# flysoaryun/LF-VIO

Measured on AMD Instinct MI355X. Metric: sliding-window solves/sec (10 KF x N landmarks), higher is better.
Workload: dtype f64; 1 GPU; window300; landmarks=300, observations=1419, windows_per_gpu=1, marginalization=MARGIN_OLD, parallelism=1 independent window stream(s), one per GPU, no data-path collective

## Files before the change

lf-vio_amd/csrc/kernels_lin.h:

```cpp
#pragma once
#include "dev_factors.h"
#include "kernels_spec.h"
#include "tr_decide.h"
#include <type_traits>

#define SLOT(base, stride) ((Slot *)((char *)(base) + (size_t)blockIdx.y * (stride)))

constexpr int MODE_SOLVE = 0;
constexpr int MODE_MARG = 1;
constexpr int MODE_GATED = 16;
constexpr int MODE_DECIDE = 64;
constexpr int MODE_NOCOUNT = 32;
DEV bool tail_gate(const Slot *S, int done) { return done && S->tail_state == 0; }
DEV bool is_marg(int mode) { return mode >= MODE_MARG; }
DEV const MargPlan *marg_plan(const Slot *S, int mode) { return &S->marg[mode - MODE_MARG]; }

DEV int gidx20(int p, int q) { return p * 20 - (p * (p - 1)) / 2 + (q - p); }

constexpr int SETUP_PRIOR_WGS = 16;
constexpr int SETUP_WGS = 2 + SETUP_PRIOR_WGS;
constexpr int SETUP_TILED_MAXN = 88;
__global__ __launch_bounds__(256, 4) void k_setup(char *base, size_t stride, int mode, int zero_wt) {
  Slot *S = SLOT(base, stride);
  const int tid = threadIdx.x;
  constexpr int SETUP_PRIOR_SLAB = 2048, SETUP_LDS = LFVIO_WINDOW_SIZE * 15 * 16;
  static_assert(SETUP_LDS >= SETUP_PRIOR_SLAB + LFVIO_MAX_PRIOR_DIM && SETUP_LDS >= 84 + TAB_SCRATCH, "k_setup's workspace");
  __shared__ double sh_setup[SETUP_LDS];
  const int setup_wgs = (zero_wt & 4) ? 3 : SETUP_WGS;
  if (blockIdx.x == 0) {
    const double *src = (const double *)&S->x0;
    double *dst = (double *)&S->x[0];
    for (int k = tid; k < (int)(sizeof(FrameState) / 8); k += 256) dst[k] = src[k];
    if (tid == 0) {
      TRState *t = &S->tr;
      tr_init(t, S->init_radius, S->fn_tol);
      S->tail_state = 0;
      S->passes_used = 0;
      S->dec_pending = 0;
      if (mode >= MODE_MARG) t->mu = 0.0;
    }
    double *bt = sh_setup;
    if (tid < 77) bt[tid] = (&S->x0.pose[0][0])[tid];
    else if (tid < 84) bt[tid] = S->x0.ex[tid - 77];
    __syncthreads();
    const unsigned offm = build_tab(bt, &S->tab[0], tid, bt + 84);
    if (tid == 0) S->ex_fixed_off = ((offm >> TAB_EX_BIT) & 1u) && !S->est_ex;
    if (tid == 0 && S->spec_on) spec_arm(S);
  } else if (blockIdx.x == 1) {
    if (tid >= 16 * ((LFVIO_WINDOW_SIZE + 3) & ~3)) return;
    const int grp = tid >> 4, l = tid & 15;
    const int f = grp < LFVIO_WINDOW_SIZE ? grp : 0;
    const bool mine = grp < LFVIO_WINDOW_SIZE && S->imu_active[f];
    const double *cov = S->imu[f].covariance;
    double m0[15], m1[15];
#pragma unroll
    for (int r = 0; r < 15; r++) {
      m0[r] = l < 15 ? cov[r * 15 + l] : (r == 0 ? 1.0 : 0.0);
      m1[r] = r == l + 1 ? 1.0 : 0.0;
    }
#pragma unroll
    for (int k = 0; k < 15; k++) {
      int p = k;
      double best = -1.0, piv = 0.0;
#pragma unroll
      for (int r = 0; r < 15; r++) {
        const double v = fabs(m0[r]);
        if (r >= k && v > best) best = v, p = r, piv = m0[r];
      }
      p = row_bcast_ik(p, k), piv = row_bcast_k(piv, k);
      double csr[15];
#pragma unroll
      for (int r = 0; r < 15; r++) csr[r] = row_bcast_k(m0[r], k);
      const double ck = csr[k];
#pragma unroll
      for (int r = 0; r < 15; r++) csr[r] = r == p ? ck : csr[r];
      auto step = [&](double(&m)[15]) {
        double Mp = m[0];
#pragma unroll
        for (int r = 1; r < 15; r++) Mp = p == r ? m[r] : Mp;
        const double Mk = m[k], mk = Mp / piv;
#pragma unroll
        for (int r = 0; r < 15; r++) {
          const double Msr = r == p ? Mk : m[r];
          m[r] = r == k ? mk : Msr - csr[r] * mk;
        }
      };
      step(m0), step(m1);
    }
    double *T = sh_setup + f * (15 * 16);
#pragma unroll
    for (int r = 0; r < 15; r++) {
      if (l == 15) T[r * 16] = m0[r];
      else if (l < 14) T[r * 16 + l + 1] = m1[r];
    }
    __syncthreads();
    const int li = l < 15 ? l : 0;
    double lrow[15], mrow[15];
#pragma unroll
    for (int j = 0; j < 15; j++) mrow[j] = T[li * 16 + j], lrow[j] = 0.0;
    bool ok = true;
#pragma unroll
    for (int j = 0; j < 15; j++) {
      double t = mrow[j];
#pragma unroll
      for (int k = 0; k < j; k++) t -= lrow[k] * row_bcast_k(lrow[k], j);
      const double sj = row_bcast_k(t, j);
      if (!(sj > 0.0)) ok = false;
      const double d = sqrt(sj);
      lrow[j] = l == j ? d : t / d;
    }
    if (mine && l < 15) {
#pragma unroll
      for (int i = 0; i < 15; i++) S->imu_sqrt[f][i * 15 + l] = (l >= i && ok) ? lrow[i] : 0.0;
    }
    if (mine && !ok && l == 0) S->imu_active[f] = 0;
  } else if (blockIdx.x >= setup_wgs) {
    const int l = (blockIdx.x - setup_wgs) * 256 + tid;
    if (l < S->N) S->lam[0][l] = S->lam0[l];
    if ((zero_wt & 1) && !S->wt_clean) {
      double2 *wt = (double2 *)(double *)S->Wt;
      const int nw = gridDim.x - setup_wgs, w = blockIdx.x - setup_wgs;
      for (int e = w * 256 + tid; e < WT_PAIRS * SPEC_MAX_LM; e += nw * 256) wt[e] = make_double2(0.0, 0.0);
    }
  } else {
    if (!S->prior_valid) return;
    const int n = S->prior_n;
    const int part = blockIdx.x - 2;
    constexpr int PRIOR_EPT = 8;
    const int nb4 = (n + 3) >> 2, tiles = nb4 * (nb4 + 1) / 2;
    static_assert(((SETUP_TILED_MAXN + 3) / 4) * ((SETUP_TILED_MAXN + 3) / 4 + 1) / 2 <= 256, "a thread per 4 x 4 block of the upper triangle");
    if (zero_wt & 4) {
      if (part != 0) return;
      constexpr int PRIOR_SLAB = SETUP_PRIOR_SLAB;
      double *Js = sh_setup;
      const double *J = S->prior_J;
      const int rows_per = PRIOR_SLAB / n;
      int br = 0, rem = tid < tiles ? tid : 0;
      while (rem >= nb4 - br) rem -= nb4 - br, br++;
      const int r0 = 4 * br, c0 = 4 * (br + rem);
      double acc[4][4], accb = 0;
#pragma unroll
      for (int i = 0; i < 4; i++)
#pragma unroll
        for (int j = 0; j < 4; j++) acc[i][j] = 0.0;
      for (int k0 = 0; k0 < n; k0 += rows_per) {
        const int nk = min(rows_per, n - k0);
        __syncthreads();
        {
          double v[8];
          const double *Jk = J + k0 * n;
#pragma unroll
          for (int q = 0; q < 8; q++) v[q] = Jk[tid + 256 * q < nk * n ? tid + 256 * q : 0];
          const double rv = S->prior_r[k0 + (tid < nk ? tid : 0)];
#pragma unroll
          for (int q = 0; q < 8; q++)
            if (tid + 256 * q < nk * n) Js[tid + 256 * q] = v[q];
          if (tid < nk) Js[PRIOR_SLAB + tid] = rv;
        }
        __syncthreads();
        if (tid < tiles) {
#pragma unroll 2
          for (int k = 0; k < nk; k++) {
            double a[4], b[4];
#pragma unroll
            for (int i = 0; i < 4; i++) a[i] = Js[k * n + r0 + i], b[i] = Js[k * n + c0 + i];
#pragma unroll
            for (int i = 0; i < 4; i++)
#pragma unroll
              for (int j = 0; j < 4; j++) acc[i][j] = fma(a[i], b[j], acc[i][j]);
          }
        }
        if (tid < n)
          for (int k = 0; k < nk; k++) accb = fma(Js[k * n + tid], Js[PRIOR_SLAB + k], accb);
      }
      if (tid < tiles) {
#pragma unroll
        for (int i = 0; i < 4; i++)
#pragma unroll
          for (int j = 0; j < 4; j++) {
            const int r = r0 + i, c = c0 + j;
            if (r < n && c < n) {
              S->prior_A[r * n + c] = acc[i][j];
              if (c0 != r0) S->prior_A[c * n + r] = acc[i][j];
            }
          }
      }
      if (tid < n) S->prior_b0[tid] = accb;
      return;
    }
    const int np = gridDim.y >= 8 ? min(SETUP_PRIOR_WGS, (n * n + 256 * PRIOR_EPT - 1) / (256 * PRIOR_EPT)) : SETUP_PRIOR_WGS;
    if (part >= np) return;
    constexpr int PRIOR_SLAB = SETUP_PRIOR_SLAB;
    double *Js = sh_setup;
    const double *J = S->prior_J;
    const int rows_per = PRIOR_SLAB / n;
    double acc[PRIOR_EPT], accb = 0;
#pragma unroll
    for (int q = 0; q < PRIOR_EPT; q++) acc[q] = 0;
    for (int k0 = 0; k0 < n; k0 += rows_per) {
      const int nk = min(rows_per, n - k0);
      __syncthreads();
      {
        static_assert(PRIOR_SLAB <= 8 * 256, "eight elements of a slab per thread");
        double v[8];
        const double *Jk = J + k0 * n;
#pragma unroll
        for (int q = 0; q < 8; q++) v[q] = Jk[tid + 256 * q < nk * n ? tid + 256 * q : 0];
        const double rv = S->prior_r[k0 + (tid < nk ? tid : 0)];
#pragma unroll
        for (int q = 0; q < 8; q++)
          if (tid + 256 * q < nk * n) Js[tid + 256 * q] = v[q];
        if (tid < nk) Js[PRIOR_SLAB + tid] = rv;
      }
      __syncthreads();
#pragma unroll
      for (int q = 0; q < PRIOR_EPT; q++) {
        const int e = part * 256 + tid + q * 256 * np;
        if (e < n * n) {
          const int r = e / n, c = e % n;
          double s = acc[q];
          for (int k = 0; k < nk; k++) s = fma(Js[k * n + r], Js[k * n + c], s);
          acc[q] = s;
        }
      }
      if (part == 0 && tid < n)
        for (int k = 0; k < nk; k++) accb = fma(Js[k * n + tid], Js[PRIOR_SLAB + k], accb);
    }
#pragma unroll
    for (int q = 0; q < PRIOR_EPT; q++) {
      const int e = part * 256 + tid + q * 256 * np;
      if (e < n * n) S->prior_A[e] = acc[q];
    }
    if (part == 0 && tid < n) S->prior_b0[tid] = accb;
  }
}

DEV void load_pair_uniform(const Tab *T, int pair, PairU &u) {
  u.M2 = ldm(T->M2[pair]);
  u.T = ldm(T->T[pair]);
  u.ric = ldm(T->ric);
  u.ricT = ldm(T->ricT);
  u.c = ld3(T->c[pair]);
  u.tic = ld3(T->tic);
  u.offc = u.offr = nullptr;
}
DEV void load_pair_uniform(const Tab *T, int pair, unsigned offm, PairU &u) {
  load_pair_uniform(T, pair, u);
  if (offm && pair_is_off(offm, pair % 11)) u.offc = T->c[tab_cj(pair)], u.offr = T->T[0];
}

typedef double double4_t __attribute__((ext_vector_type(4)));

constexpr int LIN_THREADS = 256;
constexpr int LIN_LDS_LM = LM_BLOCK * (WLD + 1) + 64 + 2 * LM_BLOCK;
constexpr int LIN_PRIOR_N = 76;
constexpr int LIN_LDS_PRIOR = LIN_PRIOR_N * LIN_PRIOR_N + 4 * KP;
constexpr int LIN_LDS = LIN_LDS_LM > LIN_LDS_PRIOR ? LIN_LDS_LM : LIN_LDS_PRIOR;

DEV double quad_sum(double v) {
  v += dpp_f64<0xB1>(v);
  v += dpp_f64<0x4E>(v);
  return v;
}
DEV d3 quad_sum3(d3 v) { return mk3(quad_sum(v.x), quad_sum(v.y), quad_sum(v.z)); }
template <int LPT>
DEV double track_sum(double v) { return LPT == 8 ? sum8(v) : quad_sum(v); }
template <int LPT>
DEV d3 track_sum3(d3 v) { return mk3(track_sum<LPT>(v.x), track_sum<LPT>(v.y), track_sum<LPT>(v.z)); }

template <bool TIGHT>
DEV void schur_block(int lm0, int lmb, int mode, int Nlim, double (*tile)[WLD + 1], const double *lcoef, const double *le, double *part) {
  const int tid = threadIdx.x;
  const int wv = tid >> 6, lane = tid & 63, kk = lane >> 4, cc = lane & 15;
  double4_t acc[4];
  int ct[4], cu[4];
  bool scale_k[4];
#pragma unroll
  for (int j = 0; j < 4; j++) {
    acc[j] = double4_t{0, 0, 0, 0};
    const int ti = wv + 4 * j;
    const int t = ti < 5 ? 0 : ti < 9 ? 1 : ti < 12 ? 2 : ti < 14 ? 3 : 4;
    const int u = ti - (t * 5 - (t * (t - 1)) / 2) + t;
    ct[j] = ti < NT ? 16 * t + cc : 0, cu[j] = ti < NT ? 16 * u + cc : 0;
    scale_k[j] = mode == MODE_SOLVE && cu[j] == COL_K;
  }
  int rows = Nlim - lm0;
  rows = rows > lmb ? lmb : rows;
  auto sweep = [&](auto ntl) {
    constexpr int NTL = decltype(ntl)::value;
    for (int s4 = 0; 4 * s4 < rows; s4++) {
      const int row = 4 * s4 + kk;
      const double coef = lcoef[row], eb = le[row];
#pragma unroll
      for (int j = 0; j < NTL; j++)
        acc[j] = __builtin_amdgcn_mfma_f64_16x16x4f64(coef * tile[row][ct[j]], tile[row][cu[j]] * (scale_k[j] ? eb : 1.0), acc[j], 0, 0, 0);
    }
  };
  if (TIGHT) {
    if (__builtin_amdgcn_readfirstlane(wv) + 12 < NT) sweep(std::integral_constant<int, 4>{});
    else sweep(std::integral_constant<int, 3>{});
  } else {
    for (int s4 = 0; 4 * s4 < rows; s4++) {
      const int row = 4 * s4 + kk;
      const double coef = lcoef[row], eb = le[row];
#pragma unroll
      for (int j = 0; j < 4; j++) {
        if (wv + 4 * j >= NT) continue;
        const double xa = tile[row][ct[j]];
        double xb = tile[row][cu[j]];
        if (mode == MODE_SOLVE && cu[j] == COL_K) xb *= eb;
        acc[j] = __builtin_amdgcn_mfma_f64_16x16x4f64(coef * xa, xb, acc[j], 0, 0, 0);
      }
    }
  }
#pragma unroll
  for (int j = 0; j < 4; j++) {
    if (wv + 4 * j >= NT) continue;
#pragma unroll
    for (int r = 0; r < 4; r++) part[(wv + 4 * j) * 256 + r * 64 + lane] = acc[j][r];
  }
}
DEV int w_col(int ci, int start, int cnt) { return ci < 6 * cnt ? 6 * start + ci : 66 + (ci - 6 * cnt); }

struct LinView {
  const FrameState *x;
  const Tab *tab;
  const double *lam;
  double mu;
};

template <int LPT>
DEV void lin_schur_only_role(Slot *S, const LinView &lv, int wg, double *lds, double *part) {
  constexpr int LMB = LIN_THREADS / LPT;
  double(*tile)[WLD + 1] = (double(*)[WLD + 1]) lds;
  double *lcoef = lds + LM_BLOCK * (WLD + 1) + 64, *le = lcoef + LM_BLOCK;
  const int tid = threadIdx.x;
  for (int e = tid; e < LM_BLOCK * (WLD + 1); e += LIN_THREADS) lds[e] = 0.0;
  __syncthreads();
  {
    const int lml = tid / LPT, q = tid % LPT, l = wg * LMB + lml;
    if (l < S->N) {
      const int st = S->lm_start[l], cnt = S->lm_cnt[l];
      const double *w = S->W + S->lm_woff[l];
      for (int ci = q; ci < w_row_len(cnt); ci += LPT) tile[lml][w_col(ci, st, cnt)] = w[ci];
    }
  }
  if (tid < LM_BLOCK) {
    const int l = wg * LMB + tid;
    double cf = 0.0, eb = 0.0;
    if (tid < LMB && l < S->N) {
      const double sc = S->scale_l[l], s2a = sc * sc * S->a[l];
      const double D2 = fmin(fmax(s2a, 1e-6), 1e32);
      eb = s2a + lv.mu * D2;
      const double einv = 1.0 / eb;
      cf = sc * sc * einv;
      S->einv_l[l] = einv;
    }
    lcoef[tid] = cf, le[tid] = eb;
  }
  __syncthreads();
  schur_block<false>(wg * LMB, LMB, MODE_SOLVE, S->N, tile, lcoef, le, part);
}

#ifdef LFVIO_LIN_PROFILE
#define LSTAMP(k) do { if (blockIdx.x == 0 && mode == MODE_SOLVE && threadIdx.x == 0) S->dbg[k] = (long long)__builtin_readcyclecounter(); } while (0)
#else
#define LSTAMP(k) do { } while (0)
#endif
template <bool TIGHT, int LPT, bool OFFS>
DEV void lin_landmark_role(Slot *S, const LinView &lv, int wg, int mode, double *lds, double *part) {
  constexpr int LMB = LIN_THREADS / LPT;
  double(*tile)[WLD + 1] = (double(*)[WLD + 1]) lds;
  double *red = lds + LM_BLOCK * (WLD + 1);
  double *lcoef = red + 64, *le = lcoef + LM_BLOCK;
  const int tid = threadIdx.x, lml = tid / LPT, q = tid % LPT;
  const TRState *tr = &S->tr;
  const Tab *T = lv.tab;
  const int Nlim = is_marg(mode) ? marg_plan(S, mode)->N0 : S->N;
  const int l = wg * LMB + lml;
  const bool valid = l < Nlim;
  const int est_td = S->est_td;
  const int est_ex = is_marg(mode) ? 1 : S->est_ex;
  const double td = lv.x->td;
  LSTAMP(22);
  for (int e = tid; e < LM_BLOCK * (WLD + 1); e += LIN_THREADS) lds[e] = 0.0;
  if (tid < 2 * LM_BLOCK) lcoef[tid] = 0.0;
// ... 82 lines not shown
    }
    S->a[l] = a;
    S->b[l] = b;
    tile[lml][COL_B] = b;
    lam2 = lam * lam;
    bmax = fabs(b);
  } else {
    cost = 0.0;
  }
  LSTAMP(18);
  cost = wave_sum(cost);
  g2 = wave_sum(g2);
  asv2 = wave_sum(asv2);
  lam2 = wave_sum(lam2);
  bmax = wave_max(bmax);
  if ((tid & 63) == 0) {
    double *r = red + 8 * (tid >> 6);
    r[0] = cost, r[1] = g2, r[2] = asv2, r[3] = lam2, r[4] = bmax;
  }
  lds_barrier();
  if (tid < 5) {
    double *p = S->lm_part + (size_t)(LPT == 8 ? wg >> 1 : wg) * LMS + (LPT == 8 && (wg & 1) ? 10 : 0);
    p[tid] = tid < 4 ? ((red[tid] + red[8 + tid]) + (red[16 + tid] + red[24 + tid]))
                     : fmax(fmax(red[4], red[12]), fmax(red[20], red[28]));
  }
  LSTAMP(19);
  if (valid) {
    double *w = S->W + woff_l;
    for (int ci = q; ci < w_row_len(cnt_l); ci += LPT) w[ci] = tile[lml][w_col(ci, i, cnt_l)];
  }
  if (TIGHT && mode == MODE_SOLVE && S->N <= SPEC_MAX_LM) {
    constexpr int WGRP = LIN_THREADS / LMB;
    const int lr = tid % LMB, wg4 = tid / LMB;
    double2 *wt = (double2 *)(double *)S->Wt + wg * LMB + lr;
    constexpr int WPT = (WT_PAIRS + WGRP - 1) / WGRP;
    double2 v[WPT];
#pragma unroll
    for (int k = 0; k < WPT; k++) {
      const int cp = wg4 + WGRP * k, c = cp < WT_PAIRS ? 2 * cp : 0;
      v[k] = make_double2(tile[lr][c], c + 1 < KC ? tile[lr][c + 1] : 0.0);
    }
#pragma unroll
    for (int k = 0; k < WPT; k++) {
      const int cp = wg4 + WGRP * k;
      if (cp < WT_PAIRS) wt[(size_t)cp * SPEC_MAX_LM] = v[k];
    }
  }
  LSTAMP(23);
  schur_block<TIGHT>(wg * LMB, LMB, mode, Nlim, tile, lcoef, le, part);
  LSTAMP(20);
}

template <bool OFFS>
DEV void lin_gram_role(Slot *S, const LinView &lv, int wg, int mode, double *lds) {
  const int wv = threadIdx.x >> 6, lane = threadIdx.x & 63;
  const int chunk = 4 * wg + wv;
  if (chunk >= S->nChunks) return;
  if (is_marg(mode) && chunk >= marg_plan(S, mode)->nChunks0) return;
  double *my = lds + wv * (32 * 17 + 256 + 14 * 20);
  double(*stage)[17] = (double(*)[17]) my;
  double(*Qf)[16] = (double(*)[16])(my + 32 * 17);
  double(*E)[20] = (double(*)[20])(my + 32 * 17 + 256);
  double(*T1)[20] = (double(*)[20]) my;
  const Tab *T = lv.tab;
  const int pair = S->chunk_pair[chunk];
  const int j = pair % 11;
  const int begin = S->chunk_begin[chunk], end = S->chunk_end[chunk];
  const int est_td = S->est_td;
  const double td = lv.x->td;
  PairU u;
  if (OFFS) load_pair_uniform(T, pair, tab_offmask(T), u);
  else load_pair_uniform(T, pair, u);
  for (int e = lane; e < 14 * 20; e += 64) E[0][e] = 0.0;
  for (int e = lane; e < 32 * 17; e += 64) stage[0][e] = 0.0;
  const int idx = begin + lane;
  double c0[14], c1[14];
#pragma unroll
  for (int e = 0; e < 14; e++) c0[e] = c1[e] = 0.0;
  if (idx < end) {
    const int oj = S->pm_obs[idx], l = S->pm_lm[idx];
    const int oi = S->lm_obs0[l];
    const double lam = lv.lam[l];
    ObsPair ob;
    load_obs(S, oi, ob.pi, ob.vi, ob.tdi, ob.rowi);
    load_obs(S, oj, ob.pj, ob.vj, ob.tdj, ob.rowj);
    Basis B;
    visual_basis<OFFS>(ob, lam, td, est_td, S->tr_over_row, S->half_row, S->sqrt_info, u, B);
    c0[0] = B.red[0].x, c0[1] = B.red[0].y, c0[2] = B.red[0].z;
    c1[0] = B.red[1].x, c1[1] = B.red[1].y, c1[2] = B.red[1].z;
    c0[3] = B.jti[0].x, c0[4] = B.jti[0].y, c0[5] = B.jti[0].z;
    c1[3] = B.jti[1].x, c1[4] = B.jti[1].y, c1[5] = B.jti[1].z;
    c0[6] = B.jtj[0].x, c0[7] = B.jtj[0].y, c0[8] = B.jtj[0].z;
    c1[6] = B.jtj[1].x, c1[7] = B.jtj[1].y, c1[8] = B.jtj[1].z;
    c0[9] = B.jtx[0].x, c0[10] = B.jtx[0].y, c0[11] = B.jtx[0].z;
    c1[9] = B.jtx[1].x, c1[10] = B.jtx[1].y, c1[11] = B.jtx[1].z;
    c0[12] = B.jtd[0], c1[12] = B.jtd[1];
    c0[13] = B.r[0], c1[13] = B.r[1];
  }
  double4_t acc = double4_t{0, 0, 0, 0};
  const int nrounds = (end - begin + 15) >> 4;
  for (int r = 0; r < nrounds; r++) {
    __builtin_amdgcn_fence(__ATOMIC_RELEASE, "wavefront");
    if ((lane >> 4) == r) {
      const int row = 2 * (lane & 15);
#pragma unroll
      for (int e = 0; e < 14; e++) stage[row][e] = c0[e], stage[row + 1][e] = c1[e];
    }
    __builtin_amdgcn_fence(__ATOMIC_ACQ_REL, "wavefront");
#pragma unroll
    for (int g = 0; g < 8; g++) {
      const double v = stage[4 * g + (lane >> 4)][lane & 15];
      acc = __builtin_amdgcn_mfma_f64_16x16x4f64(v, v, acc, 0, 0, 0);
    }
  }
  __builtin_amdgcn_fence(__ATOMIC_RELEASE, "wavefront");
#pragma unroll
  for (int r = 0; r < 4; r++) Qf[(lane >> 4) + 4 * r][lane & 15] = acc[r];
  if (lane < 9) {
    const int r = lane / 3, c = lane % 3;
    const double m1 = T->M1[j][lane];
    E[r][c] = m1;
    E[r][6 + c] = -m1;
    E[r][12 + c] = T->M2[pair][lane] - T->ricT[lane];
  } else if (lane < 12) {
    const int k = lane - 9;
    E[3 + k][3 + k] = 1.0;
    E[6 + k][9 + k] = 1.0;
    E[9 + k][15 + k] = 1.0;
  } else if (lane == 12) {
    E[12][18] = 1.0;
    E[13][19] = 1.0;
  }
  __builtin_amdgcn_fence(__ATOMIC_ACQ_REL, "wavefront");
  for (int e = lane; e < 14 * 20; e += 64) {
    const int r = e / 20, c = e % 20;
    double s = 0;
#pragma unroll
    for (int k = 0; k < 14; k++) s = fma(Qf[r][k], E[k][c], s);
    T1[r][c] = s;
  }
  __builtin_amdgcn_fence(__ATOMIC_ACQ_REL, "wavefront");
  double *out = S->gram_part + (size_t)chunk * NGP;
  for (int e = lane; e < 400; e += 64) {
    const int p = e / 20, c = e % 20;
    if (p > c) continue;
    double s = 0;
#pragma unroll
    for (int k = 0; k < 14; k++) s = fma(E[k][p], T1[k][c], s);
    out[gidx20(p, c)] = s;
  }
}

template <bool raw_ready>
DEV void lin_imu_role(Slot *S, const LinView &lv, int f, int mode, double *lds) {
  double(*Jr)[30] = (double(*)[30]) lds;
  double(*Jw)[31] = (double(*)[31])(lds + 450);
  double *rr = lds + 450 + 465, *rw = rr + 16;
  const int tid = threadIdx.x;
  double *out = S->imu_out + (size_t)f * IMU_OUT;
  const bool active = S->imu_active[f] && (mode == MODE_SOLVE || (f == 0 && marg_plan(S, mode)->use_imu0)) &&
                      (!S->sharded || S->pose_side);
  if (!active) {
    for (int e = tid; e < IMU_OUT; e += LIN_THREADS) out[e] = 0.0;
    return;
  }
  const FrameState *x = lv.x;
  if (raw_ready) {
    const double *raw = S->imu_raw + (size_t)f * IMU_RAW;
    for (int e = tid; e < 450; e += LIN_THREADS) Jr[e / 30][e % 30] = raw[e];
    if (tid < 15) rr[tid] = raw[450 + tid];
  } else {
    for (int e = tid; e < 450; e += LIN_THREADS) Jr[e / 30][e % 30] = 0.0;
    __syncthreads();
    if (tid == 0) imu_raw_residual(&S->imu[f], S->g, x->pose[f], x->sb[f], x->pose[f + 1], x->sb[f + 1], rr);
    if (tid == 64) imu_raw_jacobian(&S->imu[f], S->g, x->pose[f], x->sb[f], x->pose[f + 1], x->sb[f + 1], &Jr[0][0]);
  }
  __syncthreads();
  const double *Sq = S->imu_sqrt[f];
  if (tid < 15) {
    double s = 0;
    for (int k = 0; k < 15; k++) s = fma(Sq[tid * 15 + k], rr[k], s);
    rw[tid] = s;
  }
  for (int e = tid; e < 450; e += LIN_THREADS) {
    const int r = e / 30, c = e % 30;
    double s = 0;
    for (int k = r; k < 15; k++) s = fma(Sq[r * 15 + k], Jr[k][c], s);
    Jw[r][c] = s;
  }
  __syncthreads();
  for (int e = tid; e < 900; e += LIN_THREADS) {
    const int p = e / 30, c = e % 30;
    double s = 0;
#pragma unroll
    for (int k = 0; k < 15; k++) s = fma(Jw[k][p], Jw[k][c], s);
    out[e] = s;
  }
  if (tid < 30) {
    double s = 0;
#pragma unroll
    for (int k = 0; k < 15; k++) s = fma(Jw[k][tid], rw[k], s);
    out[900 + tid] = s;
  }
  if (tid == 32) {
    double s = 0;
    for (int k = 0; k < 15; k++) s = fma(rw[k], rw[k], s);
    out[930] = 0.5 * s;
  }
}

template <bool STAGED>
DEV void lin_prior_role(Slot *S, const LinView &lv, int mode, double *lds) {
  const int n = S->prior_n;
  const bool staged = STAGED && n <= LIN_PRIOR_N;
  double *Js = lds, *dx = lds + (STAGED ? LIN_PRIOR_N * LIN_PRIOR_N : 0), *r = dx + KP, *part = r + KP;
  const int tid = threadIdx.x;
  double *g = S->prior_g;
  for (int c = tid; c < KP + 4; c += LIN_THREADS) g[c] = 0.0;
  if (!S->prior_valid || (S->sharded && !S->pose_side)) return;
  const FrameState *x = lv.x;
  const double *Jg = S->prior_J;
  if (staged) {
    constexpr int PER = (LIN_PRIOR_N * LIN_PRIOR_N + LIN_THREADS - 1) / LIN_THREADS;
    double v[PER];
#pragma unroll
    for (int k = 0; k < PER; k++) v[k] = tid + LIN_THREADS * k < n * n ? Jg[tid + LIN_THREADS * k] : 0.0;
    if (tid < S->prior_nb) prior_block_dx(S, x, tid, dx);
#pragma unroll
    for (int k = 0; k < PER; k++)
      if (tid + LIN_THREADS * k < n * n) Js[tid + LIN_THREADS * k] = v[k];
  } else if (tid < S->prior_nb) {
    prior_block_dx(S, x, tid, dx);
  }
  __syncthreads();
  const double *J = staged ? Js : Jg;
  for (int row = tid >> 2; row < n; row += LIN_THREADS / 4) {
    double s = 0;
    for (int c = tid & 3; c < n; c += 4) s = fma(J[row * n + c], dx[c], s);
    s = quad_sum(s);
    if ((tid & 3) == 0) r[row] = S->prior_r[row] + s;
  }
  __syncthreads();
  {
    const int c = tid & 127, h = tid >> 7, k0 = h ? n / 2 : 0, k1 = h ? n : n / 2;
    for (int cc = c; cc < n; cc += 128) {
      double s = 0;
      for (int k = k0; k < k1; k++) s = fma(J[k * n + cc], r[k], s);
      part[h * KP + cc] = s;
    }
  }
  __syncthreads();
  for (int c = tid; c < n; c += LIN_THREADS) g[S->prior_cmap[c]] = part[c] + part[KP + c];
  if (tid < 64) {
    double cs = 0;
    for (int row = tid; row < n; row += 64) cs += r[row] * r[row];
    cs = wave_sum(cs);
    if (tid == 0) g[KP] = 0.5 * cs;
  }
}

__global__ __launch_bounds__(64) void k_imu_raw(char *base, size_t stride, int count) {
  const int g = blockIdx.x * 64 + threadIdx.x;
  if (g >= count * LFVIO_WINDOW_SIZE) return;
  const int slot = g / LFVIO_WINDOW_SIZE, f = g - slot * LFVIO_WINDOW_SIZE;
  Slot *S = reinterpret_cast<Slot *>(base + stride * (size_t)slot);
  const TRFlags fl = tr_flags(&S->tr);
  if (fl.done | !fl.do_lin) return;
  if (!S->imu_active[f] || (S->sharded && !S->pose_side)) return;
  const FrameState *x = &S->x[fl.cur];
  double *raw = S->imu_raw + (size_t)f * IMU_RAW;
  for (int e = 0; e < 450; e++) raw[e] = 0.0;
  imu_raw_residual(&S->imu[f], S->g, x->pose[f], x->sb[f], x->pose[f + 1], x->sb[f + 1], raw + 450);
  imu_raw_jacobian(&S->imu[f], S->g, x->pose[f], x->sb[f], x->pose[f + 1], x->sb[f + 1], raw);
}

constexpr int LIN_ROLE_LM = 1, LIN_ROLE_GRAM = 2, LIN_ROLE_POSE = 4, LIN_ROLE_ALL = 7;
constexpr int LIN_ROLE_POSE_RAW = 8;
constexpr int LIN_LDS_POSE = 1024;
template <int ROLES, bool OFFS = true>
__global__ __launch_bounds__(LIN_THREADS, ROLES == LIN_ROLE_GRAM ? 3 : (ROLES == LIN_ROLE_POSE_RAW ? 6 : 2)) void k_lin(char *base, size_t stride, int mode_bits, int gLw, int gCh) {
  Slot *S = SLOT(base, stride);
  TRState *tr = &S->tr;
  const int mode = mode_bits & (MODE_GATED - 1);
  LSTAMP(21);
  const TRFlags fl = tr_flags(tr);
  int do_lin = fl.do_lin, do_schur = fl.do_schur, cur = fl.cur, acc_z = 0;
  double mu = tr->mu;
  int num_succ = tr->num_succ;
  if (mode_bits & MODE_GATED) {
    if (!tail_gate(S, fl.done)) return;
  } else {
    int done = fl.done;
    const bool owner = blockIdx.x == 0 && !(mode_bits & MODE_NOCOUNT);
    if ((mode_bits & MODE_DECIDE) && !done) {
      __shared__ TRDecision dsh;
      if (threadIdx.x < 64) {
        TRHead t = *reinterpret_cast<const TRHead *>(tr);
        const int K = decide_candidates(t);
        DecideSums sm;
        decide_sums(S, t, K, 0, S->nLmBlocks, threadIdx.x, sm);
        if (threadIdx.x == 0) {
          const int az = decide_walk(t, sm, K, 0, S->max_iter, owner ? tr : nullptr);
          decision_from(dsh, t, az);
          if (owner) S->dec = dsh, S->dec_pending = 1;
        }
      }
      __syncthreads();
      do_lin = __builtin_amdgcn_readfirstlane(dsh.do_lin), do_schur = __builtin_amdgcn_readfirstlane(dsh.do_schur);
      cur = __builtin_amdgcn_readfirstlane(dsh.cur), acc_z = __builtin_amdgcn_readfirstlane(dsh.acc_z), done = __builtin_amdgcn_readfirstlane(dsh.done);
      num_succ = __builtin_amdgcn_readfirstlane(dsh.num_succ);
      mu = __hiloint2double(__builtin_amdgcn_readfirstlane(__double2hiint(dsh.mu)), __builtin_amdgcn_readfirstlane(__double2loint(dsh.mu)));
      if (acc_z > 0 && blockIdx.x == gridDim.x - 1 && !(mode_bits & MODE_NOCOUNT)) {
        copy_accepted(S, acc_z, cur, S->N, threadIdx.x, LIN_THREADS);
        if (S->spec_on) {
          __threadfence();
          __syncthreads();
          if (threadIdx.x == 0) spec_publish(S, num_succ, cur);
        }
      } else if (acc_z == 0 && owner && threadIdx.x == 0 && S->spec_on) spec_publish(S, num_succ, cur);
    } else if (owner && threadIdx.x == 0 && mode == MODE_SOLVE && S->spec_on) spec_publish(S, num_succ, cur);
    if (mode == MODE_SOLVE && owner && !done && threadIdx.x == 0) S->passes_used++;
    if (done | (!do_lin & !do_schur)) return;
  }
  LinView lv;
  lv.x = acc_z > 0 ? &S->xE[acc_z > 0 ? acc_z - 1 : 0] : &S->x[cur];
  lv.tab = acc_z > 0 ? &S->tabE[acc_z > 0 ? acc_z - 1 : 0] : &S->tab[cur];
  lv.lam = acc_z > 0 ? (const double *)S->lamE[acc_z > 0 ? acc_z - 1 : 0] : (const double *)S->lam[cur];
  lv.mu = mu;
  __shared__ __attribute__((aligned(16))) double lds[(ROLES & (LIN_ROLE_LM | LIN_ROLE_GRAM)) ? LIN_LDS : LIN_LDS_POSE];
  int b = blockIdx.x;
  if (b < gLw) {
    if (ROLES & LIN_ROLE_LM) {
      const int half = S->lm_half, lmb = half ? LM_BLOCK / 2 : LM_BLOCK;
      const int nblk = ((is_marg(mode) ? marg_plan(S, mode)->N0 : S->N) + lmb - 1) / lmb;
      if (b >= nblk) return;
      double *part = S->schur_part + (size_t)b * SCHUR_LEN;
      if (half) {
        if (do_lin) lin_landmark_role<ROLES == LIN_ROLE_ALL, 8, OFFS>(S, lv, b, mode, lds, part);
        else lin_schur_only_role<8>(S, lv, b, lds, part);
      } else {
        if (do_lin) lin_landmark_role<ROLES == LIN_ROLE_ALL, 4, OFFS>(S, lv, b, mode, lds, part);
        else lin_schur_only_role<4>(S, lv, b, lds, part);
      }
    }
    return;
  }
  if (!do_lin) return;
  b -= gLw;
  if (b < gCh) {
    if (ROLES & LIN_ROLE_GRAM) lin_gram_role<OFFS>(S, lv, b, mode, lds);
    return;
  }
  b -= gCh;
  if (ROLES & (LIN_ROLE_POSE | LIN_ROLE_POSE_RAW)) {
    if (b < LFVIO_WINDOW_SIZE) {
      if (ROLES & LIN_ROLE_POSE_RAW) lin_imu_role<true>(S, lv, b, mode, lds);
      else lin_imu_role<false>(S, lv, b, mode, lds);
      return;
    }
    lin_prior_role<ROLES == LIN_ROLE_ALL>(S, lv, mode, lds);
  }
}

DEV int schur_index(int R, int Cc) {
  const int t = R >> 4, u = Cc >> 4;
  const int tile = t * 5 - (t * (t - 1)) / 2 + (u - t);
  const int row = R & 15, col = Cc & 15;
  return tile * 256 + (row >> 2) * 64 + ((row & 3) << 4) + col;
}

constexpr int HPP_ITEMS = PACKED + KP;
constexpr int HPP_BLOCKS = (HPP_ITEMS + 255) / 256;

DEV int imu_local(int c, int f) {
  if (c < 66) {
    const int fr = c / 6, l = c - 6 * fr;
    if (fr == f) return l;
    if (fr == f + 1) return 15 + l;
    return -1;
  }
  if (c < KC) return -1;
  const int fr = (c - KC) / 9, l = (c - KC) - 9 * fr;
  if (fr == f) return 6 + l;
  if (fr == f + 1) return 21 + l;
  return -1;
}
DEV int col_frame(int c) { return c < 66 ? c / 6 : (c < KC ? -10 : (c - KC) / 9); }
DEV bool pose_terms_here(const Slot *S, int r) { return !S->sharded || S->pose_side == 1 || (S->pose_side == 2 && r >= KC); }

DEV bool col_active(const Slot *S, int c, int mode) {
  if (mode >= MODE_MARG) return true;
  if (!S->est_ex && c >= off_ex() && c < off_ex() + 6) return false;
  if (!S->est_td && c == off_td()) return false;
  return true;
}

constexpr int PRE_GROUP = 32;
__global__ __launch_bounds__(256) void k_presum(char *base, size_t stride, int mode_bits, int groups) {
  const int PRE_SCHUR_BLOCKS = (SCHUR_LEN / 256) * groups;
  Slot *S = SLOT(base, stride);
  const TRState *tr = &S->tr;
  const int mode = mode_bits & (MODE_GATED - 1);
  const TRFlags fl = tr_flags_decided(S);
  if (mode_bits & MODE_GATED) {
    if (!tail_gate(S, fl.done)) return;
  } else if (fl.done | (!fl.do_lin & !fl.do_schur)) return;
  const int tid = threadIdx.x;
  int b = blockIdx.x;
  if (b < NPAIR) {
    if (!fl.do_lin) return;
    const int chunk_limit = is_marg(mode) ? marg_plan(S, mode)->nChunks0 : S->nChunks;
    const int c0 = S->pair_chunk0[b];
    int c1 = S->pair_chunk0[b + 1];
    if (c1 > chunk_limit) c1 = chunk_limit;
    if (tid < NGP) {
      const double *gp = S->gram_part + tid;
      double s0 = 0, s1 = 0, s2 = 0, s3 = 0;
      int c = c0;
      for (; c + 4 <= c1; c += 4) {
        s0 += gp[(size_t)c * NGP], s1 += gp[(size_t)(c + 1) * NGP];
        s2 += gp[(size_t)(c + 2) * NGP], s3 += gp[(size_t)(c + 3) * NGP];
      }
      for (; c < c1; c++) s0 += gp[(size_t)c * NGP];
      S->pairG[(size_t)b * NGP + tid] = (s0 + s1) + (s2 + s3);
    }
    return;
  }
  b -= NPAIR;
  if (b < PRE_SCHUR_BLOCKS) {
    if (!fl.do_schur) return;
    const int grp = b / (SCHUR_LEN / 256), e = (b % (SCHUR_LEN / 256)) * 256 + tid;
    int parts = S->nSchurParts;
    if (is_marg(mode)) parts = (marg_plan(S, mode)->N0 + S->schur_lm - 1) / S->schur_lm;
    const int p0 = grp * PRE_GROUP;
    if (p0 >= parts) return;
    const int p1 = min(parts, p0 + PRE_GROUP);
    double *sp = S->schur_part + e;
    double a0 = 0, a1 = 0, a2 = 0, a3 = 0;
    int p = p0;
    for (; p + 4 <= p1; p += 4) {
      a0 += sp[(size_t)p * SCHUR_LEN], a1 += sp[(size_t)(p + 1) * SCHUR_LEN];
      a2 += sp[(size_t)(p + 2) * SCHUR_LEN], a3 += sp[(size_t)(p + 3) * SCHUR_LEN];
    }
    for (; p < p1; p++) a0 += sp[(size_t)p * SCHUR_LEN];
    sp[(size_t)p0 * SCHUR_LEN] = (a0 + a1) + (a2 + a3);
    return;
  }
  if (!fl.do_lin) return;
  __shared__ double red[5][256];
  const int blocks = S->nLmBlocks;
  double v[5] = {0, 0, 0, 0, 0};
  for (int k = tid; k < blocks; k += 256) {
    const double *q = S->lm_part + (size_t)k * LMS;
    v[0] += q[0], v[1] += q[1], v[2] += q[2], v[3] += q[3], v[4] = fmax(v[4], q[4]);
  }
#pragma unroll
  for (int k = 0; k < 5; k++) red[k][tid] = v[k];
  __syncthreads();
  for (int w = 128; w > 0; w >>= 1) {
    if (tid < w) {
#pragma unroll
      for (int k = 0; k < 4; k++) red[k][tid] += red[k][tid + w];
      red[4][tid] = fmax(red[4][tid], red[4][tid + w]);
    }
    __syncthreads();
  }
  if (tid < 5) S->lm_sum[tid] = red[tid][0];
}

struct SumArgs {
  long long sum_off, sum_end_marg, sum_items, gram_part, pairG, imu_out, prior_A;
};
template <class T>
DEV T *blob_at(const Slot *S, long long off) { return (T *)((char *)S + off); }
#define SUM_KEEP(v) asm volatile("" ::"v"(v))

DEV void sum_hpp_entry(Slot *S, const SumArgs &o, int mode_bits, int e) {
  const int mode = mode_bits & (MODE_GATED - 1);
  const bool in = e < HPP_ITEMS;
  const int ec = in ? e : 0;
  const bool packed = ec < PACKED;
  int r, c;
  if (packed) {
    r = (int)((sqrt(8.0 * ec + 1.0) - 1.0) * 0.5);
    while ((r + 1) * (r + 2) / 2 <= ec) r++;
    while (r * (r + 1) / 2 > ec) r--;
    c = ec - r * (r + 1) / 2;
  } else {
    r = c = ec - PACKED;
  }
  const TRFlags fl = tr_flags_decided(S);
  const int tail_state = S->tail_state, est_ex = S->est_ex, est_td = S->est_td, prior_valid = S->prior_valid, sharded = S->sharded;
  const int pose_side = S->pose_side, pre_gram = S->pre_gram, prior_n = S->prior_n;
  const int marg_chunks = is_marg(mode) ? marg_plan(S, mode)->nChunks0 : 1;
  const int vis = r < KC ? (packed ? ec : SUM_VIS_PACKED + r) : 0;
  const int beg = blob_at<int>(S, o.sum_off)[vis];
  int end = blob_at<int>(S, o.sum_off)[vis + 1];
  const int endm = blob_at<int>(S, o.sum_end_marg)[vis];
  const int pr = S->prior_inv[r], pc = S->prior_inv[c];
  const double pg = S->prior_g[r];
  double imu_v[2] = {0.0, 0.0};
  const int f0 = col_frame(r);
  const double *imu_out = blob_at<double>(S, o.imu_out);
#pragma unroll
  for (int u = 0; u < 2; u++) {
    const int f = f0 - 1 + u;
    if (f0 >= 0 && f >= 0 && f < LFVIO_WINDOW_SIZE) {
      const int pl = imu_local(r, f), ql = imu_local(c, f);
      if (packed) {
        if (pl >= 0 && ql >= 0) imu_v[u] = imu_out[(size_t)f * IMU_OUT + pl * 30 + ql];
      } else if (pl >= 0) {
        imu_v[u] = imu_out[(size_t)f * IMU_OUT + 900 + pl];
      }
    }
  }
  SUM_KEEP(beg);
  SUM_KEEP(end);
  SUM_KEEP(endm);
  SUM_KEEP(pr);
  SUM_KEEP(pc);
  SUM_KEEP(pg);
  SUM_KEEP(imu_v[0]);
  SUM_KEEP(imu_v[1]);
  if (mode_bits & MODE_GATED) {
    if (!(fl.done && tail_state == 0)) return;
  } else if (fl.done | !fl.do_lin) return;
  if (!in) return;
  const bool act_r = is_marg(mode) || !((!est_ex && r >= off_ex() && r < off_ex() + 6) || (!est_td && r == off_td()));
  const bool act_c = is_marg(mode) || !((!est_ex && c >= off_ex() && c < off_ex() + 6) || (!est_td && c == off_td()));
  double val = 0.0;
  if (act_r && act_c) {
    if (is_marg(mode)) end = marg_chunks > 0 ? endm : beg;
    const bool pterms = !sharded || pose_side == 1 || (pose_side == 2 && r >= KC);
    const bool use_prior = packed && prior_valid && pterms && pr >= 0 && pc >= 0;
    double pa = 0.0;
    if (use_prior) pa = blob_at<double>(S, o.prior_A)[pr * prior_n + pc];
    if (r < KC) {
      const int *it = blob_at<int>(S, o.sum_items);
      const double *gp = blob_at<double>(S, pre_gram ? o.pairG : o.gram_part);
      double s0 = 0, s1 = 0, s2 = 0, s3 = 0;
      int k = beg;
      for (; k + 4 <= end; k += 4) {
        const int o0 = it[k], o1 = it[k + 1], o2 = it[k + 2], o3 = it[k + 3];
        s0 += gp[o0], s1 += gp[o1], s2 += gp[o2], s3 += gp[o3];
      }
      for (; k < end; k++) s0 += gp[it[k]];
      val += (s0 + s1) + (s2 + s3);
    }
    if (packed) {
      if (f0 >= 0 && pterms) {
#pragma unroll
        for (int u = 0; u < 2; u++) {
          const int f = f0 - 1 + u;
          if (f >= 0 && f < LFVIO_WINDOW_SIZE && imu_local(r, f) >= 0 && imu_local(c, f) >= 0) val += imu_v[u];
        }
      }
      if (use_prior) val += pa;
    } else {
      if (f0 >= 0 && pterms) {
#pragma unroll
        for (int u = 0; u < 2; u++) {
          const int f = f0 - 1 + u;
          if (f >= 0 && f < LFVIO_WINDOW_SIZE && imu_local(r, f) >= 0) val += imu_v[u];
        }
      }
      if (pterms) val += pg;
    }
  }
  if (packed) S->Hpp[e] = val;
  else S->gp[r] = val;
}

__global__ __launch_bounds__(256) void k_sum(char *base, size_t stride, int mode_bits, int pre, const SumArgs o) {
  Slot *S = SLOT(base, stride);
  const int mode = mode_bits & (MODE_GATED - 1);
  const int tid = threadIdx.x;
  int b = blockIdx.x;
  if (S->sharded && mode == MODE_SOLVE && !(mode_bits & MODE_GATED)) {
    const TRFlags f0 = tr_flags(&S->tr);
    if (f0.done | (!f0.do_lin & !f0.do_schur)) {
      if (S->pose_side != 1) {
        const bool cam_only = S->pose_side == 2;
        const int e = b * 256 + tid;
        double *x = S->xch;
        if (b < HPP_BLOCKS) {
          if (e < (cam_only ? SUM_VIS_PACKED : PACKED)) x[XOFF_H + e] = 0.0;
          else if (e >= PACKED && e < PACKED + (cam_only ? KC : KP)) x[XOFF_G + (e - PACKED)] = 0.0;
        } else if (b < HPP_BLOCKS + SCHUR_LEN / 256) {
          x[XOFF_S + (e - HPP_BLOCKS * 256)] = 0.0;
        } else if (tid < 16) {
          x[XOFF_C + tid] = 0.0;
        }
      }
      return;
    }
  }
  if (b < HPP_BLOCKS) {
    sum_hpp_entry(S, o, mode_bits, b * 256 + tid);
    return;
  }
  const TRFlags fl = tr_flags_decided(S);
  if (mode_bits & MODE_GATED) {
    if (!tail_gate(S, fl.done)) return;
  } else if (fl.done | (!fl.do_lin & !fl.do_schur)) return;
  b -= HPP_BLOCKS;
  if (b < SCHUR_LEN / 256) {
    if (!fl.do_schur) return;
    const int e = b * 256 + tid;
    int parts = S->nSchurParts;
    if (is_marg(mode)) parts = (marg_plan(S, mode)->N0 + S->schur_lm - 1) / S->schur_lm;
    const size_t ps = pre ? (size_t)PRE_GROUP * SCHUR_LEN : (size_t)SCHUR_LEN;
    if (pre) parts = (parts + PRE_GROUP - 1) / PRE_GROUP;
    const double *sp = S->schur_part + e;
    double a0 = 0, a1 = 0, a2 = 0, a3 = 0, a4 = 0, a5 = 0, a6 = 0, a7 = 0;
    int p = 0;
    for (; p + 8 <= parts; p += 8) {
      a0 += sp[p * ps], a1 += sp[(p + 1) * ps], a2 += sp[(p + 2) * ps], a3 += sp[(p + 3) * ps];
      a4 += sp[(p + 4) * ps], a5 += sp[(p + 5) * ps], a6 += sp[(p + 6) * ps], a7 += sp[(p + 7) * ps];
    }
    for (; p < parts; p++) a0 += sp[p * ps];
    S->schur_sum[e] = ((a0 + a1) + (a2 + a3)) + ((a4 + a5) + (a6 + a7));
    return;
  }
  if (!fl.do_lin) return;
  int blocks = pre ? 0 : S->nLmBlocks;
  if (pre) {
  } else if (tid < 4) {
    const int half = S->lm_half, N = S->N;
    double s = 0;
    for (int k = 0; k < blocks; k++) {
      s += S->lm_part[(size_t)k * LMS + tid];
      if (half && k * LM_BLOCK + LM_BLOCK / 2 < N) s += S->lm_part[(size_t)k * LMS + 10 + tid];
    }
    S->lm_sum[tid] = s;
  } else if (tid == 4) {
    const int half = S->lm_half, N = S->N;
    double m = 0;
    for (int k = 0; k < blocks; k++) {
      m = fmax(m, S->lm_part[(size_t)k * LMS + 4]);
      if (half && k * LM_BLOCK + LM_BLOCK / 2 < N) m = fmax(m, S->lm_part[(size_t)k * LMS + 14]);
    }
    S->lm_sum[4] = m;
  }
  if (S->sharded) {
    __syncthreads();
    double *sc = S->xch + XOFF_C;
    if (tid < 16) sc[tid] = 0.0;
    __syncthreads();
    if (tid == 0) {
      double cost = S->lm_sum[0];
      if (S->pose_side == 1) {
        cost += S->prior_g[KP];
        for (int f = 0; f < LFVIO_WINDOW_SIZE; f++) cost += S->imu_out[(size_t)f * IMU_OUT + 930];
      }
      sc[XS_COST] = cost;
      sc[XS_G2] = S->lm_sum[1], sc[XS_ASV2] = S->lm_sum[2], sc[XS_LAM2] = S->lm_sum[3], sc[XS_BMAX] = S->lm_sum[4];
      if (is_marg(mode)) sc[XS_N0] = (double)marg_plan(S, mode)->N0;
    }
  }
}
```

lf-vio_amd/csrc/kernels_marg.h:

```cpp
#pragma once
#include "kernels_solve.h"

constexpr int MARG_THREADS = 768;
constexpr int MARG_MAXD = 96;
constexpr int LDN = 80;
constexpr double JACOBI_TOL = 1e-19;
constexpr size_t MARG_LDS = (size_t)19072 * sizeof(double);
constexpr int BT_GROUP = 4;

DEV void gauge_landmarks(Slot *S, int l0) {
  const int l = l0 + (int)threadIdx.x;
  double *lam = S->lam[S->tr.cur];
  if (l < S->N) lam[l] = 1.0 / (1.0 / lam[l]);
}
template <class T>
DEV void copy_rounds(T *dst, const T *src, int n, int tid, int nthr) {
  for (int k0 = tid; k0 < n; k0 += 8 * nthr) {
    T v[8];
#pragma unroll
    for (int q = 0; q < 8; q++) v[q] = src[k0 + q * nthr < n ? k0 + q * nthr : 0];
#pragma unroll
    for (int q = 0; q < 8; q++)
      if (k0 + q * nthr < n) dst[k0 + q * nthr] = v[q];
  }
// ... 88 lines not shown
  const bool head = !late && src->valid == 1 && src->n == n && src->num_blocks == nb;
  if (head && tid < nb && !(src->blocks[tid].kind == S->prior_kind[tid] && src->blocks[tid].frame == S->prior_frame[tid] && src->block_idx[tid] == S->prior_idx[tid]))
    differs = 1;
  for (int i = 256 + tid; head && i < nb; i += 256)
    if (!(src->blocks[i].kind == S->prior_kind[i] && src->blocks[i].frame == S->prior_frame[i] && src->block_idx[i] == S->prior_idx[i])) differs = 1;
  __syncthreads();
  const bool same = head && !differs;
  if (!same) {
    if (tid == 0) S->prior_valid = 0, S->chain_err = 1;
    return;
  }
  double *J = S->prior_J, *r = S->prior_r;
  copy_rounds(J, src->linearized_jacobians, n * n, tid, 256);
  copy_rounds(r, src->linearized_residuals, n, tid, 256);
  copy_rounds(&S->prior_x0[0][0], &src->block_x0[0][0], nb * 9, tid, 256);
}
__global__ __launch_bounds__(128) void k_gauge(char *base, size_t stride, int gated) {
  Slot *S = SLOT(base, stride);
  if (gated && !tail_gate(S, S->tr.done)) return;
  if (blockIdx.x > 0) {
    gauge_landmarks(S, (blockIdx.x - 1) * 128);
    return;
  }
  gauge_poses(S, gated, false);
  if (gated && S->spec_on && threadIdx.x == 0) spec_settle(S);
}
__global__ __launch_bounds__(128) void k_decide_gauge(char *base, size_t stride, int publish) {
  Slot *S = SLOT(base, stride);
  decide_body(S);
  __syncthreads();
  if (!tail_gate(S, S->tr.done)) return;
  const int spec = S->spec_on;
  if (spec) {
    if (threadIdx.x == 0) spec_closing(S);
    __syncthreads();
  }
  {
    constexpr int LT = (SPEC_MAX_LM + 127) / 128;
    double *lam = S->lam[S->tr.cur];
    const int N = S->N, tid = threadIdx.x;
    double lv[LT];
#pragma unroll
    for (int k = 0; k < LT; k++) lv[k] = lam[tid + 128 * k < N ? tid + 128 * k : 0];
#pragma unroll
    for (int k = 0; k < LT; k++)
      if (tid + 128 * k < N) lam[tid + 128 * k] = 1.0 / (1.0 / lv[k]);
    for (int l0 = 128 * LT; l0 < N; l0 += 128) gauge_landmarks(S, l0);
  }
  gauge_poses(S, 1, publish != 0);
  if (spec && threadIdx.x == 0) spec_settle(S);
}
DEV void gauge_poses(Slot *S, int gated, bool publish) {
  TRState *ts = &S->tr;
  const int tid = threadIdx.x;
  __shared__ double rot[9], P0[3], oP0[3];
  FrameState *x = &S->x[ts->cur];
  if (tid == 0) {
    const m33 Rs0 = q2R(q_from_pose(S->x0.pose[0]));
    const m33 R00 = q2R(q_from_pose(x->pose[0]));
    const double h0 = sqrt(Rs0.a[0] * Rs0.a[0] + Rs0.a[3] * Rs0.a[3]), h00 = sqrt(R00.a[0] * R00.a[0] + R00.a[3] * R00.a[3]);
    const double c0 = Rs0.a[0] / h0, s0 = Rs0.a[3] / h0, c00 = R00.a[0] / h00, s00 = R00.a[3] / h00;
    const double cyd = c0 * c00 + s0 * s00, syd = s0 * c00 - c0 * s00;
    m33 rd;
    rd.a[0] = cyd, rd.a[1] = -syd, rd.a[2] = 0;
    rd.a[3] = syd, rd.a[4] = cyd, rd.a[5] = 0;
    rd.a[6] = 0, rd.a[7] = 0, rd.a[8] = 1;
    const double sin1deg = 0.017452406437283512;
    if (h0 < sin1deg || h00 < sin1deg) rd = mm(Rs0, tr(R00));
    for (int k = 0; k < 9; k++) rot[k] = rd.a[k];
    for (int k = 0; k < 3; k++) P0[k] = x->pose[0][k], oP0[k] = S->x0.pose[0][k];
  }
  __syncthreads();
  const m33 rd = ldm(rot);
  d3 Psi = mk3(0, 0, 0), Vsi = Psi;
  q4 qn = q4{1, 0, 0, 0};
  if (tid < 11) {
    const m33 Rsi = mm(rd, q2R(qnormalized(q_from_pose(x->pose[tid]))));
    Psi = mul(rd, ld3(x->pose[tid]) - ld3(P0)) + ld3(oP0);
    Vsi = mul(rd, ld3(x->sb[tid]));
    qn = R2q(Rsi);
  } else if (tid == 11) {
    qn = R2q(q2R(q_from_pose(x->ex)));
  }
  __syncthreads();
  __shared__ double bt[84 + TAB_SCRATCH];
  if (tid < 11) {
    const double pn[7] = {Psi.x, Psi.y, Psi.z, qn.x, qn.y, qn.z, qn.w};
#pragma unroll
    for (int k = 0; k < 7; k++) x->pose[tid][k] = pn[k], bt[7 * tid + k] = pn[k];
    x->sb[tid][0] = Vsi.x, x->sb[tid][1] = Vsi.y, x->sb[tid][2] = Vsi.z;
  } else if (tid == 11) {
    x->ex[3] = qn.x, x->ex[4] = qn.y, x->ex[5] = qn.z, x->ex[6] = qn.w;
#pragma unroll
    for (int k = 0; k < 3; k++) bt[77 + k] = x->ex[k];
    bt[80] = qn.x, bt[81] = qn.y, bt[82] = qn.z, bt[83] = qn.w;
  }
  __syncthreads();
  if (publish) publish_solution(S);
  if (tid == 0) {
    if (!gated) ts->done = 0;
    ts->do_lin = 1;
    ts->do_schur = 1;
    ts->chol_fail = 0;
  }
  build_tab(bt, &S->tab[ts->cur], tid, bt + 84);
}

__global__ __launch_bounds__(64) void k_spec_wait(char *base) {
  Slot *S = (Slot *)base;
  if (threadIdx.x != 0) return;
  const long long t0 = wall_clock64();
  while (spec_peek(&S->tail_state) == 3 && wall_clock64() - t0 < 10 * SPEC_WAIT_TICKS) __builtin_amdgcn_s_sleep(8);
}
__global__ __launch_bounds__(128) void k_spec_begin(char *base, size_t back) {
  Slot *S = (Slot *)base;
  Slot *S0 = (Slot *)(base - back);
  const int tid = threadIdx.x;
  __shared__ int sh_word, sh_go;
  const long long t0 = wall_clock64();
  for (;;) {
    if (tid == 0) {
      int go = 0, w = 0;
      const int last = S->shadow.last_word;
      for (;;) {
        const int f = spec_peek(&S0->spec.fin);
        w = spec_peek(&S0->spec.word);
        if (w != 0) {
          const int st = spec_ep(f) == spec_ep(w) ? spec_fin_state(f) : FIN_OPEN;
          if (st != FIN_OPEN) break;
          if (w != last) {
            go = 1;
            break;
          }
        }
        if (wall_clock64() - t0 > SPEC_WAIT_TICKS) break;
        __builtin_amdgcn_s_sleep(8);
      }
      spec_acquire();
      sh_word = w, sh_go = go;
    }
    __syncthreads();
    int go = __builtin_amdgcn_readfirstlane(sh_go);
    const int w = __builtin_amdgcn_readfirstlane(sh_word);
    if (!go) {
      if (tid == 0) S->shadow.word = 0, S->tr.done = 0;
      return;
    }
    const int ep = spec_ep(w), a = spec_acc(w), cur = w & 1;
    if (S->shadow.hdr_ep != ep) {
      const long long *src = (const long long *)S0;
      long long *dst = (long long *)S;
      constexpr int W0 = (int)(offsetof(Slot, lm_start) / 8), W1 = (int)(offsetof(Slot, x) / 8);
      static_assert(offsetof(Slot, lm_start) % 8 == 0 && offsetof(Slot, x) % 8 == 0, "header words");
      for (int k = tid; k < W1; k += 128) dst[k] = src[k] - (k >= W0 ? (long long)back : 0ll);
      const double *is = &S0->imu_sqrt[0][0];
      double *id = &S->imu_sqrt[0][0];
      for (int k = tid; k < LFVIO_WINDOW_SIZE * 225; k += 128) id[k] = is[k];
    }
    __syncthreads();
    {
      constexpr int XW = (int)(sizeof(FrameState) / 8), TW = (int)(sizeof(TRHead) / 8), XT = (XW + 127) / 128, LT = (SPEC_MAX_LM + 127) / 128;
      static_assert(TW <= 128, "the trust-region header in one trip");
      const double *xs = (const double *)&S0->x[cur];
      double *xd = (double *)&S->x[0];
      const double *ls = S0->lam[cur];
      double *ld = S->lam[0];
      const int N = S0->N;
      const long long *ts = (const long long *)&S0->tr;
      long long *td = (long long *)&S->tr;
      double xv[XT], lv[LT];
#pragma unroll
      for (int k = 0; k < XT; k++) xv[k] = xs[tid + 128 * k < XW ? tid + 128 * k : 0];
#pragma unroll
      for (int k = 0; k < LT; k++) lv[k] = ls[tid + 128 * k < N ? tid + 128 * k : 0];
      const long long tv = ts[tid < TW ? tid : 0];
#pragma unroll
      for (int k = 0; k < XT; k++)
        if (tid + 128 * k < XW) xd[tid + 128 * k] = xv[k];
#pragma unroll
      for (int k = 0; k < LT; k++)
        if (tid + 128 * k < N) ld[tid + 128 * k] = 1.0 / (1.0 / lv[k]);
      if (tid < TW) td[tid] = tv;
      for (int k = tid + 128 * LT; k < N; k += 128) ld[k] = 1.0 / (1.0 / ls[k]);
    }
    __syncthreads();
    if (tid == 0) {
      const int f = spec_ld(&S0->spec.fin), w2 = spec_ld(&S0->spec.word);
      const bool open = spec_ep(f) != ep || spec_fin_state(f) == FIN_OPEN;
      sh_go = (w2 == w && open && spec_cas(&S0->spec.own[a], SPEC_FREE, SPEC_SIDE) == SPEC_FREE) ? 1 : 0;
      S->shadow.hdr_ep = ep;
      S->shadow.last_word = w;
    }
    __syncthreads();
    go = __builtin_amdgcn_readfirstlane(sh_go);
    if (!go) {
      __syncthreads();
      continue;
    }
    if (tid == 0) {
      S->shadow.word = w, S->shadow.ticket = S0->spec.ticket;
      S->spec_on = 0, S->dec_pending = 0, S->tail_state = 0, S->chain_err = 0;
      S->tr.cur = 0, S->tr.done = 1;
    }
    __syncthreads();
    break;
  }
  gauge_poses(S, 1, false);
}

DEV bool spd_inverse_wave(const double *Am, double *Xout, int m, int lane, double floor) {
  double a[15];
#pragma unroll
  for (int j = 0; j < 15; j++) a[j] = (lane < m && j < m) ? Am[lane * m + j] : (lane == j ? 1.0 : 0.0);
  bool ok = true;
  double dinv = 1.0;
#pragma unroll
  for (int j = 0; j < 15; j++) {
    const double d = readlane_f64(a[j], j);
    ok = ok && (d > 0.0);
    const double rs = fast_rsqrt(d);
    const double l = lane == j ? d * rs : a[j] * rs;
    a[j] = l;
    dinv = lane == j ? rs : dinv;
#pragma unroll
    for (int c = j + 1; c < 15; c++) a[c] = fma(-l, readlane_f64(l, c), a[c]);
  }
  double y[15];
#pragma unroll
  for (int i = 0; i < 15; i++) {
    double t = lane == i ? 1.0 : 0.0;
#pragma unroll
    for (int k = 0; k < i; k++) t = fma(-readlane_f64(a[k], i), y[k], t);
    y[i] = t * readlane_f64(dinv, i);
  }
  double fro = 0;
#pragma unroll
  for (int r = 0; r < 15; r++) {
    double x = 0;
#pragma unroll
    for (int i = r; i < 15; i++) x = fma(readlane_f64(y[i], r), y[i], x);
    if (lane < m && r < m) Xout[r * m + lane] = x, fro += x * x;
  }
  fro = wave_sum(fro);
  return ok && fro * floor * floor < 1.0;
}

DEV void rr_pair(int k, int step, int np, int n, int &p, int &q) {
  if (k == 0) {
    p = step, q = np - 1;
  } else {
    p = step + k;
    if (p >= np - 1) p -= np - 1;
    q = step - k;
    if (q < 0) q += np - 1;
  }
  if (q >= n) q = -1;
}

DEV void jacobi_angle(double app, double aqq, double apq, double &c, double &s) {
  c = 1.0, s = 0.0;
  if (apq != 0.0 && fabs(apq) > 1e-18 * (fabs(app) + fabs(aqq))) {
#if defined(JAC_TRIVIAL)
    c = 0.8, s = 0.6;
#elif defined(JAC_IEEE)
    const double theta = (aqq - app) / (2.0 * apq);
    const double t = (theta >= 0 ? 1.0 : -1.0) / (fabs(theta) + sqrt(theta * theta + 1.0));
    c = rsqrt(t * t + 1.0);
    s = t * c;
#else
    const double d = aqq - app, e = 2.0 * apq;
    const double h2 = fma(d, d, e * e);
    const double h = h2 * fast_rsqrt(h2);
    const double t = (d >= 0 ? e : -e) * fast_rcp(fabs(d) + h);
    c = fast_rsqrt(fma(t, t, 1.0));
    s = t * c;
#endif
  }
}

DEV int jacobi_small(double *Am, double *Vm, int n, int tid, int nthreads, double *buf, double2 *cs, double *scratch) {
  const int np = n + (n & 1), half = np / 2;
  double *Ac = buf, *An = buf + 256, *Vc = buf + 512, *Vn = buf + 768;
  const bool act = tid < np * np;
  const int u = act ? tid / np : 0, v = act ? tid % np : 0;
  const int ku = u >> 1, bu = u & 1, kv = v >> 1, bv = v & 1;
  auto idx0 = [&](int p) { return (p & 1) ? np - 1 - (p >> 1) : (p >> 1); };
  auto sigma = [&](int p) {
    const int k = p >> 1;
    if (!(p & 1)) return k >= 1 ? 2 * (k - 1) : 3;
    if (k == 0) return 1;
    return k <= half - 2 ? 2 * (k + 1) + 1 : 2 * (half - 1);
  };
  if (act) {
    const int iu = idx0(u), iv = idx0(v);
    Ac[tid] = (iu < n && iv < n) ? Am[iu * n + iv] : 0.0;
    Vc[tid] = (u == iv) ? 1.0 : 0.0;
  }
  const int dst_a = sigma(u) * np + sigma(v), dst_v = u * np + sigma(v);
  const int blk = (2 * ku) * np + 2 * kv;
  __syncthreads();
  int sweeps = 0, g = 0;
  double prev_off = 1e300;
  for (int sweep = 0; sweep < JMAX_SWEEPS; sweep++) {
    double off = 0, dia = 0;
    if (act) {
      const double a = Ac[tid];
      if (u == v) dia = a * a;
      else off = a * a;
    }
    off = wave_sum(off), dia = wave_sum(dia);
// ... 257 lines not shown
        case 1: tri_matvec<1>(tc, k, ar, vj); break;
        case 2: tri_matvec<2>(tc, k, ar, vj); break;
        case 3: tri_matvec<3>(tc, k, ar, vj); break;
        default: tri_matvec<4>(tc, k, ar, vj); break;
      }
    }
    TSTAMP(1);
    __syncthreads();
    TSTAMP(2);
    if (tri) {
      switch (P) {
        case 0: tri_update<0>(tc, k, ar, vj); break;
        case 1: tri_update<1>(tc, k, ar, vj); break;
        case 2: tri_update<2>(tc, k, ar, vj); break;
        case 3: tri_update<3>(tc, k, ar, vj); break;
        default: tri_update<4>(tc, k, ar, vj); break;
      }
    }
    TSTAMP(3);
    __syncthreads();
    TSTAMP(4);
    if (sp && (k & 7) == 6 && *sp->flag) return true;
  }
  if (tri) {
#pragma unroll
    for (int i = 0; i < 5; i++)
#pragma unroll
      for (int q = 0; q < 5; q++)
        if (r0 + 16 * i == n - 1 && c0 + 16 * q == n - 1) dd[n - 1] = ar[i][q];
  }
  if (poller) spec_poll_issue(*sp);
  __syncthreads();
  ESTAMP(27);
  if (tid < n) ee2[tid] = ee[tid] * ee[tid];
  {
    double lo = 1e300, hi = -1e300;
    if (tid < n) {
      const double r = (tid > 0 ? fabs(ee[tid - 1]) : 0.0) + (tid + 1 < n ? fabs(ee[tid]) : 0.0);
      lo = dd[tid] - r, hi = dd[tid] + r;
    }
    lo = -wave_max(-lo), hi = wave_max(hi);
    if (lane == 0) scr[wave] = lo, scr[16 + wave] = hi;
  }
  __syncthreads();
  double gl = fmin(scr[0], scr[1]), gu = fmax(scr[16], scr[17]);
  {
    const double tn = fmax(fabs(gl), fabs(gu));
    gl -= 2.2e-16 * tn * n + 1e-300, gu += 2.2e-16 * tn * n + 1e-300;
  }
  if (tid < 96) Tglob[tid] = tid < n ? dd[tid] : gu + 1.0, Tglob[96 + tid] = tid + 1 < n ? ee[tid] * ee[tid] : 0.0;
  __threadfence();
  __syncthreads();
  __builtin_amdgcn_s_dcache_inv();
  const unsigned long long ta = (unsigned long long)Tglob;
  unsigned tlo = __builtin_amdgcn_readfirstlane((unsigned)ta), thi = __builtin_amdgcn_readfirstlane((unsigned)(ta >> 32));
  asm volatile("" : "+s"(tlo), "+s"(thi));
  sdouble *Tg = (sdouble *)(((unsigned long long)thi << 32) | tlo);
  {
    const double pivmin = 1e-290;
    const int g3 = lane == 63 ? 20 : lane / 3, l8 = lane == 63 ? 3 : lane - 3 * g3;
    const int m = wave * 21 + g3;
    const int mm = m < n ? m : n - 1;
    {
      int *cntg = (int *)pp;
      double *blo = nn2, *bhi = nn2 + 96;
      const double step = (gu - gl) * (1.0 / 257.0);
      if (tid < 96) blo[tid] = gl, bhi[tid] = gu;
      if (tid < 256) cntg[tid] = sturm_count(Tg, n, gl + step * (double)(tid + 1));
      __syncthreads();
      if (tid <= 256) {
        const int c0 = tid > 0 ? cntg[tid - 1] : 0, c1 = tid < 256 ? cntg[tid] : n;
        const double a = tid > 0 ? gl + step * (double)tid : gl, b = tid < 256 ? gl + step * (double)(tid + 1) : gu;
        for (int e = max(c0, 0); e < min(c1, n); e++) blo[e] = a, bhi[e] = b;
      }
      __syncthreads();
    }
    double lo = nn2[mm], hi = nn2[96 + mm];
    if (tid < 256)
      for (int round = 0; round < 23; round++) {
        const double w = hi - lo;
        const double sigma = lo + w * (double)(l8 < 3 ? l8 + 1 : 1) * 0.25;
        const int cnt = sturm_count(Tg, n, sigma);
        const int f1 = cnt <= mm ? 1 : 0;
        const unsigned long long bal = __ballot(f1);
        const int f = __builtin_popcount((unsigned)(bal >> (3 * g3)) & 7u);
        const double nlo = f == 0 ? lo : lo + w * (double)f * 0.25, nhi = f == 3 ? hi : lo + w * (double)(f + 1) * 0.25;
        lo = nlo, hi = nhi;
      }
    if (tid < 256 && m < n && l8 == 0) lam[m] = 0.5 * (lo + hi);
    if (poller) spec_poll_take(*sp), spec_poll_issue(*sp);
    __syncthreads();
    ESTAMP(28);
    if (sp && *sp->flag) return true;
    const int set = tid >> 7, me = tid & 127;
    const bool work = set < 2 && me < n;
    const int mec = work ? me : 0;
    const double l = lam[mec];
    if (work && set == 0) {
      double q = dd[0] - l;
      A[mec] = q;
      for (int i0 = 1; i0 < n; i0 += 8) {
        double dv[8], ev[8], qs[8];
#pragma unroll
        for (int u = 0; u < 8; u++) dv[u] = dd[i0 + u], ev[u] = ee2[i0 + u - 1];
#pragma unroll
        for (int u = 0; u < 8; u++) {
          q = fma(-ev[u], fast_rcp(guard_pivot(q, pivmin)), dv[u] - l);
          qs[u] = q;
        }
#pragma unroll
        for (int u = 0; u < 8; u++)
          if (i0 + u < n) A[(i0 + u) * LDN + mec] = qs[u];
      }
    } else if (work) {
      double q = dd[n - 1] - l;
      DM[(n - 1) * LDN + mec] = q;
      for (int i0 = n - 2; i0 >= 0; i0 -= 8) {
        double dv[8], ev[8], qs[8];
#pragma unroll
        for (int u = 0; u < 8; u++) dv[u] = dd[max(i0 - u, 0)], ev[u] = ee2[max(i0 - u, 0)];
#pragma unroll
        for (int u = 0; u < 8; u++) {
          q = fma(-ev[u], fast_rcp(guard_pivot(q, pivmin)), dv[u] - l);
          qs[u] = q;
        }
#pragma unroll
        for (int u = 0; u < 8; u++)
          if (i0 - u >= 0) DM[(i0 - u) * LDN + mec] = qs[u];
      }
    }
    __syncthreads();
    ESTAMP(16);
    {
      const int half = (n + 1) >> 1, i0 = set == 0 ? 0 : half, i1 = set == 0 ? half : n;
      double gmin = 1e300;
      int kt = i0;
      if (work) {
#pragma unroll 8
        for (int i = i0; i < i1; i++) {
          const double g = fabs(A[i * LDN + mec] + DM[i * LDN + mec] - (dd[i] - l));
          if (g < gmin) gmin = g, kt = i;
        }
      }
      __syncthreads();
      if (work) {
        pp[set * 96 + mec] = gmin;
        ((int *)ee2)[set * 96 + mec] = kt;
      }
    }
    if (poller) spec_poll_take(*sp);
    __syncthreads();
    ESTAMP(17);
    if (sp && *sp->flag) return true;
    if (work) {
      const double g0 = pp[mec], g1 = pp[96 + mec];
      const int kt = g1 < g0 ? ((int *)ee2)[96 + mec] : ((int *)ee2)[mec];
      double z = 1.0, nn = 0.0;
      if (set == 0) {
        A[kt * LDN + mec] = 1.0;
        for (int i0 = n - 2; i0 >= 0; i0 -= 8) {
          double c[8], zs[8];
#pragma unroll
          for (int u = 0; u < 8; u++) {
            const int i = max(i0 - u, 0);
            c[u] = -ee[i] * fast_rcp(guard_pivot(A[i * LDN + mec], pivmin));
          }
#pragma unroll
          for (int u = 0; u < 8; u++) {
            const bool on = i0 - u < kt && i0 - u >= 0;
            z = on ? c[u] * z : 1.0;
            zs[u] = z;
            nn = on ? fma(z, z, nn) : nn;
          }
#pragma unroll
          for (int u = 0; u < 8; u++)
            if (i0 - u < kt && i0 - u >= 0) A[(i0 - u) * LDN + mec] = zs[u];
        }
      } else {
        for (int i0 = 1; i0 < n; i0 += 8) {
          double c[8], zs[8];
#pragma unroll
          for (int u = 0; u < 8; u++) {
            const int i = min(i0 + u, n - 1);
            c[u] = -ee[i - 1] * fast_rcp(guard_pivot(DM[i * LDN + mec], pivmin));
          }
#pragma unroll
          for (int u = 0; u < 8; u++) {
            const bool on = i0 + u > kt && i0 + u < n;
            z = on ? c[u] * z : 1.0;
            zs[u] = z;
            nn = on ? fma(z, z, nn) : nn;
          }
#pragma unroll
          for (int u = 0; u < 8; u++)
            if (i0 + u > kt && i0 + u < n) A[(i0 + u) * LDN + mec] = zs[u];
        }
      }
      nn2[set * 96 + mec] = nn;
    }
  }
  __syncthreads();
  ESTAMP(29);
  {
    const int m = tid >> 3, l8 = tid & 7;
    const bool live = m < n;
    const int mm = live ? m : 0;
    double zz[10];
    const double sc = fast_rsqrt(1.0 + nn2[mm] + nn2[96 + mm]);
#pragma unroll
    for (int q = 0; q < 10; q++) {
      const int i = l8 + 8 * q;
      zz[q] = i < n ? A[i * LDN + mm] * sc : 0.0;
    }
    int k = n - 3;
    for (; k >= 0 && (k & (BT_GROUP - 1)) != BT_GROUP - 1; k--) bt_dispatch<1>(RV, tau, k, n, l8, zz);
    for (; k >= 0; k -= BT_GROUP) bt_dispatch<BT_GROUP>(RV, tau, k, n, l8, zz);
    const double l = lam[mm];
    double rb = 0.0;
#pragma unroll
    for (int q = 0; q < 10; q++) {
      const int i = l8 + 8 * q;
      if (i < n) rb = fma(zz[q], b[i], rb);
    }
    rb = sum8(rb);
    if (live) {
      const bool keep = l > eps;
      const double sq = keep ? sqrt(l) : 0.0;
#pragma unroll
      for (int q = 0; q < 10; q++) {
        const int i = l8 + 8 * q;
        if (i < n) out->linearized_jacobians[m * n + i] = sq * zz[q];
      }
      if (l8 == 0) out->linearized_residuals[m] = keep ? rb / sq : 0.0;
    }
  }
  return false;
}

DEV void spec_deliver(Slot *S, Slot *S0, int my_word, bool publish) {
  const int tid = threadIdx.x, nthr = blockDim.x;
  __shared__ int give;
  if (tid == 0) {
    const int ep = spec_ep(my_word), a = spec_acc(my_word);
    long long t0 = wall_clock64();
    int g = 0;
    for (;;) {
      const int f = spec_peek(&S0->spec.fin), w = spec_peek(&S0->spec.word);
      if (spec_ep(w) != ep) break;
      const int st = spec_ep(f) == ep ? spec_fin_state(f) : FIN_OPEN;
      if (st >= FIN_MAIN) {
        g = st == FIN_SIDE && spec_fin_acc(f) == a;
        break;
      }
      if (w != my_word) break;
      if (wall_clock64() - t0 > SPEC_WAIT_TICKS) {
        if (spec_cas(&S0->spec.own[a], SPEC_SIDE, SPEC_ABANDON) == SPEC_SIDE) break;
        t0 = wall_clock64();
      }
      __builtin_amdgcn_s_sleep(8);
    }
    give = g;
  }
  __syncthreads();
  if (!give) return;
  const LfvioPrior *src = &S->prior_out;
  LfvioPrior *dst = &S0->prior_out;
  const int n = src->valid == 1 ? src->n : 0;
  copy_rounds((long long *)dst, (const long long *)src, (int)(offsetof(LfvioPrior, linearized_jacobians) / 8), tid, nthr);
  copy_rounds(dst->linearized_jacobians, src->linearized_jacobians, n * n, tid, nthr);
  copy_rounds(dst->linearized_residuals, src->linearized_residuals, n, tid, nthr);
  __syncthreads();
  if (publish) publish_prior(S0);
  char *m = (char *)S0->mail;
  if (tid == 0) {
    __threadfence_system();
    __hip_atomic_store(&S0->tail_state, 2, __ATOMIC_RELAXED, __HIP_MEMORY_SCOPE_AGENT);
    if (m) __hip_atomic_store((int *)m + 7, S->shadow.ticket, __ATOMIC_RELAXED, __HIP_MEMORY_SCOPE_SYSTEM);
  }
}

template <bool WORKER>
__global__ __launch_bounds__(MARG_THREADS) void k_marg_solve(char *base, size_t stride, int flag_bits) {
  extern __shared__ __attribute__((aligned(16))) double smem[];
  const int flag = flag_bits & 255, force_eig = (flag_bits >> 8) & 1, gated = (flag_bits >> 9) & 1;
  const int publish = (flag_bits >> 10) & 1;
  constexpr bool worker = WORKER;
  Slot *S = worker ? (Slot *)base : SLOT(base, stride);
  Slot *S0 = worker ? (Slot *)(base - stride) : S;
  __shared__ int spec_flag;
  SpecPoll sp{S0, worker ? S->shadow.word : 0, &spec_flag, 0, 0};
  if (threadIdx.x == 0) spec_flag = 0;
  const bool poller = worker && threadIdx.x == MARG_THREADS - 1;
  TRState *tr = &S->tr;
  const MargPlan *mp = &S->marg[flag];
  const int tid = threadIdx.x;
  LfvioPrior *out = &S->prior_out;
  if (gated && !tail_gate(S, tr->done)) return;
  if (worker && sp.my_word == 0) return;
  if (!mp->valid) {
    if (tid == 0) out->valid = -1;
    if (worker) {
      __syncthreads();
      spec_deliver(S, S0, sp.my_word, publish != 0);
      return;
    }
    if (gated && tid == 0) S->iters_done = tr->iteration, S->tail_state = 2;
    if (gated && publish) {
      __syncthreads();
      publish_prior(S);
    }
    return;
  }
  if (poller) spec_poll_issue(sp);
  STAMP(S, 10);
  const double *Sc = S->schur_sum;
  const bool sub = mp->N0 > 0 || S->sharded;
  const int m15 = mp->m15, n = mp->n, D = m15 + n;
  double *Ag = S->mscr;
  double *A = smem;
  double *bv = A + 92 * 92;
  double *Am = bv + 96;
  double *Vm = Am + 256;
  double *Ainv = Vm + 256;
  double *Tm = Ainv + 256;
  double *Ar = smem + 12544;
  double *br = Ar + 76 * LDN;
  double2 *cs = (double2 *)(br + 80);
  int *perm = (int *)(cs + 96);
  double *scr = (double *)(perm + 96);
  double *RV = smem, *vec8 = smem + 5776, *DMs = smem + 5776 + 672;
  for (int c = tid; c < KP; c += MARG_THREADS) {
    const int a = mp->col[c];
    if (a >= 0) perm[a] = c;
  }
  __syncthreads();
  {
    constexpr int GR = (92 * 92 + MARG_THREADS - 1) / MARG_THREADS;
    const double *Hp = &S->Hpp[0];
    double hv[GR], sv[GR];
#pragma unroll
    for (int k = 0; k < GR; k++) {
      const int e = tid + MARG_THREADS * k, ec = e < D * D ? e : 0;
      const int r = D ? perm[ec / max(D, 1)] : 0, c = D ? perm[ec % max(D, 1)] : 0;
      const int hi = max(r, c), lo = min(r, c);
      hv[k] = Hp[hi * (hi + 1) / 2 + lo];
      sv[k] = (sub && hi < KC) ? Sc[schur_index(lo, hi)] : 0.0;
    }
#pragma unroll
    for (int k = 0; k < GR; k++) {
      const int e = tid + MARG_THREADS * k;
      if (e < D * D) A[e] = hv[k] - sv[k];
    }
  }
  for (int a = tid; a < D; a += MARG_THREADS) {
    const int c = perm[a];
    double v = S->gp[c];
    if (sub && c < KC) v -= Sc[schur_index(c, COL_B)];
    bv[a] = v;
  }
  if (poller) spec_poll_take(sp), spec_poll_issue(sp);
  __syncthreads();
  STAMP(S, 11);
  if (worker && spec_flag) return;
  for (int e = tid; e < m15 * m15; e += MARG_THREADS) {
    const int r = e / m15, c = e % m15;
    Am[e] = 0.5 * (A[r * D + c] + A[c * D + r]);
  }
  __syncthreads();
  const double eps = 1e-8;
  __shared__ int spd_fast;
  if (tid < 64) {
    const bool fast = m15 <= 15 && !force_eig && spd_inverse_wave(Am, Ainv, m15, tid, 1e3 * eps);
    if (tid == 0) spd_fast = fast ? 1 : 0;
  }
  __syncthreads();
  int sw1 = 0;
  if (!spd_fast) {
    sw1 = jacobi_small(Am, Vm, m15, tid, MARG_THREADS, Tm, cs, scr);
    __syncthreads();
    for (int e = tid; e < m15 * m15; e += MARG_THREADS) {
      const int r = e / m15, c = e % m15;
      double s = 0;
      for (int k = 0; k < m15; k++) {
        const double ev = Am[k * m15 + k];
        if (ev > eps) s += Vm[r * m15 + k] * (1.0 / ev) * Vm[c * m15 + k];
      }
      Ainv[e] = s;
    }
    __syncthreads();
  }
  STAMP(S, 12);
  for (int e = tid; e < n * m15; e += MARG_THREADS) {
    const int r = e / m15, c = e % m15;
    double s = 0;
    for (int k = 0; k < m15; k++) s = fma(A[(m15 + r) * D + k], Ainv[k * m15 + c], s);
    Tm[e] = s;
  }
  __syncthreads();
  {
    const int nb4 = (n + 3) >> 2;
    for (int blk = tid; blk < nb4 * nb4; blk += MARG_THREADS) {
      const int r0 = 4 * (blk / nb4), c0 = 4 * (blk % nb4);
      double acc[4][4];
#pragma unroll
      for (int i = 0; i < 4; i++)
#pragma unroll
        for (int j = 0; j < 4; j++) acc[i][j] = 0.0;
      for (int k = 0; k < m15; k++) {
        double tv[4], av[4];
#pragma unroll
        for (int i = 0; i < 4; i++) tv[i] = Tm[min(r0 + i, n - 1) * m15 + k], av[i] = A[k * D + m15 + min(c0 + i, n - 1)];
#pragma unroll
        for (int i = 0; i < 4; i++)
#pragma unroll
          for (int j = 0; j < 4; j++) acc[i][j] = fma(tv[i], av[j], acc[i][j]);
      }
#pragma unroll
      for (int i = 0; i < 4; i++)
#pragma unroll
        for (int j = 0; j < 4; j++)
          if (r0 + i < n && c0 + j < n) Ar[(r0 + i) * LDN + c0 + j] = A[(m15 + r0 + i) * D + m15 + c0 + j] - acc[i][j];
    }
  }
  for (int r = tid; r < n; r += MARG_THREADS) {
    double s = 0;
    for (int k = 0; k < m15; k++) s = fma(Tm[r * m15 + k], bv[k], s);
    br[r] = bv[m15 + r] - s;
  }
  __syncthreads();
  double *Aout = Ag + 92 * 92 + 96;
  for (int e = tid; e < n * n; e += MARG_THREADS) {
    const int r = e / n, c = e % n;
    Aout[e] = Ar[max(r, c) * LDN + min(r, c)];
  }
  for (int r = tid; r < n; r += MARG_THREADS) Aout[n * n + r] = br[r];
  if (poller) spec_poll_take(sp);
  __syncthreads();
  if (worker && spec_flag) return;
  STAMP(S, 13);
  if (eig_tridiag<WORKER>(Ar, br, n, tid, RV, DMs, vec8, scr, (double *)cs, S->eig_aux, out, 1e-8, S->dbg, &sp)) return;
  if (tid == 0) S->dbg[24] = sw1;
  STAMP(S, 14);
  const FrameState *x = &S->x[tr->cur];
  if (tid < mp->nb) {
    const int kind = mp->kind[tid], frame = mp->frame[tid];
    out->blocks[tid].kind = kind;
    out->blocks[tid].frame = mp->shifted_frame[tid];
    out->block_idx[tid] = mp->idx[tid];
    const double *xb = kind == LFVIO_BLOCK_POSE ? x->pose[frame]
                       : kind == LFVIO_BLOCK_SPEEDBIAS ? x->sb[frame]
                       : kind == LFVIO_BLOCK_EX_POSE ? x->ex
                                                     : &x->td;
    const int gs = (kind == LFVIO_BLOCK_POSE || kind == LFVIO_BLOCK_EX_POSE) ? 7 : (kind == LFVIO_BLOCK_SPEEDBIAS ? 9 : 1);
    for (int k = 0; k < 9; k++) out->block_x0[tid][k] = k < gs ? xb[k] : 0.0;
  }
  STAMP(S, 15);
  if (tid == 0) {
    out->valid = 1;
    out->m = m15 + (S->sharded ? (int)(S->xch[XOFF_C + XS_N0] + 0.5) : mp->N0);
    out->n = n;
    out->num_blocks = mp->nb;
    if (gated && !worker) S->iters_done = tr->iteration, S->tail_state = 2;
  }
  if (worker) {
    __syncthreads();
    spec_deliver(S, S0, sp.my_word, publish != 0);
    return;
  }
  if (gated && publish) {
    __syncthreads();
    publish_prior(S);
  }
}
```

lf-vio_amd/csrc/kernels_spec.h:

```cpp
#pragma once
#include "dev_math.h"
#include "dev_types.h"

constexpr long long SPEC_WAIT_TICKS = 300000;

DEV int spec_ld(const int *p) { return __hip_atomic_load(p, __ATOMIC_ACQUIRE, __HIP_MEMORY_SCOPE_AGENT); }
DEV int spec_peek(const int *p) { return __hip_atomic_load(p, __ATOMIC_RELAXED, __HIP_MEMORY_SCOPE_AGENT); }
DEV void spec_acquire() { __builtin_amdgcn_fence(__ATOMIC_ACQUIRE, "agent"); }
DEV void spec_st(int *p, int v) { __hip_atomic_store(p, v, __ATOMIC_RELEASE, __HIP_MEMORY_SCOPE_AGENT); }
DEV int spec_cas(int *p, int expect, int v) {
  __hip_atomic_compare_exchange_strong(p, &expect, v, __ATOMIC_ACQ_REL, __ATOMIC_ACQUIRE, __HIP_MEMORY_SCOPE_AGENT);
  return expect;
}
DEV int spec_ep(int w) { return (int)((unsigned)w >> 16); }
DEV int spec_acc(int w) { return (w & 0xffff) >> 1; }
DEV int spec_fin_state(int f) { return f & 3; }
DEV int spec_fin_acc(int f) { return (f & 0xffff) >> 2; }

DEV void spec_arm(Slot *S) {
  const int ep = (S->spec.ep % 0x7fff) + 1;
  spec_st(&S->spec.word, 0);
  for (int k = 0; k < SPEC_OWN; k++) S->spec.own[k] = SPEC_FREE;
  S->spec.ep = ep;
  S->spec.ticket = S->mail ? __hip_atomic_load((const int *)S->mail + 6, __ATOMIC_RELAXED, __HIP_MEMORY_SCOPE_SYSTEM) : 0;
  spec_st(&S->spec.fin, 0);
}
DEV void spec_publish(Slot *S, int num_succ, int cur) {
  if (num_succ < SPEC_OWN && S->spec.ticket != 0) spec_st(&S->spec.word, S->spec.ep << 16 | num_succ << 1 | cur);
}
DEV void spec_closing(Slot *S) {
  __hip_atomic_store(&S->spec.fin, S->spec.ep << 16 | FIN_CLOSING, __ATOMIC_SEQ_CST, __HIP_MEMORY_SCOPE_AGENT);
  __threadfence();
}
DEV bool spec_settle(Slot *S) {
  const int a = S->tr.num_succ;
  bool side = false;
  if (a < SPEC_OWN) {
    const int was = spec_cas(&S->spec.own[a], SPEC_FREE, SPEC_MAIN);
    if (was == SPEC_SIDE) side = spec_cas(&S->spec.own[a], SPEC_SIDE, SPEC_COMMIT) == SPEC_SIDE;
    if (was != SPEC_FREE && !side) spec_st(&S->spec.own[a], SPEC_MAIN);
  }
  if (side) S->tail_state = 3, S->iters_done = S->tr.iteration;
  spec_st(&S->spec.fin, S->spec.ep << 16 | (a < SPEC_OWN ? a : 0) << 2 | (side ? FIN_SIDE : FIN_MAIN));
  return side;
}

DEV bool spec_stale(const Slot *S0, int my_word) {
  const int f = spec_ld(&S0->spec.fin), w = spec_ld(&S0->spec.word);
  if (spec_ep(w) != spec_ep(my_word)) return true;
  if (w != my_word) return true;
  const int st = spec_ep(f) == spec_ep(my_word) ? spec_fin_state(f) : FIN_OPEN;
  return st >= FIN_MAIN && spec_fin_acc(f) != spec_acc(my_word);
}

struct SpecPoll {
  const Slot *S0;
  int my_word;
  int *flag;
  int f, w;
};
DEV void spec_poll_issue(SpecPoll &p) {
  p.f = __hip_atomic_load(&p.S0->spec.fin, __ATOMIC_RELAXED, __HIP_MEMORY_SCOPE_AGENT);
  p.w = __hip_atomic_load(&p.S0->spec.word, __ATOMIC_RELAXED, __HIP_MEMORY_SCOPE_AGENT);
}
DEV void spec_poll_take(SpecPoll &p) {
  const int st = spec_ep(p.f) == spec_ep(p.my_word) ? spec_fin_state(p.f) : FIN_OPEN;
  if (p.w != p.my_word || (st >= FIN_MAIN && spec_fin_acc(p.f) != spec_acc(p.my_word))) *p.flag = 1;
}
```

lf-vio_amd/csrc/lfvio_hip.hip:

```cpp
#include <hip/hip_runtime.h>
#include <dlfcn.h>
typedef struct ncclComm *ncclComm_t;
#define NCCL_UNIQUE_ID_BYTES 128
typedef struct {
  char internal[NCCL_UNIQUE_ID_BYTES];
} ncclUniqueId;
typedef int ncclResult_t;
typedef int ncclDataType_t;
typedef int ncclRedOp_t;
constexpr ncclResult_t ncclSuccess = 0;
constexpr ncclRedOp_t ncclSum = 0;
constexpr ncclDataType_t ncclDouble = 8;

#include <algorithm>
#include <chrono>
#include <cmath>
#include <cstdio>
#include <cstdlib>
#include <cstring>
#include <memory>
#include <string>
#include <type_traits>
#include <vector>

// ... 31 lines not shown
  size_t lm_start, lm_cnt, lm_obs0, lm_perm, lm_woff, lam0, obs[8], pm_obs, pm_lm, chunk_pair, chunk_begin, chunk_end, sum_off, sum_end_marg, sum_items, prior_J,
      prior_r;
  size_t lam[2], lamE[SPEC_EXTRA], cost_partE, prior_A, a, b, W, Wt, scale_l, grad_l, gn_l, diag_l, einv_l, d1, d2, gram_part, pairG, schur_part,
      xch, lm_part, cost_part, imu_out, imu_raw, mscr, eig_aux;
};

Layout make_layout(int maxN, int maxM) {
  Layout L;
  L.maxN = maxN;
  L.maxM = maxM;
  L.capLmBlocks = std::max(1, (maxN + LM_BLOCK - 1) / LM_BLOCK);
  L.capChunks = 64 + maxM / CHUNK_MAX;
  L.capSchurParts = std::max(L.capLmBlocks + 1, 2 * ((std::min(maxN, SPEC_MAX_LM) + LM_BLOCK - 1) / LM_BLOCK));
  static_assert(LINB_LEN >= SCHUR_LEN, "the Schur partials of k_lin share the array of k_linb's group partials, which are the larger");
  size_t o = align_up(sizeof(Slot), 256);
  auto take = [&](size_t bytes) {
    size_t r = o;
    o = align_up(o + bytes, 256);
    return r;
  };
  const size_t N = std::max(maxN, 1), M = std::max(maxM, 1), LB = (size_t)L.capLmBlocks * LM_BLOCK;
  L.in_begin = o;
  L.lm_start = take(N * 4), L.lm_cnt = take(N * 4), L.lm_obs0 = take(N * 4), L.lm_perm = take(N * 4);
  L.lm_woff = take((N + 1) * 4);
  L.lam0 = take(N * 8);
  for (int k = 0; k < 8; k++) L.obs[k] = take(M * 8);
  L.pm_obs = take(M * 4), L.pm_lm = take(M * 4);
  L.chunk_pair = take((size_t)L.capChunks * 4), L.chunk_begin = take((size_t)L.capChunks * 4),
  L.chunk_end = take((size_t)L.capChunks * 4);
  L.prior_r = take(LFVIO_MAX_PRIOR_DIM * 8);
  L.sum_off = take((size_t)(SUM_VIS + 1) * 4), L.sum_end_marg = take((size_t)SUM_VIS * 4);
  L.sum_items = take((size_t)SUM_ITEMS_CAP * 4);
  L.prior_J = take((size_t)LFVIO_MAX_PRIOR_DIM * LFVIO_MAX_PRIOR_DIM * 8);
  L.in_end = o;
  L.linw_begin = o;
  for (int k = 0; k < 8; k++) L.anc[k] = take(N * 8);
  for (int k = 0; k < 8; k++) L.pmo[k] = take(M * 8);
  L.pm_pair = take(M);
  L.linb_lm0 = take(((size_t)L.capLmBlocks + LFVIO_NUM_FRAMES + 1) * 4), L.linb_ns = take(((size_t)L.capLmBlocks + LFVIO_NUM_FRAMES + 1) * 4);
  L.linw_end = o;
  L.lam[0] = take(LB * 8), L.lam[1] = take(LB * 8);
  for (int k = 0; k < SPEC_EXTRA; k++) L.lamE[k] = take((size_t)SPEC_MAX_LM * 8);
  L.cost_partE = take((size_t)SPEC_EXTRA * (SPEC_MAX_LM / 64) * LMS * 8);
  L.prior_A = take((size_t)LFVIO_MAX_PRIOR_DIM * LFVIO_MAX_PRIOR_DIM * 8);
  L.a = take(LB * 8), L.b = take(LB * 8), L.W = take(LB * WLD * 8);
  L.Wt = take((size_t)WT_PAIRS * std::max((size_t)SPEC_MAX_LM, LB) * 16);
  L.scale_l = take(LB * 8), L.grad_l = take(LB * 8), L.gn_l = take(LB * 8), L.diag_l = take(LB * 8);
  L.einv_l = take(LB * 8), L.d1 = take(LB * 8), L.d2 = take(LB * 8);
  L.gram_part = take((size_t)L.capChunks * NGP * 8);
  L.pairG = take((size_t)NPAIR * NGP * 8);
  L.schur_part = take((size_t)L.capSchurParts * LINB_LEN * 8);
  L.xch = take((size_t)XCH_ALLOC * 8);
  L.lm_part = take((size_t)L.capLmBlocks * LMS * 8);
  L.cost_part = take((size_t)L.capLmBlocks * LMS * 8);
  L.imu_out = take((size_t)LFVIO_WINDOW_SIZE * IMU_OUT * 8);
  L.imu_raw = take((size_t)LFVIO_WINDOW_SIZE * IMU_RAW * 8);
  L.mscr = take((size_t)HPP_CAP * 8);
  L.eig_aux = take(4096);
  L.total = align_up(o, 4096);
  return L;
}

size_t down_bytes(int maxN) { return sizeof(FrameState) * 2 + sizeof(TRState) + 2 * ((size_t)maxN * 8 + 128) + sizeof(LfvioPrior) + 4096; }

struct SlotHostInfo {
  bool spec_on = false;
  bool offs_first = false, offs_all = false;
  int N = 0, M = 0, gLm = 0, gLw = 0, gCh = 0, gSc = 0;
  int marg_n = 0;
  int prior_n = 0;
  int max_iter = 0;
  double max_seconds = -1.0;
  std::vector<int> perm;
  bool linw_ok = false;
  bool linb_ok = false;
  int linb_ng = 0;
  bool uploaded = false;
  bool resident = false;
  LfvioPrior in_prior;
  bool has_in_prior = false;
  bool in_prior_device = false;
  struct MargOut {
    int valid = 0, n = 0, m = 0, nb = 0;
    int kind[LFVIO_MAX_PRIOR_BLOCKS], frame[LFVIO_MAX_PRIOR_BLOCKS], idx[LFVIO_MAX_PRIOR_BLOCKS];
  } marg_out[2];
  int mail_seq = 0;
  std::vector<int> list_key;
  int list_items = -1;
};

struct Grid {
  int lm, ch, sc, lw;
  int ch_raw;
};

struct SetupLaunch {
  int gx, bits;
};

struct Route {
  enum Sweep { ROLES = 0, LINW = 1, LINB = 2 } sweep;
  int count;
  Grid g;
  size_t role_wgs;
  bool split;
  int linb_gx;
  SetupLaunch setup;
  int offs;
};

struct GraphKey {
  int count = 0, lm = 0, ch = 0, sc = 0, sweep = -1, linb_gx = 0, offs = 0, setup = -1, spec = 0, passes = 0;
  bool operator==(const GraphKey &o) const {
    return count == o.count && lm == o.lm && ch == o.ch && sc == o.sc && sweep == o.sweep && linb_gx == o.linb_gx && offs == o.offs &&
           setup == o.setup && spec == o.spec && passes == o.passes;
  }
};

}

struct lfvio_ctx {
  int device = 0;
  hipStream_t stream = nullptr;
  char *d_feat = nullptr;
  size_t feat_bytes = 0;
  char *h_feat = nullptr;
  std::string err;
  int batch = 0;
  Layout L;
  char *d_base = nullptr;
  char *h_stage = nullptr;
  char *h_down = nullptr;
  size_t h_down_bytes = 0;
  std::vector<SlotHostInfo> info;
  std::vector<int> perm_build;
  hipGraphExec_t graph = nullptr;
  GraphKey graph_key;
  bool publish = false;
  hipGraphExec_t chunk[2] = {}, tail[2][3] = {};
  hipGraphExec_t first[2][2][4][13] = {};
  int fixed_passes = 0;
  int recent_passes[4] = {0, 0, 0, 0}, recent_head = 0;
  bool predicted_early = false;
  int predict_passes = 4;
  double pass_seconds = 2e-4;
  GraphKey chunk_key;
  int *d_pending = nullptr, *h_pending = nullptr;
  char *h_mail = nullptr, *d_mail = nullptr;
  hipStream_t fstream = nullptr;
  static constexpr int WORKERS = 2;
  hipStream_t sstream[WORKERS] = {};
  bool shadow = false;
  bool marg_ahead = true;
  hipGraphExec_t side[WORKERS][2][2] = {};
  int side_ticket = 0;
  bool side_launched = false;
  bool side_known = false;
  long long stat_ahead_calls = 0, stat_ahead_hits = 0;
  bool inflight = false;
  bool unsynced = false;
  hipEvent_t stage_event = nullptr;
  bool stage_busy = false;
  double up_us[4] = {0, 0, 0, 0};
  std::unique_ptr<LfvioPrior> held;
  bool has_held = false;
  int inflight_flag = 0;
  bool pipelined = false;
  int mail_seq = 0;
  std::unique_ptr<LfvioPrior> chain_struct;
  bool chain_err_told = false;
  char *d_relo = nullptr, *h_relo = nullptr;
  size_t relo_dev_cap = 0, relo_stage_cap = 0;
  int relo_done_word = 0;
  bool relo_force = false;
  bool debug_break_chain = false;
  bool inflight_first = false;
  bool use_graph = true;
  int stat_chunks = 0;
  int last_passes = 0;
  int last_iters = 0;
  bool fixed_spec = false;
  int spec_count = 3;
  int *d_lwt = nullptr;
  int *d_asm = nullptr;
  bool shard_group = false;
  int shard_kmax0 = -1;
  int lm_half = 1;
  int linw_mode = 1;
  double init_radius = 1e4;
  double fn_tol = 1e-6;
  bool force_eig = false;
  bool shard_active = false;
  int shard_begin = 0, shard_end = 0, shard_state = 0;
  std::vector<int> sh_start, sh_off;
  static constexpr int FLAG_RING = 4;
  int *h_flags = nullptr;
  hipEvent_t flag_event[FLAG_RING] = {};
  long long flag_head = 0, flag_tail = 0;
};

namespace {

void destroy_graph(lfvio_ctx *c, bool keep_side = false) {
  if (c->stream && (c->inflight || c->unsynced || c->pipelined)) {
    (void)hipStreamSynchronize(c->stream);
    c->unsynced = false, c->pipelined = false;
  }
  if (c->graph) {
    (void)hipGraphExecDestroy(c->graph);
    c->graph = nullptr;
  }
  if (!keep_side) {
    for (auto &st : c->sstream)
      if (st) (void)hipStreamSynchronize(st);
    for (auto &wk : c->side)
      for (auto &row : wk)
        for (auto &t : row)
          if (t) (void)hipGraphExecDestroy(t), t = nullptr;
  }
  for (auto &t : c->chunk)
    if (t) (void)hipGraphExecDestroy(t), t = nullptr;
  for (auto &row : c->tail)
    for (auto &t : row)
      if (t) (void)hipGraphExecDestroy(t), t = nullptr;
  for (auto &var : c->first)
    for (auto &plane : var)
      for (auto &row : plane)
        for (auto &t : row)
          if (t) (void)hipGraphExecDestroy(t), t = nullptr;
}

void predict(lfvio_ctx *c) {
  c->recent_passes[c->recent_head++ & 3] = c->last_passes;
  int m = 1;
  for (int k = 0; k < 4; k++) m = std::max(m, c->recent_passes[k]);
  c->predict_passes = m;
}
int wait_side(lfvio_ctx *c) {
  if (!c->side_launched) return LFVIO_OK;
  c->side_launched = false;
  int ts = 0;
  if (c->side_known) ts = c->h_pending[2];
  else HIPCHK(c, hipMemcpy(&ts, c->d_base + offsetof(Slot, tail_state), sizeof ts, hipMemcpyDeviceToHost));
  const int *echo = (const int *)c->h_mail + 7;
  if (ts == 3) {
    const auto t0 = std::chrono::steady_clock::now();
    while (__atomic_load_n(echo, __ATOMIC_ACQUIRE) != c->side_ticket) {
      if (std::chrono::duration<double>(std::chrono::steady_clock::now() - t0).count() > 2.0) {
        c->err = "the marginalization handed to a worker stream did not arrive";
        return LFVIO_ERR_DEVICE;
      }
    }
  }
  if (__atomic_load_n(echo, __ATOMIC_ACQUIRE) == c->side_ticket) c->stat_ahead_hits++;
  ((volatile int *)c->h_mail)[6] = 0;
  return LFVIO_OK;
}
constexpr const char *CHAIN_ERR_TEXT = "the prior this window was to take over on the device was not there (the marginalization before it produced none): it ran without a prior";
int join_inflight(lfvio_ctx *c, bool pipelined_ok = false) {
  if (c->pipelined && !c->inflight && pipelined_ok) return LFVIO_OK;
  if (c->unsynced || c->pipelined) {
    c->unsynced = false, c->pipelined = false;
    HIPCHK(c, hipStreamSynchronize(c->stream));
    if (!c->inflight)
      if (int rc = wait_side(c)) return rc;
  }
  if (!c->inflight) return LFVIO_OK;
  c->inflight = false;
  HIPCHK(c, hipStreamSynchronize(c->stream));
  const bool handed = c->side_launched && c->side_known && c->h_pending[2] == 3;
  if (int rc = wait_side(c)) return rc;
  if (c->inflight_first) {
    c->last_passes = std::max(c->h_pending[3], 1), c->last_iters = c->h_pending[4];
    if (!c->predicted_early) predict(c);
    c->predicted_early = false;
    if (c->h_pending[2] != 2 && !handed) {
      c->err = "the marginalization behind an early solution did not finish";
      return LFVIO_ERR_DEVICE;
    }
    const bool told = c->chain_err_told;
    c->chain_err_told = false;
    if (c->h_pending[5] && !told) {
      c->err = CHAIN_ERR_TEXT;
      return LFVIO_ERR_DEVICE;
    }
  }
  return LFVIO_OK;
}

bool wait_early(lfvio_ctx *c) {
  int *flag = (int *)c->h_mail;
  const int want = c->info[0].mail_seq;
  for (;;) {
    if (__atomic_load_n(flag, __ATOMIC_ACQUIRE) == want) return true;
    if (hipStreamQuery(c->stream) != hipErrorNotReady) return __atomic_load_n(flag, __ATOMIC_ACQUIRE) == want;
  }
}

constexpr int SHADOW_MAX_LM = 1024;
int reserve(lfvio_ctx *c, int batch, int maxN, int maxM) {
  if (c->d_base && batch <= c->batch && maxN <= c->L.maxN && maxM <= c->L.maxM) return LFVIO_OK;
  if (c->inflight) {
    if (!c->held) c->held.reset(new LfvioPrior);
    if (int rc = lfvio_batch_optimize_finish(c, c->held.get())) return rc;
    c->has_held = true;
  }
  if (int rc = join_inflight(c)) return rc;
  batch = std::max(batch, c->batch);
  maxN = std::max(maxN, c->L.maxN);
  maxM = std::max(maxM, c->L.maxM);
  destroy_graph(c);
// ... 525 lines not shown
  info.marg_n = std::max(S->marg[0].valid ? S->marg[0].n : 0, S->marg[1].valid ? S->marg[1].n : 0);
  info.linw_ok = linw;
  info.linb_ok = linb, info.linb_ng = linb_ng;
  if (slot == 0 && c->side_launched) hipLaunchKernelGGL(k_spec_wait, dim3(1), dim3(64), 0, c->stream, d);
  HIPCHK(c, hipMemcpyAsync(d, h, offsetof(Slot, x), hipMemcpyHostToDevice, c->stream));
  HIPCHK(c, hipMemcpyAsync(d + L.in_begin, h + L.in_begin, (lists_cached ? L.sum_off : L.sum_items + (size_t)used_items * 4) - L.in_begin, hipMemcpyHostToDevice,
                           c->stream));
  if (pr && !device_chain) HIPCHK(c, hipMemcpyAsync(d + L.prior_J, h + L.prior_J, sizeof(double) * pr->n * pr->n, hipMemcpyHostToDevice, c->stream));
  if (device_chain) {
    hipLaunchKernelGGL(k_prior_chain, dim3(1, 1), dim3(256), 0, c->stream, d, L.total);
    c->inflight = false, c->pipelined = true;
  }
  if (linw) HIPCHK(c, hipMemcpyAsync(d + L.linw_begin, h + L.linw_begin, L.pm_pair + (size_t)std::max(M - N, 0) - L.linw_begin, hipMemcpyHostToDevice, c->stream));
  if (linb) HIPCHK(c, hipMemcpyAsync(d + L.linb_lm0, h + L.linb_lm0, L.linw_end - L.linb_lm0, hipMemcpyHostToDevice, c->stream));
  info.list_items = used_items;
  if (!info.uploaded) {
    Slot W;
    std::memset(&W, 0, sizeof W);
    W.lam[0].set(&W, L.lam[0]), W.lam[1].set(&W, L.lam[1]);
    for (int k = 0; k < SPEC_EXTRA; k++) W.lamE[k].set(&W, L.lamE[k]);
    W.cost_partE.set(&W, L.cost_partE);
    W.prior_A.set(&W, L.prior_A);
    W.a.set(&W, L.a), W.b.set(&W, L.b), W.W.set(&W, L.W), W.Wt.set(&W, L.Wt);
    W.scale_l.set(&W, L.scale_l), W.grad_l.set(&W, L.grad_l), W.gn_l.set(&W, L.gn_l);
    W.diag_l.set(&W, L.diag_l), W.einv_l.set(&W, L.einv_l), W.d1.set(&W, L.d1), W.d2.set(&W, L.d2);
    W.gram_part.set(&W, L.gram_part), W.pairG.set(&W, L.pairG);
    W.schur_part.set(&W, L.schur_part);
    W.xch.set(&W, L.xch);
    W.schur_sum.set(&W, L.xch + (size_t)XOFF_S * 8), W.gp.set(&W, L.xch + (size_t)XOFF_G * 8), W.Hpp.set(&W, L.xch + (size_t)XOFF_H * 8);
    W.lm_part.set(&W, L.lm_part), W.cost_part.set(&W, L.cost_part), W.imu_out.set(&W, L.imu_out), W.imu_raw.set(&W, L.imu_raw);
    W.mscr.set(&W, L.mscr);
    W.eig_aux.set(&W, L.eig_aux);
#define PUTP(field) HIPCHK(c, hipMemcpyAsync(d + offsetof(Slot, field), &W.field, sizeof W.field, hipMemcpyHostToDevice, c->stream))
    PUTP(lam); PUTP(lamE); PUTP(cost_partE);
    PUTP(prior_A);
    PUTP(a); PUTP(b); PUTP(W); PUTP(Wt); PUTP(scale_l); PUTP(grad_l); PUTP(gn_l); PUTP(diag_l); PUTP(einv_l); PUTP(d1); PUTP(d2);
    PUTP(gram_part); PUTP(pairG); PUTP(schur_part); PUTP(schur_sum); PUTP(xch); PUTP(gp); PUTP(lm_part); PUTP(cost_part); PUTP(imu_out); PUTP(imu_raw);
    PUTP(Hpp);
    PUTP(mscr); PUTP(eig_aux);
#undef PUTP
    if (c->shadow && slot == 0) {
      GP<double> prior_A[lfvio_ctx::WORKERS];
      for (int wk = 0; wk < lfvio_ctx::WORKERS; wk++) {
        char *ds = c->d_base + (size_t)(c->batch + wk) * L.total;
#define PUTS(field) HIPCHK(c, hipMemcpyAsync(ds + offsetof(Slot, field), &W.field, sizeof W.field, hipMemcpyHostToDevice, c->stream))
        PUTS(lam); PUTS(lamE); PUTS(cost_partE);
        PUTS(a); PUTS(b); PUTS(W); PUTS(Wt); PUTS(scale_l); PUTS(grad_l); PUTS(gn_l); PUTS(diag_l); PUTS(einv_l); PUTS(d1); PUTS(d2);
        PUTS(gram_part); PUTS(pairG); PUTS(schur_part); PUTS(schur_sum); PUTS(xch); PUTS(gp); PUTS(lm_part); PUTS(cost_part); PUTS(imu_out); PUTS(imu_raw);
        PUTS(Hpp);
        PUTS(mscr); PUTS(eig_aux);
#undef PUTS
        prior_A[wk].off = W.prior_A.off - (long long)((size_t)(c->batch + wk) * L.total);
        HIPCHK(c, hipMemcpyAsync(ds + offsetof(Slot, prior_A), &prior_A[wk], sizeof prior_A[wk], hipMemcpyHostToDevice, c->stream));
      }
    }
    HIPCHK(c, hipStreamSynchronize(c->stream));
    info.uploaded = true;
  }
  if (linb) hipLaunchKernelGGL(k_linb_gather, dim3((std::max(N, M - N) + 255) / 256, 1), dim3(256), 0, c->stream, d, L.total);
  const auto t_up2 = lap(2, t_up1);
  if (!c->stage_event) HIPCHK(c, hipEventCreateWithFlags(&c->stage_event, hipEventDisableTiming));
  HIPCHK(c, hipEventRecord(c->stage_event, c->stream));
  c->stage_busy = true;
  lap(3, t_up2);
  info.resident = true;
  return LFVIO_OK;
}

struct CaptureGuard {
  hipStream_t stream;
  bool active = true;
  explicit CaptureGuard(hipStream_t s) : stream(s) {}
  hipError_t end(hipGraph_t *g) {
    active = false;
    return hipStreamEndCapture(stream, g);
  }
  ~CaptureGuard() {
    if (!active) return;
    hipGraph_t g = nullptr;
    (void)hipStreamEndCapture(stream, &g);
    if (g) (void)hipGraphDestroy(g);
  }
};

template <class F>
int capture_graph(lfvio_ctx *c, hipStream_t stream, hipGraphExec_t *out, F &&enqueue) {
  hipGraph_t graph;
  HIPCHK(c, hipStreamBeginCapture(stream, hipStreamCaptureModeThreadLocal));
  CaptureGuard guard(stream);
  if (int rc = enqueue()) return rc;
  HIPCHK(c, guard.end(&graph));
  HIPCHK(c, hipGraphInstantiate(out, graph, nullptr, nullptr, 0));
  HIPCHK(c, hipGraphDestroy(graph));
  return LFVIO_OK;
}

constexpr int CH_BUCKET = 16;

Grid grid_for(lfvio_ctx *c, int count) {
  Grid g{1, 1, 1, 1, 1};
  for (int s = 0; s < count; s++) {
    g.ch_raw = std::max(g.ch_raw, c->info[s].gCh);
    g.lm = std::max(g.lm, c->info[s].gLm);
    g.lw = std::max(g.lw, c->info[s].gLw);
    g.ch = std::max(g.ch, c->info[s].gCh);
    g.sc = std::max(g.sc, c->info[s].gSc);
  }
  g.ch = (g.ch + CH_BUCKET - 1) / CH_BUCKET * CH_BUCKET;
  return g;
}

int slots_offs(const lfvio_ctx *c, int count) {
  int r = 0;
  for (int k = 0; k < count; k++) r |= (c->info[k].offs_first ? 1 : 0) | (c->info[k].offs_all ? 2 : 0);
  return r;
}

SetupLaunch setup_launch(lfvio_ctx *c, int count, int lm, bool zero_wt) {
  bool compact = count >= 8;
  for (int s = 0; compact && s < count; s++) compact = c->info[s].prior_n <= SETUP_TILED_MAXN;
  return {(compact ? 3 : SETUP_WGS) + (lm + 3) / 4, (zero_wt ? 1 : 0) | (compact ? 4 : 0)};
}

Route route_for(lfvio_ctx *c, int count, int mode) {
  Route r;
  r.count = count;
  r.g = grid_for(c, count);
  r.role_wgs = (size_t)count * (r.g.lw + (r.g.ch + 3) / 4 + LFVIO_WINDOW_SIZE + 1);
  r.split = count >= LIN_SPLIT_MIN_BATCH && r.role_wgs > LIN_SPLIT_WGS;
  bool linw = true, linb = count > 0;
  int ng = 0;
  for (int s = 0; s < count; s++) {
    linw = linw && c->info[s].linw_ok, linb = linb && c->info[s].linb_ok;
    ng = std::max(ng, c->info[s].linb_ng);
  }
  const bool solve = mode == MODE_SOLVE;
  const bool marg_sweep = (mode & (MODE_GATED - 1)) >= MODE_MARG && !(mode & (MODE_DECIDE | MODE_NOCOUNT));
  if (c->linw_mode != 0 && !c->shard_active && linw && (solve || marg_sweep) && (c->linw_mode == 2 || r.split)) r.sweep = Route::LINW;
  else if (c->linw_mode != 0 && solve && linb && (!c->shard_active || count == 1)) r.sweep = Route::LINB;
  else r.sweep = Route::ROLES;
  r.linb_gx = r.sweep == Route::LINB ? (ng + 1 + 63) / 64 * 64 : 0;
  r.setup = setup_launch(c, count, r.g.lm, r.sweep == Route::LINW);
  r.offs = slots_offs(c, count);
  return r;
}

GraphKey graph_key(const Route &r, int spec, int passes, bool with_setup) {
  GraphKey k;
  k.count = r.count, k.lm = r.g.lm, k.ch = r.g.ch, k.sc = r.g.sc, k.sweep = r.sweep, k.linb_gx = r.linb_gx, k.offs = r.offs;
  k.setup = with_setup ? r.setup.bits : 0, k.spec = spec, k.passes = passes;
  return k;
}

void launch_setup(lfvio_ctx *c, const Route &r, int mode) {
  hipLaunchKernelGGL(k_setup, dim3(r.setup.gx, r.count), dim3(256), 0, c->stream, c->d_base, c->L.total, mode, r.setup.bits);
}

template <class F>
void with_offs(bool offs, F &&launch) {
  if (offs) launch(std::true_type());
  else launch(std::false_type());
}

void launch_lin(lfvio_ctx *c, const Route &r, int mode, bool offs) {
  const int count = r.count, lw = r.g.lw, gram_wgs = (r.g.ch + 3) / 4;
  const size_t st = c->L.total;
  with_offs(offs, [&](auto o) {
    if (!r.split) {
      hipLaunchKernelGGL((k_lin<LIN_ROLE_ALL, decltype(o)::value>), dim3(lw + gram_wgs + LFVIO_WINDOW_SIZE + 1, count), dim3(LIN_THREADS), 0, c->stream, c->d_base, st,
                         mode, lw, gram_wgs);
      return;
    }
    hipLaunchKernelGGL((k_lin<LIN_ROLE_LM, decltype(o)::value>), dim3(lw, count), dim3(LIN_THREADS), 0, c->stream, c->d_base, st, mode, lw, 0);
    hipLaunchKernelGGL((k_lin<LIN_ROLE_GRAM, decltype(o)::value>), dim3(gram_wgs, count), dim3(LIN_THREADS), 0, c->stream, c->d_base, st, mode | MODE_NOCOUNT, 0, gram_wgs);
  });
  if (!r.split) return;
  const bool raw = (mode & (MODE_GATED - 1)) == MODE_SOLVE && !(mode & (MODE_GATED | MODE_DECIDE));
  if (raw) hipLaunchKernelGGL(k_imu_raw, dim3((count * LFVIO_WINDOW_SIZE + 63) / 64), dim3(64), 0, c->stream, c->d_base, st, count);
  if (raw) hipLaunchKernelGGL((k_lin<LIN_ROLE_POSE_RAW, false>), dim3(LFVIO_WINDOW_SIZE + 1, count), dim3(LIN_THREADS), 0, c->stream, c->d_base, st, mode | MODE_NOCOUNT, 0, 0);
  else hipLaunchKernelGGL((k_lin<LIN_ROLE_POSE, false>), dim3(LFVIO_WINDOW_SIZE + 1, count), dim3(LIN_THREADS), 0, c->stream, c->d_base, st, mode | MODE_NOCOUNT, 0, 0);
}

void launch_sum(lfvio_ctx *c, const Route &r, int mode) {
  const int count = r.count;
  const Grid &g = r.g;
  const size_t st = c->L.total;
  const int pre = (g.ch_raw > PRE_CHUNK_LIMIT || g.sc > 4 * PRE_GROUP) ? 1 : 0;
  const int groups = (g.sc + PRE_GROUP - 1) / PRE_GROUP;
  if (pre) hipLaunchKernelGGL(k_presum, dim3(NPAIR + (SCHUR_LEN / 256) * groups + 1, count), dim3(256), 0, c->stream, c->d_base, st, mode, groups);
  const Layout &L = c->L;
  const SumArgs sa{(long long)L.sum_off, (long long)L.sum_end_marg, (long long)L.sum_items, (long long)L.gram_part, (long long)L.pairG, (long long)L.imu_out,
                   (long long)L.prior_A};
  hipLaunchKernelGGL(k_sum, dim3(HPP_BLOCKS + SCHUR_LEN / 256 + 1, count), dim3(256), 0, c->stream, c->d_base, st, mode, pre, sa);
}

LinwArgs linw_args(const lfvio_ctx *c) {
  const Layout &L = c->L;
  LinwArgs a;
  a.anc0 = (long long)L.anc[0], a.anc_stride = (long long)(L.anc[1] - L.anc[0]);
  a.pmo0 = (long long)L.pmo[0], a.pmo_stride = (long long)(L.pmo[1] - L.pmo[0]);
  a.Wt = (long long)L.Wt, a.lam[0] = (long long)L.lam[0], a.lam[1] = (long long)L.lam[1];
  a.a = (long long)L.a, a.b = (long long)L.b, a.scale_l = (long long)L.scale_l, a.diag_l = (long long)L.diag_l, a.grad_l = (long long)L.grad_l;
  a.einv_l = (long long)L.einv_l, a.imu_out = (long long)L.imu_out;
  a.Hpp = (long long)(L.xch + (size_t)XOFF_H * 8), a.gp = (long long)(L.xch + (size_t)XOFF_G * 8), a.schur_sum = (long long)(L.xch + (size_t)XOFF_S * 8);
  a.part = (long long)L.schur_part, a.wt_ld = L.capLmBlocks * LM_BLOCK;
  a.asm_tab = c->d_lwt;
  return a;
}

void launch_sweep(lfvio_ctx *c, const Route &r, int mode, bool offs, bool decide = false) {
  if (r.sweep == Route::ROLES) {
    launch_lin(c, r, mode | (decide ? MODE_DECIDE : 0), offs);
    launch_sum(c, r, mode);
    return;
  }
  const size_t st = c->L.total;
  with_offs(offs, [&](auto o) {
    if (r.sweep == Route::LINW)
      hipLaunchKernelGGL(k_linw<decltype(o)::value>, dim3(1, r.count), dim3(LW_THREADS), LW_LDS_BYTES, c->stream, c->d_base, st, linw_args(c), mode);
    else
      hipLaunchKernelGGL(k_linb<decltype(o)::value>, dim3(r.linb_gx, r.count), dim3(LW_THREADS), LW_LDS_BYTES, c->stream, c->d_base, st, linw_args(c));
  });
  if (r.sweep == Route::LINB) hipLaunchKernelGGL(k_sumb, dim3(LINB_SUM_GRID, r.count), dim3(LINB_SUM_THREADS), 0, c->stream, c->d_base, st, linw_args(c));
}

void launch_solve(lfvio_ctx *c, int count, bool lw = false) {
  const size_t st = c->L.total;
  const long long xo = (long long)c->L.xch, io = (long long)c->L.imu_out, po = (long long)c->L.prior_A;
  if (lw)
    hipLaunchKernelGGL(k_solve_dense<true>, dim3(1, count), dim3(SOLVE_THREADS), SOLVE_LDS, c->stream, c->d_base, st, xo, io, po, (const int *)c->d_asm);
  else
    hipLaunchKernelGGL(k_solve_dense<false>, dim3(1, count), dim3(SOLVE_THREADS), SOLVE_LDS, c->stream, c->d_base, st, xo, io, po, (const int *)nullptr);
}

bool launch_iteration(lfvio_ctx *c, const Route &r, int mode, bool speculate = false, bool first = true, bool last = true, bool gauge = false, bool offs = true) {
  const int count = r.count;
  const Grid &g = r.g;
  const size_t st = c->L.total;
  const bool solve = (mode & (MODE_GATED - 1)) == MODE_SOLVE && !(mode & MODE_GATED);
  const bool lw = r.sweep == Route::LINW, lb = r.sweep == Route::LINB;
  const bool merge = solve && !lw && g.lm <= DOGLEG_INLINE_BLOCKS && r.role_wgs <= LIN_SPLIT_WGS;
  launch_sweep(c, r, mode, offs, merge && !first);
  if ((mode & (MODE_GATED - 1)) == MODE_SOLVE) {
    launch_solve(c, count, lw);
    const bool inl = g.lm <= DOGLEG_INLINE_BLOCKS;
    const int spec = speculate && inl ? c->spec_count : 1;
    const int nb = g.lm + LFVIO_WINDOW_SIZE + 1;
    const bool split = r.split || lw;
    const bool fuse = inl && !split && !c->shard_active && (size_t)count * nb <= 2048;
    const bool stepw = lw && inl && spec == 1;
    if (stepw) {
      hipLaunchKernelGGL(k_stepw, dim3(1, count), dim3(STEPW_LAUNCH_THREADS), 0, c->stream, c->d_base, st);
      return false;
    }
    if (!inl && lb) hipLaunchKernelGGL(k_backsub_wt, dim3(g.lm, count), dim3(64), 0, c->stream, c->d_base, st, c->L.capLmBlocks * LM_BLOCK);
    else if (!inl) hipLaunchKernelGGL(k_backsub, dim3(g.lm, count), dim3(64), 0, c->stream, c->d_base, st);
    if (fuse) hipLaunchKernelGGL(k_step, dim3(spec * nb, count), dim3(DOGLEG_INLINE_THREADS), 0, c->stream, c->d_base, st, g.lm, spec);
    else {
      if (inl && (!split || lw)) hipLaunchKernelGGL((k_dogleg<true, true>), dim3(spec, count), dim3(DOGLEG_INLINE_THREADS), 0, c->stream, c->d_base, st, spec);
      else if (inl) hipLaunchKernelGGL((k_dogleg<true, false>), dim3(spec, count), dim3(DOGLEG_INLINE_THREADS), 0, c->stream, c->d_base, st, spec);
      else hipLaunchKernelGGL(k_dogleg<false>, dim3(spec, count), dim3(128), 0, c->stream, c->d_base, st, spec);
    }
    if (fuse) {
    } else if ((size_t)count * nb <= 2048)
      hipLaunchKernelGGL(k_cost<4>, dim3(spec * nb, count), dim3(256), 0, c->stream, c->d_base, st, g.lm, spec);
    else if (spec == 1 && !c->shard_active) {
      hipLaunchKernelGGL((k_cost<1, false>), dim3(g.lm + 1, count), dim3(64), 0, c->stream, c->d_base, st, g.lm, 1);
      hipLaunchKernelGGL(k_cost_imu, dim3((count * LFVIO_WINDOW_SIZE + 63) / 64), dim3(64), 0, c->stream, c->d_base, st, count);
    } else
      hipLaunchKernelGGL(k_cost<1>, dim3(spec * nb, count), dim3(64), 0, c->stream, c->d_base, st, g.lm, spec);
    if (merge && last && gauge) {
      hipLaunchKernelGGL(k_decide_gauge, dim3(1, count), dim3(128), 0, c->stream, c->d_base, st, c->publish ? 1 : 0);
      return true;
    }
    if (!merge || last) hipLaunchKernelGGL(k_decide, dim3(1, count), dim3(64), 0, c->stream, c->d_base, st);
  }
  return false;
}

__global__ void k_pending(char *base, size_t stride, int count, int *out, int tail) {
  int n = 0, used = 0;
  for (int s = threadIdx.x; s < count; s += 64) {
    const Slot *S = (const Slot *)(base + (size_t)s * stride);
    n += (tail ? S->tail_state == 2 : S->tr.done != 0) ? 0 : 1;
    used = max(used, S->passes_used);
  }
  used = __reduce_max_sync(~0ull, used);
  if (threadIdx.x == 0) out[1] = used;
  n = __reduce_add_sync(~0ull, n);
  if (threadIdx.x == 0) *out = n;
}

__global__ void k_force_done(char *base, size_t stride, int count) {
  const int s = blockIdx.x * blockDim.x + threadIdx.x;
  if (s < count) {
    Slot *S = (Slot *)(base + (size_t)s * stride);
    if (!S->tr.done) S->tr.done = 1;
    if (S->spec_on && S->tail_state == 0) spec_closing(S);
  }
}

constexpr int SOLVE_CHUNK = 2, MAX_FIRST_PASSES = 12;
constexpr int SIDE_ROUNDS = 4;
int enqueue_marg(lfvio_ctx *c, int count, int flag, bool standalone, bool gated = false);
int enqueue_solve(lfvio_ctx *c, int count, int max_iter, bool adaptive, int fused_flag = -1, bool *tail_done = nullptr,
                  double max_seconds = -1.0, bool early = false) {
  if (int rc = join_inflight(c, early)) return rc;
  const Route r = route_for(c, count, MODE_SOLVE);
  const Grid &g = r.g;
  const int passes = std::max(max_iter, 0) + 4;
  if (adaptive && c->use_graph) {
    const bool speculate = (size_t)count * (g.lm + LFVIO_WINDOW_SIZE + 1) <= 512;
    if (speculate && !c->fixed_spec) c->spec_count = (c->last_iters > 0 && c->last_iters >= 2 * c->last_passes) ? std::min(4, 1 + SPEC_EXTRA) : 3;
    if (!c->d_pending) {
      HIPCHK(c, hipMalloc((void **)&c->d_pending, 256));
      HIPCHK(c, hipHostMalloc((void **)&c->h_pending, 256, hipHostMallocDefault));
    }
    const int offs = r.offs;
    const GraphKey key = graph_key(r, (int)speculate, 0, true);
    if (!(c->chunk_key == key)) {
      destroy_graph(c, c->chunk_key.count == count && ((c->chunk_key.offs ^ offs) & 2) == 0);
      c->chunk_key = key;
    }
    if (tail_done) *tail_done = false;
    const bool fuse = fused_flag >= 0 && fused_flag < 2;
    const bool capped = max_seconds > 0.0;
    const auto t_start = std::chrono::steady_clock::now();
    int first_passes = std::min(std::max(c->fixed_passes > 0 ? c->fixed_passes : c->predict_passes, 1), std::min(passes, MAX_FIRST_PASSES));
    if (capped) first_passes = std::max(std::min(SOLVE_CHUNK, passes), std::min(first_passes, (int)std::min(max_seconds / c->pass_seconds, 1e6)));
    const int sv = speculate && c->spec_count > 3 ? 1 : 0;
    hipGraphExec_t &first_graph = c->first[sv][c->publish ? 1 : 0][fuse ? 1 + fused_flag : 0][first_passes];
    auto capture = [&](hipGraphExec_t *out, bool setup, int npass, int tail_flag) {
      return capture_graph(c, c->stream, out, [&]() -> int {
        if (setup) launch_setup(c, r, MODE_SOLVE);
        bool gauged = false;
        for (int it = 0; it < npass; it++)
          gauged = launch_iteration(c, r, MODE_SOLVE, speculate, it == 0, it == npass - 1, tail_flag >= 0, (offs & 2) || (setup && it == 0 && (offs & 1)));
        if (tail_flag >= 0) {
          if (!gauged) {
            hipLaunchKernelGGL(k_gauge, dim3(1 + (g.lm + 1) / 2, count), dim3(128), 0, c->stream, c->d_base, c->L.total, 1);
            if (c->publish) hipLaunchKernelGGL(k_publish, dim3(1), dim3(256), 0, c->stream, c->d_base, c->L.total);
          }
          if (int rc = enqueue_marg(c, count, tail_flag, false, true)) return rc;
        }
        if (tail_flag >= 0 && count == 1) {
          HIPCHK(c, hipMemcpyAsync(c->h_pending + 2, c->d_base + offsetof(Slot, tail_state), 4 * sizeof(int), hipMemcpyDeviceToHost, c->stream));
        } else {
          hipLaunchKernelGGL(k_pending, dim3(1), dim3(64), 0, c->stream, c->d_base, c->L.total, count, c->d_pending, tail_flag >= 0 ? 1 : 0);
          HIPCHK(c, hipMemcpyAsync(c->h_pending, c->d_pending, 2 * sizeof(int), hipMemcpyDeviceToHost, c->stream));
        }
        return LFVIO_OK;
      });
    };
    if (!first_graph) {
      const int rc = capture(&first_graph, true, first_passes, fuse ? fused_flag : -1);
      if (rc) return rc;
    }
    if (!c->chunk[sv]) {
      const int rc = capture(&c->chunk[sv], false, SOLVE_CHUNK, -1);
      if (rc) return rc;
    }
    const bool ahead = fuse && count == 1 && c->info[0].spec_on && c->shadow && c->marg_ahead  && !c->shard_active && !c->pipelined &&
                       g.lm <= DOGLEG_INLINE_BLOCKS && g.ch_raw <= PRE_CHUNK_LIMIT && g.sc <= 4 * PRE_GROUP && r.sweep == Route::ROLES;
    for (int wk = 0; ahead && wk < lfvio_ctx::WORKERS; wk++) {
      hipGraphExec_t *side_graph = &c->side[wk][fused_flag][c->publish ? 1 : 0];
      if (*side_graph) continue;
      hipStream_t ss = c->sstream[wk];
      const size_t back = (size_t)(c->batch + wk) * c->L.total;
      char *sh = c->d_base + back;
      const Layout &L = c->L;
      const int mode = (MODE_MARG + fused_flag) | MODE_GATED, gram_wgs = (L.capChunks + 3) / 4, lw_cap = 2 * DOGLEG_INLINE_BLOCKS;
      const SumArgs sa{(long long)L.sum_off - (long long)back, (long long)L.sum_end_marg - (long long)back, (long long)L.sum_items - (long long)back,
                       (long long)L.gram_part, (long long)L.pairG, (long long)L.imu_out, (long long)L.prior_A - (long long)back};
      const int rc = capture_graph(c, ss, side_graph, [&]() -> int {
        for (int rd = 0; rd < SIDE_ROUNDS; rd++) {
          hipLaunchKernelGGL(k_spec_begin, dim3(1), dim3(128), 0, ss, sh, back);
          with_offs(offs & 2, [&](auto o) {
            hipLaunchKernelGGL((k_lin<LIN_ROLE_ALL, decltype(o)::value>), dim3(lw_cap + gram_wgs + LFVIO_WINDOW_SIZE + 1, 1), dim3(LIN_THREADS), 0, ss, sh, back, mode,
                               lw_cap, gram_wgs);
          });
          hipLaunchKernelGGL(k_sum, dim3(HPP_BLOCKS + SCHUR_LEN / 256 + 1, 1), dim3(256), 0, ss, sh, back, mode, 0, sa);
          hipLaunchKernelGGL(k_marg_solve<true>, dim3(1, 1), dim3(MARG_THREADS), MARG_LDS, ss, sh, back,
                             fused_flag | (c->force_eig ? 256 : 0) | 512 | (c->publish ? 1024 : 0));
        }
        return LFVIO_OK;
      });
      if (rc) return rc;
    }
    c->side_launched = false, c->side_known = false;
    c->stat_chunks = 0;
    for (int done_passes = 0; done_passes < passes;) {
      c->stat_chunks++;
      const auto t_launch = std::chrono::steady_clock::now();
      const bool watch = early && done_passes == 0 && fuse && c->publish;
      if (watch) __atomic_store_n((int *)c->h_mail + 1, 0, __ATOMIC_RELAXED), __atomic_store_n((int *)c->h_mail, 0, __ATOMIC_RELEASE);
      if (done_passes == 0 && c->h_mail && count == 1) ((volatile int *)c->h_mail)[6] = ahead ? (c->side_ticket = (c->side_ticket == 0x7fffffff ? 1 : c->side_ticket + 1)) : 0;
      HIPCHK(c, hipGraphLaunch(done_passes == 0 ? first_graph : c->chunk[sv], c->stream));
      if (ahead && done_passes == 0) {
        for (int wk = 0; wk < lfvio_ctx::WORKERS; wk++) HIPCHK(c, hipGraphLaunch(c->side[wk][fused_flag][c->publish ? 1 : 0], c->sstream[wk]));
        c->side_launched = true, c->stat_ahead_calls++;
      }
      if (c->pipelined && done_passes == 0) c->up_us[1] = std::chrono::duration<double>(std::chrono::steady_clock::now() - t_launch).count() * 1e6;
      if (watch && wait_early(c)) {
        c->inflight = true, c->inflight_first = true;
        c->side_known = c->side_launched;
        if (tail_done) *tail_done = true;
        return LFVIO_OK;
      }
      HIPCHK(c, hipStreamSynchronize(c->stream));
      const bool first = done_passes == 0;
      if (!first) {
        const double dt = std::chrono::duration<double>(std::chrono::steady_clock::now() - t_launch).count() / SOLVE_CHUNK;
        c->pass_seconds = 0.75 * c->pass_seconds + 0.25 * dt;
      }
      done_passes += first ? first_passes : SOLVE_CHUNK;
      if (first && fuse && count == 1) c->h_pending[0] = c->h_pending[2] >= 2 ? 0 : 1, c->h_pending[1] = c->h_pending[3], c->last_iters = c->h_pending[4];
      if (first && fuse && count == 1 && c->h_pending[0] == 0) c->side_known = c->side_launched;
      if (first && fuse && count == 1 && c->h_pending[5]) {
        c->err = CHAIN_ERR_TEXT;
        return LFVIO_ERR_DEVICE;
      }
      if (c->h_pending[0] == 0) {
        if (tail_done && fuse && first) *tail_done = true;
        break;
      }
      if (capped && std::chrono::duration<double>(std::chrono::steady_clock::now() - t_start).count() >= max_seconds) {
        hipLaunchKernelGGL(k_force_done, dim3((count + 63) / 64), dim3(64), 0, c->stream, c->d_base, c->L.total, count);
        HIPCHK(c, hipStreamSynchronize(c->stream));
        break;
      }
    }
    c->last_passes = std::max(c->h_pending[1], 1);
    predict(c);
    HIPCHK(c, hipGetLastError());
    if (tail_done && *tail_done)
      if (int rc = wait_side(c)) return rc;
    return LFVIO_OK;
  }
  launch_setup(c, r, MODE_SOLVE);
  auto loop = [&]() {
    for (int it = 0; it < passes; it++) launch_iteration(c, r, MODE_SOLVE, false, it == 0, it == passes - 1, false, (r.offs & 2) || (it == 0 && (r.offs & 1)));
    return LFVIO_OK;
  };
  if (c->use_graph) {
    const GraphKey key = graph_key(r, 0, passes, false);
    if (!c->graph || !(c->graph_key == key)) {
      if (c->graph) (void)hipGraphExecDestroy(c->graph), c->graph = nullptr;
      if (int rc = capture_graph(c, c->stream, &c->graph, loop)) return rc;
      c->graph_key = key;
    }
    HIPCHK(c, hipGraphLaunch(c->graph, c->stream));
  } else {
    loop();
  }
  HIPCHK(c, hipGetLastError());
  return LFVIO_OK;
}

int enqueue_marg(lfvio_ctx *c, int count, int flag, bool standalone, bool gated) {
  if (int rc = join_inflight(c, gated)) return rc;
  const int mode = (MODE_MARG + flag) | (gated ? MODE_GATED : 0);
  const Route r = route_for(c, count, mode);
  if (standalone) launch_setup(c, r, mode);
  launch_iteration(c, r, mode, false, true, true, false, standalone ? r.offs != 0 : (r.offs & 2) != 0);
  hipLaunchKernelGGL(k_marg_solve<false>, dim3(1, count), dim3(MARG_THREADS), MARG_LDS, c->stream, c->d_base, c->L.total,
                     flag | (c->force_eig ? 256 : 0) | (gated ? 512 : 0) | (gated && c->publish ? 1024 : 0));
  HIPCHK(c, hipGetLastError());
  return LFVIO_OK;
}

constexpr int ONE_TRIP_LM = 8192;
struct Fetched {
  const FrameState *xs;
  const TRState *tr;
  const double *lam[2];
  LfvioPrior *prior;
};

int fetch(lfvio_ctx *c, int slot, bool want_sol, bool want_prior, Fetched *f) {
  if (int rc = join_inflight(c)) return rc;
  const Layout &L = c->L;
  char *d = c->d_base + (size_t)slot * L.total;
  const SlotHostInfo &info = c->info[slot];
  if (!info.resident) {
    c->err = "slot not uploaded";
    return LFVIO_ERR_ARG;
  }
  char *hd = c->h_down;
  const size_t hdr = sizeof(FrameState) * 2 + sizeof(TRState), lam_bytes = (size_t)info.N * 8;
  char *h_lam0 = hd + hdr, *h_lam1 = h_lam0 + align_up(lam_bytes + 8, 64), *h_prior = h_lam1 + align_up(lam_bytes + 8, 64);
// ... 522 lines not shown
  return ref > 0 ? LFVIO_OK : LFVIO_ERR_ARG;
}

int lfvio_debug_marg_system(lfvio_ctx *c, int n, double *A, double *b) {
  if (!c || !c->d_base) return LFVIO_ERR_ARG;
  (void)hipSetDevice(c->device);
  if (int rc = join_inflight(c)) return rc;
  if (n < 0 || n > 76) return LFVIO_ERR_ARG;
  if (n == 0) return LFVIO_OK;
  char *d = c->d_base + c->L.mscr;
  if (c->shadow) {
    const size_t head = offsetof(LfvioPrior, linearized_jacobians), bytes = head + sizeof(double) * n * n;
    std::vector<char> p0(bytes), pw(bytes);
    HIPCHK(c, hipMemcpy(p0.data(), c->d_base + offsetof(Slot, prior_out), bytes, hipMemcpyDeviceToHost));
    const LfvioPrior *h0 = (const LfvioPrior *)p0.data();
    for (int wk = 0; wk < lfvio_ctx::WORKERS && h0->valid == 1 && h0->n == n; wk++) {
      char *ds = c->d_base + (size_t)(c->batch + wk) * c->L.total;
      HIPCHK(c, hipMemcpy(pw.data(), ds + offsetof(Slot, prior_out), bytes, hipMemcpyDeviceToHost));
      const LfvioPrior *hw = (const LfvioPrior *)pw.data();
      if (hw->valid == 1 && hw->n == n && std::memcmp(p0.data() + head, pw.data() + head, bytes - head) == 0) {
        d = ds + c->L.mscr;
        break;
      }
    }
  }
  HIPCHK(c, hipMemcpy(A, d + sizeof(double) * (92 * 92 + 96), sizeof(double) * n * n, hipMemcpyDeviceToHost));
  HIPCHK(c, hipMemcpy(b, d + sizeof(double) * (92 * 92 + 96 + n * n), sizeof(double) * n, hipMemcpyDeviceToHost));
  return LFVIO_OK;
}

int lfvio_debug_read_clocks(lfvio_ctx *c, long long *out32) {
  if (!c || !c->d_base) return LFVIO_ERR_ARG;
  if (int rc = join_inflight(c)) return rc;
  HIPCHK(c, hipMemcpy(out32, c->d_base + offsetof(Slot, dbg), sizeof(long long) * 32, hipMemcpyDeviceToHost));
  HIPCHK(c, hipMemcpy(out32 + 32, c->d_base + offsetof(Slot, jtrace), sizeof(double) * 32, hipMemcpyDeviceToHost));
  return LFVIO_OK;
}

int lfvio_debug_time_kernel(lfvio_ctx *c, int which, int count, int reps, double *avg_ms) {
  if (!c || !c->d_base || count <= 0 || count > c->batch || reps <= 0) return LFVIO_ERR_ARG;
  (void)hipSetDevice(c->device);
  if (int rc = join_inflight(c)) return rc;
  const Route r = route_for(c, count, MODE_SOLVE);
  const Grid &g = r.g;
  const size_t st = c->L.total;
  const bool lw = r.sweep == Route::LINW, lb = r.sweep == Route::LINB;
  const bool offs = (r.offs & 2) != 0;
  if ((which == 11 || which == 12) && !lw) {
    c->err = "the resident windows are not linearized by k_linw";
    return LFVIO_ERR_ARG;
  }
  if (which >= 15 && which <= 17 && !lb) {
    c->err = "the resident window is not linearized by k_linb";
    return LFVIO_ERR_ARG;
  }
  hipEvent_t e0, e1;
  HIPCHK(c, hipEventCreate(&e0));
  if (hipError_t e = hipEventCreate(&e1); e != hipSuccess) {
    (void)hipEventDestroy(e0);
    HIPCHK(c, e);
  }
  launch_setup(c, r, MODE_SOLVE);
  Route full = r;
  if (lb && !(which >= 15 && which <= 17)) full.sweep = Route::ROLES;
  launch_sweep(c, full, MODE_SOLVE, offs);
  if (which == 14) launch_solve(c, count, lw);
  if (which == 17) launch_solve(c, count, false);

  HIPCHK(c, hipEventRecord(e0, c->stream));
  for (int rep = 0; rep < reps; rep++) {
    switch (which) {
      case 0: launch_lin(c, r, MODE_SOLVE, offs); break;
      case 2: launch_sum(c, r, MODE_SOLVE); break;
      case 8: case 9: case 10: case 18: {
        const int gram_wgs = (g.ch + 3) / 4;
        const int gx = which == 8 ? g.lw : which == 9 ? gram_wgs : which == 18 ? LFVIO_WINDOW_SIZE : LFVIO_WINDOW_SIZE + 1;
        hipLaunchKernelGGL((k_lin<LIN_ROLE_ALL, false>), dim3(gx, count), dim3(LIN_THREADS), 0, c->stream, c->d_base, st, MODE_SOLVE, which == 8 ? g.lw : 0,
                           which == 9 ? gram_wgs : 0);
      } break;
      case 4: case 5: case 6: case 7: {
        const SetupLaunch sl = setup_launch(c, count, g.lm, false);
        const int wgs = (sl.bits & 4) ? 3 : SETUP_WGS, gx = which == 4 ? 1 : which == 5 ? 2 : which == 6 ? wgs : sl.gx;
        hipLaunchKernelGGL(k_setup, dim3(gx, count), dim3(256), 0, c->stream, c->d_base, st, MODE_SOLVE, sl.bits);
      } break;
      case 11: case 12: launch_sweep(c, r, MODE_SOLVE, offs); break;
      case 13: launch_solve(c, count, lw); break;
      case 14: hipLaunchKernelGGL(k_stepw, dim3(1, count), dim3(STEPW_LAUNCH_THREADS), 0, c->stream, c->d_base, st); break;
      case 15: hipLaunchKernelGGL(k_linb<false>, dim3(r.linb_gx, count), dim3(LW_THREADS), LW_LDS_BYTES, c->stream, c->d_base, st, linw_args(c)); break;
      case 16: hipLaunchKernelGGL(k_sumb, dim3(LINB_SUM_GRID, count), dim3(LINB_SUM_THREADS), 0, c->stream, c->d_base, st, linw_args(c)); break;
      case 17: hipLaunchKernelGGL(k_backsub_wt, dim3(g.lm, count), dim3(64), 0, c->stream, c->d_base, st, c->L.capLmBlocks * LM_BLOCK); break;
      default: launch_solve(c, count); break;
    }
  }
  HIPCHK(c, hipEventRecord(e1, c->stream));
  HIPCHK(c, hipEventSynchronize(e1));
  float ms = 0;
  HIPCHK(c, hipEventElapsedTime(&ms, e0, e1));
  *avg_ms = (double)ms / reps;
  (void)hipEventDestroy(e0);
  (void)hipEventDestroy(e1);
  return LFVIO_OK;
}

static int sweep_kernel_of(lfvio_ctx *c, int count) {
  return !c || !c->d_base || count <= 0 || count > c->batch ? LFVIO_ERR_ARG : route_for(c, count, MODE_SOLVE).sweep;
}

int lfvio_debug_resident_pass(lfvio_ctx *c, int count, int slot, double *gp, double *schur, double *lm_sum, double *a, double *b, double *gn_p, double *q,
                              double *x_cost) {
  if (!c || !c->d_base || count <= 0 || count > c->batch || slot < 0 || slot >= count) return LFVIO_ERR_ARG;
  (void)hipSetDevice(c->device);
  if (int rc = join_inflight(c)) return rc;
  for (int s = 0; s < count; s++)
    if (!c->info[s].resident) return LFVIO_ERR_ARG;
  const size_t st = c->L.total;
  const Route r = route_for(c, count, MODE_SOLVE);
  launch_setup(c, r, MODE_SOLVE);
  launch_sweep(c, r, MODE_SOLVE, true);
  launch_solve(c, count, r.sweep == Route::LINW);
  HIPCHK(c, hipGetLastError());
  HIPCHK(c, hipStreamSynchronize(c->stream));
  const char *d = c->d_base + (size_t)slot * st;
  const int N = c->info[slot].N;
  auto get = [&](double *dst, size_t off, size_t n) { return !dst || !n ? hipSuccess : hipMemcpy(dst, d + off, n * 8, hipMemcpyDeviceToHost); };
  HIPCHK(c, get(gp, c->L.xch + (size_t)XOFF_G * 8, KP));
  HIPCHK(c, get(schur, c->L.xch + (size_t)XOFF_S * 8, SCHUR_LEN));
  HIPCHK(c, get(lm_sum, offsetof(Slot, lm_sum), 5));
  HIPCHK(c, get(a, c->L.a, N));
  HIPCHK(c, get(b, c->L.b, N));
  HIPCHK(c, get(gn_p, offsetof(Slot, gn_p), KP));
  HIPCHK(c, get(q, offsetof(Slot, tr) + offsetof(TRState, q), Q_COUNT));
  HIPCHK(c, get(x_cost, offsetof(Slot, tr) + offsetof(TRState, x_cost), 1));
  return r.sweep;
}

int lfvio_debug_configure(lfvio_ctx *c, const char *key, double value) {
  if (!c || !key) return LFVIO_ERR_ARG;
  const std::string k = key;
  const int iv = (int)value;
  if (k == "env") {
    const char *e = getenv("LFVIO_DEBUG");
    if (!e) return LFVIO_OK;
    std::string all = e;
    for (size_t p = 0; p < all.size();) {
      const size_t q = std::min(all.find(',', p), all.size()), eq = all.find('=', p);
      if (eq != std::string::npos && eq < q) {
        const int rc = lfvio_debug_configure(c, all.substr(p, eq - p).c_str(), atof(all.substr(eq + 1, q - eq - 1).c_str()));
        if (rc) return rc;
      }
      p = q + 1;
    }
    return LFVIO_OK;
  }
  const bool structural = k == "graph" || k == "linw" || k == "force_eig";
  if (structural) {
    if (int rc = join_inflight(c)) return rc;
  }
  if (k == "graph") c->use_graph = iv != 0;
  else if (k == "first_passes") {
    if (iv < 0) return LFVIO_ERR_ARG;
    c->fixed_passes = iv;
  } else if (k == "spec_count") c->fixed_spec = iv > 0, c->spec_count = iv > 0 ? std::max(1, std::min(1 + SPEC_EXTRA, iv)) : 3;
  else if (k == "function_tolerance") {
    if (!(value >= 0.0)) return LFVIO_ERR_ARG;
    c->fn_tol = value;
  } else if (k == "initial_radius") c->init_radius = value > 0.0 ? value : 1e4;
  else if (k == "linw") {
    if (iv < 0 || iv > 2) return LFVIO_ERR_ARG;
    c->linw_mode = iv;
  } else if (k == "lm_half") c->lm_half = iv != 0;
  else if (k == "force_eig") c->force_eig = iv != 0;
  else if (k == "marg_ahead") c->marg_ahead = iv != 0;
  else if (k == "break_next_chain") c->debug_break_chain = iv != 0;
  else if (k == "relo_route") c->relo_force = iv != 0;
  else {
    c->err = "lfvio_debug_configure: unknown key '" + k + "'";
    return LFVIO_ERR_ARG;
  }
  if (structural) destroy_graph(c);
  return LFVIO_OK;
}

int lfvio_debug_query(lfvio_ctx *c, const char *key, double *out, int n) {
  if (!c || !key || !out || n <= 0) return LFVIO_ERR_ARG;
  const std::string k = key;
  auto put = [&](std::initializer_list<double> v) {
    int i = 0;
    for (double x : v)
      if (i < n) out[i++] = x;
    return LFVIO_OK;
  };
  if (k == "last_call") return put({(double)c->last_passes, (double)c->last_iters, (double)c->stat_chunks, (double)c->spec_count});
  if (k == "marg_ahead") return put({(double)c->stat_ahead_calls, (double)c->stat_ahead_hits});
  if (k == "upload_times") return put({c->up_us[0], c->up_us[1], c->up_us[2], c->up_us[3]});
  if (k == "sweep_kernel") {
    const int r = sweep_kernel_of(c, (int)out[0]);
    if (r < 0) return r;
    return put({(double)r});
  }
  c->err = "lfvio_debug_query: unknown key '" + k + "'";
  return LFVIO_ERR_ARG;
}

#include "relo.inc"
#include "feat.inc"

#include "twoview.inc"

#include "vialign.inc"

#include "pnp.inc"
#include "shard.inc"
#include "group.inc"

}
```

lf-vio_amd/lfvio/engine.py:

```python
import ctypes as C

import numpy as np

from . import abi

_dp = C.POINTER(C.c_double)


def _p(a):
    return a.ctypes.data_as(_dp)


class Engine:
    def __init__(self, device=0, lib_path=None):
        self.lib = abi.load_hip_library(lib_path)
        self.lib.lfvio_debug_linearize.argtypes = [C.c_void_p, C.POINTER(abi.WindowC), _dp, _dp, _dp, _dp, _dp, _dp]
        self.lib.lfvio_debug_marg_system.argtypes = [C.c_void_p, C.c_int, _dp, _dp]
        self.lib.lfvio_debug_configure.argtypes = [C.c_void_p, C.c_char_p, C.c_double]
        self.lib.lfvio_debug_query.argtypes = [C.c_void_p, C.c_char_p, _dp, C.c_int]
        self.lib.lfvio_debug_time_kernel.argtypes = [C.c_void_p, C.c_int, C.c_int, C.c_int, _dp]
        self.ctx = self.lib.lfvio_create(device)
        if not self.ctx:
            raise RuntimeError("lfvio_create failed: no usable HIP device (there is no CPU fallback)")

    def close(self):
        if self.ctx:
            self.lib.lfvio_destroy(self.ctx)
            self.ctx = None

    def __del__(self):
        try:
            self.close()
        except Exception:
            pass

    def _check(self, rc, what):
        if rc != 0:
            raise RuntimeError(f"{what} failed rc={rc}: {self.lib.lfvio_last_error(self.ctx).decode()}")

    def configure(self, key, value=1.0):
        self._check(self.lib.lfvio_debug_configure(self.ctx, key.encode(), float(value)), f"lfvio_debug_configure({key})")

    def query(self, key, n, first=0.0):
        out = np.zeros(max(n, 1))
        out[0] = first
        self._check(self.lib.lfvio_debug_query(self.ctx, key.encode(), _p(out), n), f"lfvio_debug_query({key})")
        return out

    def set_graph(self, on):
        self.configure("graph", int(on))

    def marg_ahead(self, on=-1):
        if on >= 0:
            self.configure("marg_ahead", int(on))
        q = self.query("marg_ahead", 2)
        return int(q[0]), int(q[1])

    def break_next_chain(self):
        self.configure("break_next_chain", 1)

    def set_lm_half(self, on):
        self.configure("lm_half", int(on))

    def set_initial_radius(self, r):
        self.configure("initial_radius", float(r))

    def set_linw(self, mode):
        self.configure("linw", int(mode))

    def resident_pass(self, count, slot, n_landmarks):
        out = dict(gp=np.zeros(abi.KP), schur=np.zeros(15 * 256), lm_sum=np.zeros(5), a=np.zeros(max(n_landmarks, 1)),
                   b=np.zeros(max(n_landmarks, 1)), gn_p=np.zeros(abi.KP), q=np.zeros(16), x_cost=np.zeros(1))
        dp = C.POINTER(C.c_double)
        self.lib.lfvio_debug_resident_pass.argtypes = [C.c_void_p, C.c_int, C.c_int] + [dp] * 8
        rc = self.lib.lfvio_debug_resident_pass(self.ctx, count, slot, *[_p(out[k]) for k in ("gp", "schur", "lm_sum", "a", "b", "gn_p", "q", "x_cost")])
        if rc < 0:
            self._check(rc, "resident_pass")
        out["a"], out["b"], out["linw"] = out["a"][:n_landmarks], out["b"][:n_landmarks], rc
        return out

    def set_function_tolerance(self, tol):
        self.configure("function_tolerance", float(tol))

    def last_chunks(self):
        return int(self.query("last_call", 4)[2])

    def last_passes(self):
        return int(self.query("last_call", 4)[0])

    def force_eig(self, on):
        self.configure("force_eig", int(on))

    def solve(self, win):
        sol = abi.Solution(win.N)
        self._check(self.lib.lfvio_solve(self.ctx, C.byref(win.c()), C.byref(sol.c)), "lfvio_solve")
        return sol

    def solve_relo(self, win, frame, relo_pose, landmark=(), match_point=()):
        relo = abi.Relo(frame, relo_pose, landmark, match_point)
        rc_ = relo.c()
        sol = abi.Solution(win.N)
        out = np.zeros(abi.SIZE_POSE)
        self._check(self.lib.lfvio_solve_relo(self.ctx, C.byref(win.c()), C.byref(rc_), C.byref(sol.c), _p(out)), "lfvio_solve_relo")
        return sol, out

    def solve_relo_rc(self, win, relo, sol, out, num_matches=None, null_arrays=False):
        rc_ = relo.c(num_matches=num_matches, null_arrays=null_arrays)
        return int(self.lib.lfvio_solve_relo(self.ctx, C.byref(win.c()), C.byref(rc_), C.byref(sol.c), _p(out)))

    def marginalize(self, win, flag):
        prior = abi.Prior()
        self._check(self.lib.lfvio_marginalize(self.ctx, C.byref(win.c()), flag, C.byref(prior)), "lfvio_marginalize")
        return prior

    def schur_repeat(self, win, mu):
        d = np.zeros(1)
        self.lib.lfvio_debug_schur_repeat.argtypes = [C.c_void_p, C.POINTER(abi.WindowC), C.c_double, _dp]
        self._check(self.lib.lfvio_debug_schur_repeat(self.ctx, C.byref(win.c()), float(mu), _p(d)), "lfvio_debug_schur_repeat")
        return float(d[0])

    def marg_system(self, n):
        A = np.zeros((n, n))
        b = np.zeros(n)
        self._check(self.lib.lfvio_debug_marg_system(self.ctx, n, _p(A), _p(b)), "lfvio_debug_marg_system")
        return A, b

    def linearize(self, win):
        N = win.N
        H = np.zeros((abi.KP, abi.KP))
        g = np.zeros(abi.KP)
        a, b = np.zeros(max(N, 1)), np.zeros(max(N, 1))
        W = np.zeros((max(N, 1), abi.KC))
        cost = np.zeros(1)
        self._check(self.lib.lfvio_debug_linearize(self.ctx, C.byref(win.c()), _p(H), _p(g), _p(a), _p(b), _p(W),
                                                   _p(cost)), "lfvio_debug_linearize")
        return dict(H=H, g=g, a=a[:N], b=b[:N], W=W[:N], cost=float(cost[0]))

    def batch_reserve(self, batch, max_landmarks, max_observations):
        self._check(self.lib.lfvio_batch_reserve(self.ctx, batch, max_landmarks, max_observations), "batch_reserve")

    def batch_upload(self, slot, win, marshalled=None):
        self._check(self.lib.lfvio_batch_upload(self.ctx, slot, C.byref(marshalled if marshalled is not None else win.c())), "batch_upload")

    def batch_upload_chained(self, slot, win, prior, marshalled=None):
        self._check(self.lib.lfvio_batch_upload_chained(self.ctx, slot, C.byref(marshalled if marshalled is not None else win.c()), C.byref(prior)),
                    "batch_upload_chained")

    def set_first_passes(self, n):
        self.configure("first_passes", int(n))

    def batch_upload_chained_device(self, slot, win, marshalled=None):
        self._check(self.lib.lfvio_batch_upload_chained_device(self.ctx, slot, C.byref(marshalled if marshalled is not None else win.c())),
                    "batch_upload_chained_device")

    def batch_optimize(self, count, flag, sync=True):
        fn = self.lib.lfvio_batch_optimize if sync else self.lib.lfvio_batch_optimize_async
        self._check(fn(self.ctx, count, flag), "batch_optimize")

    def batch_sync(self):
        self._check(self.lib.lfvio_batch_sync(self.ctx), "batch_sync")

    def batch_download(self, slot, n_landmarks, want_prior=True, out=None):
        sol = out[0] if out is not None else abi.Solution(n_landmarks)
        prior = (out[1] if out is not None else abi.Prior()) if want_prior else None
        self._check(self.lib.lfvio_batch_download(self.ctx, slot, C.byref(sol.c), C.byref(prior) if want_prior else None),
                    "batch_download")
        return sol, prior

    def optimize_begin(self, flag, n_landmarks, out=None):
        sol = out if out is not None else abi.Solution(n_landmarks)
        self._check(self.lib.lfvio_batch_optimize_begin(self.ctx, flag, C.byref(sol.c)), "batch_optimize_begin")
        return sol

    def optimize_pending(self):
        return bool(self.lib.lfvio_batch_optimize_pending(self.ctx))

    def optimize_finish(self, want_prior=True, out=None):
        prior = (out if out is not None else abi.Prior()) if want_prior else None
        self._check(self.lib.lfvio_batch_optimize_finish(self.ctx, C.byref(prior) if want_prior else None), "batch_optimize_finish")
        return prior

    def optimize(self, win, flag):
        self.batch_reserve(1, win.N, win.M)
        self.batch_upload(0, win)
        self.batch_optimize(1, flag)
        return self.batch_download(0, win.N)

    def triangulate(self, tin, depth):
        d = np.ascontiguousarray(depth, dtype=np.float64).copy()
        self._check(self.lib.lfvio_triangulate(self.ctx, C.byref(tin.c), _p(d)), "lfvio_triangulate")
        return d

    def shift_depth(self, uv_i, marg_R, marg_P, new_R, new_P, init_depth, depth):
        uv = np.ascontiguousarray(uv_i, dtype=np.float64).reshape(-1, 3)
        d = np.ascontiguousarray(depth, dtype=np.float64).copy()
        a = [np.ascontiguousarray(x, dtype=np.float64).reshape(-1) for x in (marg_R, marg_P, new_R, new_P)]
        self._check(self.lib.lfvio_shift_depth(self.ctx, len(d), _p(uv), _p(a[0]), _p(a[1]), _p(a[2]), _p(a[3]), float(init_depth), _p(d)),
                    "lfvio_shift_depth")
        return d

    def preintegrate(self, intervals, noise):
        K = len(intervals)
        arr = (abi.ImuIntervalC * max(K, 1))()
        keep = []
        f = lambda a: np.ascontiguousarray(a, dtype=np.float64)
        for k, (ba, bg, a0, g0, dts, accs, gyrs) in enumerate(intervals):
            dts, accs, gyrs = f(dts).reshape(-1), f(accs).reshape(-1, 3), f(gyrs).reshape(-1, 3)
            keep.append((dts, accs, gyrs))
            arr[k].num_samples = len(dts)
# ... 270 lines not shown
```

Measured before the change: 2407 solves/s.

## Fold IMU info-root and prior normal equations into first lin sweep; direct spec prior writes

Adds a setup-head mode in which k_setup only runs the state copy, table build and landmark init. The IMU covariance square-root factorisation moves into the first k_lin pass's IMU role, and the prior J^T J product moves into extra k_lin workgroups, which shortens the serial setup kernel on the critical path. Separately, the speculative marginalization worker can write its prior directly into slot 0's prior_out instead of copying it afterwards. The header copy in the marginalization path is batched eight words per thread and reuses copy_rounds for the IMU sqrt copy. Risks include ordering hazards between the fused prior and IMU work and the consumers in the same pass, plus extra workgroups and register pressure in k_lin.

Result: no change. 2405 solves/s (median of 3 runs) (-0.1%).

```diff
diff --git a/lf-vio_amd/csrc/kernels_lin.h b/lf-vio_amd/csrc/kernels_lin.h
--- a/lf-vio_amd/csrc/kernels_lin.h
+++ b/lf-vio_amd/csrc/kernels_lin.h
@@ -11,22 +11,136 @@
 constexpr int MODE_GATED = 16;
 constexpr int MODE_DECIDE = 64;
 constexpr int MODE_NOCOUNT = 32;
+constexpr int MODE_SETUP_TAIL = 128;
 DEV bool tail_gate(const Slot *S, int done) { return done && S->tail_state == 0; }
 DEV bool is_marg(int mode) { return mode >= MODE_MARG; }
 DEV const MargPlan *marg_plan(const Slot *S, int mode) { return &S->marg[mode - MODE_MARG]; }
 
 DEV int gidx20(int p, int q) { return p * 20 - (p * (p - 1)) / 2 + (q - p); }
 
+DEV bool imu_info_root(Slot *S, int f, int l, bool store, double *T) {
+  const double *cov = S->imu[f].covariance;
+  double m0[15], m1[15];
+#pragma unroll
+  for (int r = 0; r < 15; r++) {
+    m0[r] = l < 15 ? cov[r * 15 + l] : (r == 0 ? 1.0 : 0.0);
+    m1[r] = r == l + 1 ? 1.0 : 0.0;
+  }
+#pragma unroll
+  for (int k = 0; k < 15; k++) {
+    int p = k;
+    double best = -1.0, piv = 0.0;
+#pragma unroll
+    for (int r = 0; r < 15; r++) {
+      const double v = fabs(m0[r]);
+      if (r >= k && v > best) best = v, p = r, piv = m0[r];
+    }
+    p = row_bcast_ik(p, k), piv = row_bcast_k(piv, k);
+    double csr[15];
+#pragma unroll
+    for (int r = 0; r < 15; r++) csr[r] = row_bcast_k(m0[r], k);
+    const double ck = csr[k];
+#pragma unroll
+    for (int r = 0; r < 15; r++) csr[r] = r == p ? ck : csr[r];
+    auto step = [&](double(&m)[15]) {
+      double Mp = m[0];
+#pragma unroll
+      for (int r = 1; r < 15; r++) Mp = p == r ? m[r] : Mp;
+      const double Mk = m[k], mk = Mp / piv;
+#pragma unroll
+      for (int r = 0; r < 15; r++) {
+        const double Msr = r == p ? Mk : m[r];
+        m[r] = r == k ? mk : Msr - csr[r] * mk;
+      }
+    };
+    step(m0), step(m1);
+  }
+#pragma unroll
+  for (int r = 0; r < 15; r++) {
+    if (l == 15) T[r * 16] = m0[r];
+    else if (l < 14) T[r * 16 + l + 1] = m1[r];
+  }
+  __builtin_amdgcn_fence(__ATOMIC_ACQ_REL, "wavefront");
+  const int li = l < 15 ? l : 0;
+  double lrow[15], mrow[15];
+#pragma unroll
+  for (int j = 0; j < 15; j++) mrow[j] = T[li * 16 + j], lrow[j] = 0.0;
+  bool ok = true;
+#pragma unroll
+  for (int j = 0; j < 15; j++) {
+    double t = mrow[j];
+#pragma unroll
+    for (int k = 0; k < j; k++) t -= lrow[k] * row_bcast_k(lrow[k], j);
+    const double sj = row_bcast_k(t, j);
+    if (!(sj > 0.0)) ok = false;
+    const double d = sqrt(sj);
+    lrow[j] = l == j ? d : t / d;
+  }
+  if (store && l < 15) {
+#pragma unroll
+    for (int i = 0; i < 15; i++) S->imu_sqrt[f][i * 15 + l] = (l >= i && ok) ? lrow[i] : 0.0;
+  }
+  return ok;
+}
+
+constexpr int SETUP_PRIOR_SLAB = 2048;
+constexpr int PRIOR_EPT = 8;
+DEV void prior_normal_part(Slot *S, int part, int np, double *Js) {
+  const int tid = threadIdx.x, n = S->prior_n;
+  constexpr int PRIOR_SLAB = SETUP_PRIOR_SLAB;
+  const double *J = S->prior_J;
+  const int rows_per = PRIOR_SLAB / n;
+  double acc[PRIOR_EPT], accb = 0;
+#pragma unroll
+  for (int q = 0; q < PRIOR_EPT; q++) acc[q] = 0;
+  for (int k0 = 0; k0 < n; k0 += rows_per) {
+    const int nk = min(rows_per, n - k0);
+    __syncthreads();
+    {
+      static_assert(PRIOR_SLAB <= 8 * 256, "eight elements of a slab per thread");
+      double v[8];
+      const double *Jk = J + k0 * n;
+#pragma unroll
+      for (int q = 0; q < 8; q++) v[q] = Jk[tid + 256 * q < nk * n ? tid + 256 * q : 0];
+      const double rv = S->prior_r[k0 + (tid < nk ? tid : 0)];
+#pragma unroll
+      for (int q = 0; q < 8; q++)
+        if (tid + 256 * q < nk * n) Js[tid + 256 * q] = v[q];
+      if (tid < nk) Js[PRIOR_SLAB + tid] = rv;
+    }
+    __syncthreads();
+#pragma unroll
+    for (int q = 0; q < PRIOR_EPT; q++) {
+      const int e = part * 256 + tid + q * 256 * np;
+      if (e < n * n) {
+        const int r = e / n, c = e % n;
+        double s = acc[q];
+        for (int k = 0; k < nk; k++) s = fma(Js[k * n + r], Js[k * n + c], s);
+        acc[q] = s;
+      }
+    }
+    if (part == 0 && tid < n)
+      for (int k = 0; k < nk; k++) accb = fma(Js[k * n + tid], Js[PRIOR_SLAB + k], accb);
+  }
+#pragma unroll
+  for (int q = 0; q < PRIOR_EPT; q++) {
+    const int e = part * 256 + tid + q * 256 * np;
+    if (e < n * n) S->prior_A[e] = acc[q];
+  }
+  if (part == 0 && tid < n) S->prior_b0[tid] = accb;
+}
+
+constexpr int SETUP_HEAD = 8;
 constexpr int SETUP_PRIOR_WGS = 16;
 constexpr int SETUP_WGS = 2 + SETUP_PRIOR_WGS;
 constexpr int SETUP_TILED_MAXN = 88;
 __global__ __launch_bounds__(256, 4) void k_setup(char *base, size_t stride, int mode, int zero_wt) {
   Slot *S = SLOT(base, stride);
   const int tid = threadIdx.x;
-  constexpr int SETUP_PRIOR_SLAB = 2048, SETUP_LDS = LFVIO_WINDOW_SIZE * 15 * 16;
+  constexpr int SETUP_LDS = LFVIO_WINDOW_SIZE * 15 * 16;
   static_assert(SETUP_LDS >= SETUP_PRIOR_SLAB + LFVIO_MAX_PRIOR_DIM && SETUP_LDS >= 84 + TAB_SCRATCH, "k_setup's workspace");
   __shared__ double sh_setup[SETUP_LDS];
-  const int setup_wgs = (zero_wt & 4) ? 3 : SETUP_WGS;
+  const int setup_wgs = (zero_wt & SETUP_HEAD) ? 1 : (zero_wt & 4) ? 3 : SETUP_WGS;
   if (blockIdx.x == 0) {
     const double *src = (const double *)&S->x0;
     double *dst = (double *)&S->x[0];
@@ -46,73 +160,12 @@
     const unsigned offm = build_tab(bt, &S->tab[0], tid, bt + 84);
     if (tid == 0) S->ex_fixed_off = ((offm >> TAB_EX_BIT) & 1u) && !S->est_ex;
     if (tid == 0 && S->spec_on) spec_arm(S);
-  } else if (blockIdx.x == 1) {
+  } else if (blockIdx.x == 1 && setup_wgs > 1) {
     if (tid >= 16 * ((LFVIO_WINDOW_SIZE + 3) & ~3)) return;
     const int grp = tid >> 4, l = tid & 15;
     const int f = grp < LFVIO_WINDOW_SIZE ? grp : 0;
     const bool mine = grp < LFVIO_WINDOW_SIZE && S->imu_active[f];
-    const double *cov = S->imu[f].covariance;
-    double m0[15], m1[15];
-#pragma unroll
-    for (int r = 0; r < 15; r++) {
-      m0[r] = l < 15 ? cov[r * 15 + l] : (r == 0 ? 1.0 : 0.0);
-      m1[r] = r == l + 1 ? 1.0 : 0.0;
-    }
-#pragma unroll
-    for (int k = 0; k < 15; k++) {
-      int p = k;
-      double best = -1.0, piv = 0.0;
-#pragma unroll
-      for (int r = 0; r < 15; r++) {
-        const double v = fabs(m0[r]);
-        if (r >= k && v > best) best = v, p = r, piv = m0[r];
-      }
-      p = row_bcast_ik(p, k), piv = row_bcast_k(piv, k);
-      double csr[15];
-#pragma unroll
-      for (int r = 0; r < 15; r++) csr[r] = row_bcast_k(m0[r], k);
-      const double ck = csr[k];
-#pragma unroll
-      for (int r = 0; r < 15; r++) csr[r] = r == p ? ck : csr[r];
-      auto step = [&](double(&m)[15]) {
-        double Mp = m[0];
-#pragma unroll
-        for (int r = 1; r < 15; r++) Mp = p == r ? m[r] : Mp;
-        const double Mk = m[k], mk = Mp / piv;
-#pragma unroll
-        for (int r = 0; r < 15; r++) {
-          const double Msr = r == p ? Mk : m[r];
-          m[r] = r == k ? mk : Msr - csr[r] * mk;
-        }
-      };
-      step(m0), step(m1);
-    }
-    double *T = sh_setup + f * (15 * 16);
-#pragma unroll
-    for (int r = 0; r < 15; r++) {
-      if (l == 15) T[r * 16] = m0[r];
-      else if (l < 14) T[r * 16 + l + 1] = m1[r];
-    }
-    __syncthreads();
-    const int li = l < 15 ? l : 0;
-    double lrow[15], mrow[15];
-#pragma unroll
-    for (int j = 0; j < 15; j++) mrow[j] = T[li * 16 + j], lrow[j] = 0.0;
-    bool ok = true;
-#pragma unroll
-    for (int j = 0; j < 15; j++) {
-      double t = mrow[j];
-#pragma unroll
-      for (int k = 0; k < j; k++) t -= lrow[k] * row_bcast_k(lrow[k], j);
-      const double sj = row_bcast_k(t, j);
-      if (!(sj > 0.0)) ok = false;
-      const double d = sqrt(sj);
-      lrow[j] = l == j ? d : t / d;
-    }
-    if (mine && l < 15) {
-#pragma unroll
-      for (int i = 0; i < 15; i++) S->imu_sqrt[f][i * 15 + l] = (l >= i && ok) ? lrow[i] : 0.0;
-    }
+    const bool ok = imu_info_root(S, f, l, mine, sh_setup + f * (15 * 16));
     if (mine && !ok && l == 0) S->imu_active[f] = 0;
   } else if (blockIdx.x >= setup_wgs) {
     const int l = (blockIdx.x - setup_wgs) * 256 + tid;
@@ -126,7 +179,6 @@
     if (!S->prior_valid) return;
     const int n = S->prior_n;
     const int part = blockIdx.x - 2;
-    constexpr int PRIOR_EPT = 8;
     const int nb4 = (n + 3) >> 2, tiles = nb4 * (nb4 + 1) / 2;
     static_assert(((SETUP_TILED_MAXN + 3) / 4) * ((SETUP_TILED_MAXN + 3) / 4 + 1) / 2 <= 256, "a thread per 4 x 4 block of the upper triangle");
     if (zero_wt & 4) {
@@ -190,48 +242,7 @@
     }
     const int np = gridDim.y >= 8 ? min(SETUP_PRIOR_WGS, (n * n + 256 * PRIOR_EPT - 1) / (256 * PRIOR_EPT)) : SETUP_PRIOR_WGS;
     if (part >= np) return;
-    constexpr int PRIOR_SLAB = SETUP_PRIOR_SLAB;
-    double *Js = sh_setup;
-    const double *J = S->prior_J;
-    const int rows_per = PRIOR_SLAB / n;
-    double acc[PRIOR_EPT], accb = 0;
-#pragma unroll
-    for (int q = 0; q < PRIOR_EPT; q++) acc[q] = 0;
-    for (int k0 = 0; k0 < n; k0 += rows_per) {
-      const int nk = min(rows_per, n - k0);
-      __syncthreads();
-      {
-        static_assert(PRIOR_SLAB <= 8 * 256, "eight elements of a slab per thread");
-        double v[8];
-        const double *Jk = J + k0 * n;
-#pragma unroll
-        for (int q = 0; q < 8; q++) v[q] = Jk[tid + 256 * q < nk * n ? tid + 256 * q : 0];
-        const double rv = S->prior_r[k0 + (tid < nk ? tid : 0)];
-#pragma unroll
-        for (int q = 0; q < 8; q++)
-          if (tid + 256 * q < nk * n) Js[tid + 256 * q] = v[q];
-        if (tid < nk) Js[PRIOR_SLAB + tid] = rv;
-      }
-      __syncthreads();
-#pragma unroll
-      for (int q = 0; q < PRIOR_EPT; q++) {
-        const int e = part * 256 + tid + q * 256 * np;
-        if (e < n * n) {
-          const int r = e / n, c = e % n;
-          double s = acc[q];
-          for (int k = 0; k < nk; k++) s = fma(Js[k * n + r], Js[k * n + c], s);
-          acc[q] = s;
-        }
-      }
-      if (part == 0 && tid < n)
-        for (int k = 0; k < nk; k++) accb = fma(Js[k * n + tid], Js[PRIOR_SLAB + k], accb);
-    }
-#pragma unroll
-    for (int q = 0; q < PRIOR_EPT; q++) {
-      const int e = part * 256 + tid + q * 256 * np;
-      if (e < n * n) S->prior_A[e] = acc[q];
-    }
-    if (part == 0 && tid < n) S->prior_b0[tid] = accb;
+    prior_normal_part(S, part, np, sh_setup);
   }
 }
 
@@ -620,10 +631,11 @@
 }
 
 template <bool raw_ready>
-DEV void lin_imu_role(Slot *S, const LinView &lv, int f, int mode, double *lds) {
+DEV void lin_imu_role(Slot *S, const LinView &lv, int f, int mode, double *lds, bool root = false) {
   double(*Jr)[30] = (double(*)[30]) lds;
   double(*Jw)[31] = (double(*)[31])(lds + 450);
   double *rr = lds + 450 + 465, *rw = rr + 16;
+  int *root_ok = (int *)(rw + 15);
   const int tid = threadIdx.x;
   double *out = S->imu_out + (size_t)f * IMU_OUT;
   const bool active = S->imu_active[f] && (mode == MODE_SOLVE || (f == 0 && marg_plan(S, mode)->use_imu0)) &&
@@ -642,8 +654,17 @@
     __syncthreads();
     if (tid == 0) imu_raw_residual(&S->imu[f], S->g, x->pose[f], x->sb[f], x->pose[f + 1], x->sb[f + 1], rr);
     if (tid == 64) imu_raw_jacobian(&S->imu[f], S->g, x->pose[f], x->sb[f], x->pose[f + 1], x->sb[f + 1], &Jr[0][0]);
+    if (root && tid >= 128 && tid < 144) {
+      const bool ok = imu_info_root(S, f, tid - 128, true, &Jw[0][0]);
+      if (tid == 128) *root_ok = ok ? 1 : 0;
+    }
   }
   __syncthreads();
+  if (!raw_ready && root && !*root_ok) {
+    if (tid == 0) S->imu_active[f] = 0;
+    for (int e = tid; e < IMU_OUT; e += LIN_THREADS) out[e] = 0.0;
+    return;
+  }
   const double *Sq = S->imu_sqrt[f];
   if (tid < 15) {
     double s = 0;
@@ -786,7 +807,8 @@
           if (threadIdx.x == 0) spec_publish(S, num_succ, cur);
         }
       } else if (acc_z == 0 && owner && threadIdx.x == 0 && S->spec_on) spec_publish(S, num_succ, cur);
-    } else if (owner && threadIdx.x == 0 && mode == MODE_SOLVE && S->spec_on) spec_publish(S, num_succ, cur);
+    } else if (owner && threadIdx.x == 0 && mode == MODE_SOLVE && S->spec_on && !(mode_bits & MODE_SETUP_TAIL))
+      spec_publish(S, num_succ, cur);
     if (mode == MODE_SOLVE && owner && !done && threadIdx.x == 0) S->passes_used++;
     if (done | (!do_lin & !do_schur)) return;
   }
@@ -823,7 +845,12 @@
   if (ROLES & (LIN_ROLE_POSE | LIN_ROLE_POSE_RAW)) {
     if (b < LFVIO_WINDOW_SIZE) {
       if (ROLES & LIN_ROLE_POSE_RAW) lin_imu_role<true>(S, lv, b, mode, lds);
-      else lin_imu_role<false>(S, lv, b, mode, lds);
+      else lin_imu_role<false>(S, lv, b, mode, lds, ROLES == LIN_ROLE_ALL && (mode_bits & MODE_SETUP_TAIL));
+      return;
+    }
+    if (ROLES == LIN_ROLE_ALL && b > LFVIO_WINDOW_SIZE) {
+      static_assert(ROLES != LIN_ROLE_ALL || LIN_LDS >= SETUP_PRIOR_SLAB + LFVIO_MAX_PRIOR_DIM, "the slab of J0 in k_lin's workspace");
+      if ((mode_bits & MODE_SETUP_TAIL) && S->prior_valid && b - LFVIO_WINDOW_SIZE - 1 < SETUP_PRIOR_WGS) prior_normal_part(S, b - LFVIO_WINDOW_SIZE - 1, SETUP_PRIOR_WGS, lds);
       return;
     }
     lin_prior_role<ROLES == LIN_ROLE_ALL>(S, lv, mode, lds);
@@ -1044,6 +1071,7 @@
   const int mode = mode_bits & (MODE_GATED - 1);
   const int tid = threadIdx.x;
   int b = blockIdx.x;
+  if ((mode_bits & MODE_SETUP_TAIL) && b == 0 && tid == 0 && S->spec_on) spec_publish(S, S->tr.num_succ, S->tr.cur);
   if (S->sharded && mode == MODE_SOLVE && !(mode_bits & MODE_GATED)) {
     const TRFlags f0 = tr_flags(&S->tr);
     if (f0.done | (!f0.do_lin & !f0.do_schur)) {
diff --git a/lf-vio_amd/csrc/kernels_marg.h b/lf-vio_amd/csrc/kernels_marg.h
--- a/lf-vio_amd/csrc/kernels_marg.h
+++ b/lf-vio_amd/csrc/kernels_marg.h
@@ -264,10 +264,15 @@
       long long *dst = (long long *)S;
       constexpr int W0 = (int)(offsetof(Slot, lm_start) / 8), W1 = (int)(offsetof(Slot, x) / 8);
       static_assert(offsetof(Slot, lm_start) % 8 == 0 && offsetof(Slot, x) % 8 == 0, "header words");
-      for (int k = tid; k < W1; k += 128) dst[k] = src[k] - (k >= W0 ? (long long)back : 0ll);
-      const double *is = &S0->imu_sqrt[0][0];
-      double *id = &S->imu_sqrt[0][0];
-      for (int k = tid; k < LFVIO_WINDOW_SIZE * 225; k += 128) id[k] = is[k];
+      for (int k0 = tid; k0 < W1; k0 += 8 * 128) {
+        long long v[8];
+#pragma unroll
+        for (int q = 0; q < 8; q++) v[q] = src[k0 + 128 * q < W1 ? k0 + 128 * q : 0];
+#pragma unroll
+        for (int q = 0; q < 8; q++)
+          if (k0 + 128 * q < W1) dst[k0 + 128 * q] = v[q] - (k0 + 128 * q >= W0 ? (long long)back : 0ll);
+      }
+      copy_rounds(&S->imu_sqrt[0][0], &S0->imu_sqrt[0][0], LFVIO_WINDOW_SIZE * 225, tid, 128);
     }
     __syncthreads();
     {
@@ -831,6 +836,10 @@
     __syncthreads();
     ESTAMP(17);
     if (sp && *sp->flag) return true;
+    if (poller) {
+      const int f = spec_peek(&sp->S0->spec.fin);
+      if (spec_ep(f) == spec_ep(sp->my_word) && spec_fin_state(f) == FIN_SIDE && spec_fin_acc(f) == spec_acc(sp->my_word)) *sp->direct = 1;
+    }
     if (work) {
       const double g0 = pp[mec], g1 = pp[96 + mec];
       const int kt = g1 < g0 ? ((int *)ee2)[96 + mec] : ((int *)ee2)[mec];
@@ -884,6 +893,7 @@
     const int m = tid >> 3, l8 = tid & 7;
     const bool live = m < n;
     const int mm = live ? m : 0;
+    if (SPEC && *sp->direct) out = &const_cast<Slot *>(sp->S0)->prior_out;
     double zz[10];
     const double sc = fast_rsqrt(1.0 + nn2[mm] + nn2[96 + mm]);
 #pragma unroll
@@ -916,7 +926,7 @@
   return false;
 }
 
-DEV void spec_deliver(Slot *S, Slot *S0, int my_word, bool publish) {
+DEV void spec_deliver(Slot *S, Slot *S0, int my_word, bool publish, bool direct) {
   const int tid = threadIdx.x, nthr = blockDim.x;
   __shared__ int give;
   if (tid == 0) {
@@ -942,12 +952,15 @@
   }
   __syncthreads();
   if (!give) return;
-  const LfvioPrior *src = &S->prior_out;
-  LfvioPrior *dst = &S0->prior_out;
-  const int n = src->valid == 1 ? src->n : 0;
-  copy_rounds((long long *)dst, (const long long *)src, (int)(offsetof(LfvioPrior, linearized_jacobians) / 8), tid, nthr);
-  copy_rounds(dst->linearized_jacobians, src->linearized_jacobians, n * n, tid, nthr);
-  copy_rounds(dst->linearized_residuals, src->linearized_residuals, n, tid, nthr);
+  STAMP(S, 30);
+  if (!direct) {
+    const LfvioPrior *src = &S->prior_out;
+    LfvioPrior *dst = &S0->prior_out;
+    const int n = src->valid == 1 ? src->n : 0;
+    copy_rounds((long long *)dst, (const long long *)src, (int)(offsetof(LfvioPrior, linearized_jacobians) / 8), tid, nthr);
+    copy_rounds(dst->linearized_jacobians, src->linearized_jacobians, n * n, tid, nthr);
+    copy_rounds(dst->linearized_residuals, src->linearized_residuals, n, tid, nthr);
+  }
   __syncthreads();
   if (publish) publish_prior(S0);
   char *m = (char *)S0->mail;
@@ -955,6 +968,7 @@
     __threadfence_system();
     __hip_atomic_store(&S0->tail_state, 2, __ATOMIC_RELAXED, __HIP_MEMORY_SCOPE_AGENT);
     if (m) __hip_atomic_store((int *)m + 7, S->shadow.ticket, __ATOMIC_RELAXED, __HIP_MEMORY_SCOPE_SYSTEM);
+    S->dbg[25] += direct ? 1 : 0, S->dbg[31] = (long long)__builtin_readcyclecounter();
   }
 }
 
@@ -966,9 +980,9 @@
   constexpr bool worker = WORKER;
   Slot *S = worker ? (Slot *)base : SLOT(base, stride);
   Slot *S0 = worker ? (Slot *)(base - stride) : S;
-  __shared__ int spec_flag;
-  SpecPoll sp{S0, worker ? S->shadow.word : 0, &spec_flag, 0, 0};
-  if (threadIdx.x == 0) spec_flag = 0;
+  __shared__ int spec_flag, spec_direct;
+  SpecPoll sp{S0, worker ? S->shadow.word : 0, &spec_flag, &spec_direct, 0, 0};
+  if (threadIdx.x == 0) spec_flag = 0, spec_direct = 0;
   const bool poller = worker && threadIdx.x == MARG_THREADS - 1;
   TRState *tr = &S->tr;
   const MargPlan *mp = &S->marg[flag];
@@ -980,7 +994,7 @@
     if (tid == 0) out->valid = -1;
     if (worker) {
       __syncthreads();
-      spec_deliver(S, S0, sp.my_word, publish != 0);
+      spec_deliver(S, S0, sp.my_word, publish != 0, false);
       return;
     }
     if (gated && tid == 0) S->iters_done = tr->iteration, S->tail_state = 2;
@@ -1120,6 +1134,8 @@
   if (eig_tridiag<WORKER>(Ar, br, n, tid, RV, DMs, vec8, scr, (double *)cs, S->eig_aux, out, 1e-8, S->dbg, &sp)) return;
   if (tid == 0) S->dbg[24] = sw1;
   STAMP(S, 14);
+  const bool direct = worker && spec_direct;
+  if (direct) out = &S0->prior_out;
   const FrameState *x = &S->x[tr->cur];
   if (tid < mp->nb) {
     const int kind = mp->kind[tid], frame = mp->frame[tid];
@@ -1143,7 +1159,7 @@
   }
   if (worker) {
     __syncthreads();
-    spec_deliver(S, S0, sp.my_word, publish != 0);
+    spec_deliver(S, S0, sp.my_word, publish != 0, direct);
     return;
   }
   if (gated && publish) {
diff --git a/lf-vio_amd/csrc/kernels_spec.h b/lf-vio_amd/csrc/kernels_spec.h
--- a/lf-vio_amd/csrc/kernels_spec.h
+++ b/lf-vio_amd/csrc/kernels_spec.h
@@ -57,6 +57,7 @@
   const Slot *S0;
   int my_word;
   int *flag;
+  int *direct;
   int f, w;
 };
 DEV void spec_poll_issue(SpecPoll &p) {
diff --git a/lf-vio_amd/csrc/lfvio_hip.hip b/lf-vio_amd/csrc/lfvio_hip.hip
--- a/lf-vio_amd/csrc/lfvio_hip.hip
+++ b/lf-vio_amd/csrc/lfvio_hip.hip
@@ -207,11 +207,13 @@
   hipStream_t sstream[WORKERS] = {};
   bool shadow = false;
   bool marg_ahead = true;
+  bool setup_split = true;
   hipGraphExec_t side[WORKERS][2][2] = {};
   int side_ticket = 0;
   bool side_launched = false;
   bool side_known = false;
   long long stat_ahead_calls = 0, stat_ahead_hits = 0;
+  bool stat_setup_tail = false;
   bool inflight = false;
   bool unsynced = false;
   hipEvent_t stage_event = nullptr;
@@ -1043,8 +1045,14 @@
   return k;
 }
 
-void launch_setup(lfvio_ctx *c, const Route &r, int mode) {
-  hipLaunchKernelGGL(k_setup, dim3(r.setup.gx, r.count), dim3(256), 0, c->stream, c->d_base, c->L.total, mode, r.setup.bits);
+void launch_setup(lfvio_ctx *c, const Route &r, int mode, bool head = false) {
+  if (head) hipLaunchKernelGGL(k_setup, dim3(1 + (r.g.lm + 3) / 4, r.count), dim3(256), 0, c->stream, c->d_base, c->L.total, mode, r.setup.bits | SETUP_HEAD);
+  else hipLaunchKernelGGL(k_setup, dim3(r.setup.gx, r.count), dim3(256), 0, c->stream, c->d_base, c->L.total, mode, r.setup.bits);
+}
+
+bool setup_tail(const lfvio_ctx *c, const Route &r) {
+  return c->setup_split && r.count == 1 && r.sweep == Route::ROLES && !r.split && r.g.lm <= DOGLEG_INLINE_BLOCKS && r.role_wgs <= LIN_SPLIT_WGS &&
+         !c->shard_active && !(r.setup.bits & 4);
 }
 
 template <class F>
@@ -1058,7 +1066,8 @@
   const size_t st = c->L.total;
   with_offs(offs, [&](auto o) {
     if (!r.split) {
-      hipLaunchKernelGGL((k_lin<LIN_ROLE_ALL, decltype(o)::value>), dim3(lw + gram_wgs + LFVIO_WINDOW_SIZE + 1, count), dim3(LIN_THREADS), 0, c->stream, c->d_base, st,
+      const int tail_wgs = (mode & MODE_SETUP_TAIL) ? SETUP_PRIOR_WGS : 0;
+      hipLaunchKernelGGL((k_lin<LIN_ROLE_ALL, decltype(o)::value>), dim3(lw + gram_wgs + LFVIO_WINDOW_SIZE + 1 + tail_wgs, count), dim3(LIN_THREADS), 0, c->stream, c->d_base, st,
                          mode, lw, gram_wgs);
       return;
     }
@@ -1099,10 +1108,10 @@
   return a;
 }
 
-void launch_sweep(lfvio_ctx *c, const Route &r, int mode, bool offs, bool decide = false) {
+void launch_sweep(lfvio_ctx *c, const Route &r, int mode, bool offs, bool decide = false, bool tail = false) {
   if (r.sweep == Route::ROLES) {
-    launch_lin(c, r, mode | (decide ? MODE_DECIDE : 0), offs);
-    launch_sum(c, r, mode);
+    launch_lin(c, r, mode | (decide ? MODE_DECIDE : 0) | (tail ? MODE_SETUP_TAIL : 0), offs);
+    launch_sum(c, r, mode | (tail ? MODE_SETUP_TAIL : 0));
     return;
   }
   const size_t st = c->L.total;
@@ -1124,14 +1133,15 @@
     hipLaunchKernelGGL(k_solve_dense<false>, dim3(1, count), dim3(SOLVE_THREADS), SOLVE_LDS, c->stream, c->d_base, st, xo, io, po, (const int *)nullptr);
 }
 
-bool launch_iteration(lfvio_ctx *c, const Route &r, int mode, bool speculate = false, bool first = true, bool last = true, bool gauge = false, bool offs = true) {
+bool launch_iteration(lfvio_ctx *c, const Route &r, int mode, bool speculate = false, bool first = true, bool last = true, bool gauge = false, bool offs = true,
+                      bool tail = false) {
   const int count = r.count;
   const Grid &g = r.g;
   const size_t st = c->L.total;
   const bool solve = (mode & (MODE_GATED - 1)) == MODE_SOLVE && !(mode & MODE_GATED);
   const bool lw = r.sweep == Route::LINW, lb = r.sweep == Route::LINB;
   const bool merge = solve && !lw && g.lm <= DOGLEG_INLINE_BLOCKS && r.role_wgs <= LIN_SPLIT_WGS;
-  launch_sweep(c, r, mode, offs, merge && !first);
+  launch_sweep(c, r, mode, offs, merge && !first, tail && merge && first);
   if ((mode & (MODE_GATED - 1)) == MODE_SOLVE) {
     launch_solve(c, count, lw);
     const bool inl = g.lm <= DOGLEG_INLINE_BLOCKS;
@@ -1208,7 +1218,10 @@
       HIPCHK(c, hipHostMalloc((void **)&c->h_pending, 256, hipHostMallocDefault));
     }
     const int offs = r.offs;
-    const GraphKey key = graph_key(r, (int)speculate, 0, true);
+    const bool tail = setup_tail(c, r);
+    c->stat_setup_tail = tail;
+    GraphKey key = graph_key(r, (int)speculate, 0, true);
+    key.setup |= tail ? SETUP_HEAD : 0;
     if (!(c->chunk_key == key)) {
       destroy_graph(c, c->chunk_key.count == count && ((c->chunk_key.offs ^ offs) & 2) == 0);
       c->chunk_key = key;
@@ -1223,10 +1236,11 @@
     hipGraphExec_t &first_graph = c->first[sv][c->publish ? 1 : 0][fuse ? 1 + fused_flag : 0][first_passes];
     auto capture = [&](hipGraphExec_t *out, bool setup, int npass, int tail_flag) {
       return capture_graph(c, c->stream, out, [&]() -> int {
-        if (setup) launch_setup(c, r, MODE_SOLVE);
+        if (setup) launch_setup(c, r, MODE_SOLVE, tail);
         bool gauged = false;
         for (int it = 0; it < npass; it++)
-          gauged = launch_iteration(c, r, MODE_SOLVE, speculate, it == 0, it == npass - 1, tail_flag >= 0, (offs & 2) || (setup && it == 0 && (offs & 1)));
+          gauged = launch_iteration(c, r, MODE_SOLVE, speculate, it == 0, it == npass - 1, tail_flag >= 0, (offs & 2) || (setup && it == 0 && (offs & 1)),
+                                    setup && tail && it == 0);
         if (tail_flag >= 0) {
           if (!gauged) {
             hipLaunchKernelGGL(k_gauge, dim3(1 + (g.lm + 1) / 2, count), dim3(128), 0, c->stream, c->d_base, c->L.total, 1);
@@ -2055,7 +2069,7 @@
     }
     return LFVIO_OK;
   }
-  const bool structural = k == "graph" || k == "linw" || k == "force_eig";
+  const bool structural = k == "graph" || k == "linw" || k == "force_eig" || k == "setup_split";
   if (structural) {
     if (int rc = join_inflight(c)) return rc;
   }
@@ -2074,6 +2088,7 @@
   } else if (k == "lm_half") c->lm_half = iv != 0;
   else if (k == "force_eig") c->force_eig = iv != 0;
   else if (k == "marg_ahead") c->marg_ahead = iv != 0;
+  else if (k == "setup_split") c->setup_split = iv != 0;
   else if (k == "break_next_chain") c->debug_break_chain = iv != 0;
   else if (k == "relo_route") c->relo_force = iv != 0;
   else {
@@ -2095,6 +2110,19 @@
   };
   if (k == "last_call") return put({(double)c->last_passes, (double)c->last_iters, (double)c->stat_chunks, (double)c->spec_count});
   if (k == "marg_ahead") return put({(double)c->stat_ahead_calls, (double)c->stat_ahead_hits});
+  if (k == "setup_split") return put({c->setup_split ? 1.0 : 0.0, c->stat_setup_tail ? 1.0 : 0.0});
+  if (k == "worker_clocks") {
+    if (!c->shadow || !c->d_base) return LFVIO_ERR_ARG;
+    if (int rc = join_inflight(c)) return rc;
+    for (auto &st : c->sstream)
+      if (st) HIPCHK(c, hipStreamSynchronize(st));
+    for (int wk = 0; wk < lfvio_ctx::WORKERS; wk++) {
+      long long t[32];
+      HIPCHK(c, hipMemcpy(t, c->d_base + (size_t)(c->batch + wk) * c->L.total + offsetof(Slot, dbg), sizeof(t), hipMemcpyDeviceToHost));
+      for (int i = 0; i < 32 && 32 * wk + i < n; i++) out[32 * wk + i] = (double)t[i];
+    }
+    return LFVIO_OK;
+  }
   if (k == "upload_times") return put({c->up_us[0], c->up_us[1], c->up_us[2], c->up_us[3]});
   if (k == "sweep_kernel") {
     const int r = sweep_kernel_of(c, (int)out[0]);
diff --git a/lf-vio_amd/lfvio/engine.py b/lf-vio_amd/lfvio/engine.py
--- a/lf-vio_amd/lfvio/engine.py
+++ b/lf-vio_amd/lfvio/engine.py
@@ -55,6 +55,14 @@
             self.configure("marg_ahead", int(on))
         q = self.query("marg_ahead", 2)
         return int(q[0]), int(q[1])
+
+    def setup_split(self, on=-1):
+        if on >= 0:
+            self.configure("setup_split", int(on))
+        return bool(self.query("setup_split", 2)[1])
+
+    def worker_clocks(self):
+        return self.query("worker_clocks", 64).reshape(2, 32)
 
     def break_next_chain(self):
         self.configure("break_next_chain", 1)
```
